# Nicholaswogan/clima

Measured on AMD Instinct MI355X. Metric: radiate() calls/sec, higher is better.
Workload: dtype f64; 1 GPU; ModernEarth column, one Radtran%radiate call: nz=200, nw=1000 (600 IR + 600 solar bins), 8 g-points, 8 zenith angles, nk=5; config 2 of BASELINE.json; parallelism=1 GPU

## Files before the change

### clima_amd/csrc/kernels.hip

```cpp
#include "radtran_dev.h"
#include <algorithm>
#include <cstring>
#include <mutex>
#include <set>
#include <utility>

namespace clima {

static bool ensure_max_lds(const void *fn, int bytes = 160 * 1024) {
  static std::mutex mu;
  static std::set<std::pair<int, const void *>> done;
  int dev = 0;
  if (hipGetDevice(&dev) != hipSuccess) return false;
  std::lock_guard<std::mutex> lk(mu);
  if (done.count({dev, fn})) return true;
  if (hipFuncSetAttribute(fn, hipFuncAttributeMaxDynamicSharedMemorySize, bytes) != hipSuccess) return false;
  done.insert({dev, fn});
  return true;
}
static int device_cus() {
  static std::mutex mu;
  static int cus[64] = {0};
  int dev = 0;
  if (hipGetDevice(&dev) != hipSuccess || dev < 0 || dev >= 64) return 256;
// ... 108 lines not shown
  double p = fma3(K.c[0], r, K.c[1]);
#pragma unroll
  for (int i = 2; i < 11; i++) p = fma3(p, r, K.c[i]);
  p = __builtin_fma(p, r, 0.5);
  p = __builtin_fma(p, r, 1.0);
  p = __builtin_fma(p, r, 1.0);
  return exp_scale(p, k);
}

constexpr int EXP2_N = 256;
__device__ const double EXP2_TAB[EXP2_N] = {
    1.0, 1.0027112750502025, 1.0054299011128027, 1.0081558981184175,
    1.0108892860517005, 1.0136300849514894, 1.016378314910953, 1.019133996077738,
    1.0218971486541166, 1.0246677928971357, 1.0274459491187637, 1.030231637686041,
    1.0330248790212284, 1.0358256936019572, 1.0386341019613787, 1.041450124688316,
    1.0442737824274138, 1.0471050958792898, 1.0499440858006872, 1.0527907730046264,
    1.0556451783605572, 1.0585073227945128, 1.061377227289262, 1.0642549128844645,
    1.0671404006768237, 1.0700337118202419, 1.0729348675259756, 1.075843889062791,
    1.0787607977571199, 1.0816856149932152, 1.0846183622133092, 1.0875590609177697,
    1.0905077326652577, 1.0934643990728858, 1.0964290818163769, 1.099401802630222,
    1.102382583307841, 1.1053714457017412, 1.1083684117236787, 1.1113735033448175,
    1.1143867425958924, 1.1174081515673693, 1.1204377524096067, 1.12347556733302,
    1.1265216186082418, 1.129575928566288, 1.1326385195987192, 1.1357094141578055,
    1.1387886347566916, 1.1418762039695616, 1.1449721444318042, 1.148076478840179,
    1.1511892299529827, 1.154310420590216, 1.1574400736337511, 1.1605782120274988,
    1.1637248587775775, 1.1668800369524817, 1.1700437696832502, 1.1732160801636373,
    1.1763969916502812, 1.1795865274628758, 1.182784710984341, 1.1859915656609938,
    1.189207115002721, 1.1924313825831512, 1.1956643920398273, 1.1989061670743806,
    1.202156731452703, 1.2054161090051239, 1.2086843236265816, 1.2119613992768012,
    1.215247359980469, 1.2185422298274085, 1.2218460329727576, 1.2251587936371455,
    1.22848053610687, 1.2318112847340759, 1.2351510639369334, 1.2384998981998165,
    1.241857812073484, 1.245224830175258, 1.2486009771892048, 1.2519862778663162,
    1.255380757024691, 1.2587844395497165, 1.2621973503942507, 1.2656195145788063,
    1.2690509571917332, 1.2724917033894028, 1.275941778396392, 1.2794012075056693,
    1.2828700160787783, 1.2863482295460256, 1.2898358734066657, 1.2933329732290895,
    1.2968395546510096, 1.3003556433796506, 1.3038812651919358, 1.3074164459346773,
    1.3109612115247644, 1.3145155879493546, 1.318079601266064, 1.3216532776031575,
    1.3252366431597413, 1.3288297242059544, 1.3324325470831615, 1.3360451382041458,
    1.339667524053303, 1.3432997311868353, 1.3469417862329458, 1.3505937158920345,
    1.3542555469368927, 1.3579273062129011, 1.3616090206382248, 1.365300717204012,
    1.3690024229745905, 1.3727141650876684, 1.3764359707545302, 1.380167867260238,
    1.383909881963832, 1.387662042298529, 1.3914243757719262, 1.3951969099662003,
    1.3989796725383112, 1.4027726912202048, 1.4065759938190154, 1.4103896082172707,
    1.4142135623730951, 1.4180478843204152, 1.4218926021691656, 1.4257477441054942,
    1.42961333839197, 1.433489413367789, 1.4373759974489824, 1.4412731191286257,
    1.4451808069770467, 1.449099089642035, 1.4530279958490526, 1.4569675544014438,
    1.460917794180647, 1.4648787441464057, 1.4688504333369818, 1.4728328908693675,
    1.4768261459394993, 1.4808302278224719, 1.4848451658727524, 1.488870989524397,
    1.4929077282912648, 1.4969554117672355, 1.5010140696264256, 1.5050837316234065,
    1.5091644275934228, 1.5132561874526098, 1.5173590411982147, 1.5214730189088146,
    1.5255981507445384, 1.529734466947287, 1.533881997840956, 1.5380407738316568,
    1.5422108254079407, 1.5463921831410214, 1.550584877685, 1.5547889397770887,
    1.559004400237837, 1.5632312899713576, 1.567469639965553, 1.5717194812923414,
    1.5759808451078865, 1.5802537626528246, 1.5845382652524937, 1.588834384317164,
    1.593142151342267, 1.597461597908627, 1.6017927556826934, 1.606135656416771,
    1.6104903319492543, 1.6148568142048607, 1.6192351351948637, 1.6236253270173289,
    1.6280274218573478, 1.632441451987275, 1.6368674497669644, 1.6413054476440063,
    1.645755478153965, 1.6502175739206177, 1.6546917676561943, 1.6591780921616162,
    1.6636765803267364, 1.6681872651305825, 1.6727101796415966, 1.6772453570178785,
    1.681792830507429, 1.6863526334483934, 1.6909247992693053, 1.6955093614893326,
    1.7001063537185235, 1.7047158096580513, 1.709337763100463, 1.713972247929926,
    1.718619298122478, 1.723278947746274, 1.7279512309618377, 1.732636182022311,
    1.7373338352737062, 1.7420442251551564, 1.746767386199169, 1.7515033530318782,
    1.7562521603732995, 1.761013843037584, 1.7657884359332727, 1.7705759740635547,
    1.7753764925265212, 1.7801900265154245, 1.785016611318935, 1.789856282321401,
    1.7947090750031072, 1.7995750249405351, 1.804454167806624, 1.809346539371032,
    1.8142521755003989, 1.8191711121586085, 1.8241033854070534, 1.8290490314048973,
    1.8340080864093424, 1.8389805867758937, 1.843966568958626, 1.8489660695104508,
    1.8539791250833855, 1.8590057724288205, 1.864046048397789, 1.8690999899412386,
    1.8741676341103, 1.8792490180565602, 1.8843441790323345, 1.8894531543909392,
    1.8945759815869656, 1.8997126981765553, 1.9048633418176741, 1.9100279502703899,
    1.9152065613971474, 1.9203992131630474, 1.925605943636125, 1.930826790987627,
    1.9360617934922943, 1.9413109895286405, 1.9465744175792332, 1.9518521162309783,
    1.9571441241754002, 1.9624504802089273, 1.9677712232331759, 1.9731063922552343,
    1.978456026387951, 1.9838201648502194, 1.9891988469672663, 1.9945921121709402};
constexpr double EXP2_PER_E = 369.3299304675746, EXP2_PER_10 = 850.4135922911647;
__device__ __forceinline__ double exp_tab_any(double x, double k, const double *s_tab) {
  double f, nf, r;
  {
#pragma clang fp contract(off)
    f = x * k;
    nf = __builtin_rint(f);
    r = f - nf;
  }
  const int n = (int)nf;
  const double t = s_tab[n & (EXP2_N - 1)];
  double p = 2.239395190875157e-12;
  p = __builtin_fma(p, r, 3.3083026805413713e-09);
  p = __builtin_fma(p, r, 3.6655655969101062e-06);
  p = __builtin_fma(p, r, 0.0027076061740622863);
  p = __builtin_fma(p, r, 1.0);
  return __builtin_ldexp(t * p, n >> 8);
}
__device__ __forceinline__ double exp_tab(double x, const double *s_tab) { return exp_tab_any(x, EXP2_PER_E, s_tab); }
__device__ __forceinline__ double ten2power_tab(double y, const double *s_tab) { return exp_tab_any(y, EXP2_PER_10, s_tab); }
__device__ __forceinline__ double rcp_n1(double x) {
  double r = __builtin_amdgcn_rcp(x);
  const double e = __builtin_fma(-x, r, 1.0);
  return __builtin_fma(r, e, r);
}

__device__ __forceinline__ double ten2power(double y) { return fast_exp(y * LN10); }

__device__ __forceinline__ double planck_fcn(double nu, double T, const ExpK &K) {
  return 1.0e3 * ((2.0 * PLANK * (nu * nu * nu)) / (C_LIGHT * C_LIGHT)) *
         ((1.0) / (fast_exp((PLANK * nu) / (K_BOLTZ_SI * T), K) - 1.0));
}
__device__ __forceinline__ double planck_fcn(double nu, double T) {
  return 1.0e3 * ((2.0 * PLANK * (nu * nu * nu)) / (C_LIGHT * C_LIGHT)) *
         ((1.0) / (fast_exp((PLANK * nu) / (K_BOLTZ_SI * T)) - 1.0));
}

template <int CTRL, int ROW_MASK, int BANK_MASK>
__device__ __forceinline__ double dpp_mov(double old, double src) {
  const long long o = __double_as_longlong(old), v = __double_as_longlong(src);
  const int lo = __builtin_amdgcn_update_dpp((int)o, (int)v, CTRL, ROW_MASK, BANK_MASK, false);
  const int hi = __builtin_amdgcn_update_dpp((int)(o >> 32), (int)(v >> 32), CTRL, ROW_MASK, BANK_MASK, false);
  return __longlong_as_double(((long long)hi << 32) | (unsigned int)lo);
}
constexpr int DPP_ROW_SHL = 0x100, DPP_ROW_SHR = 0x110, DPP_WAVE_SHR1 = 0x138, DPP_ROW_BCAST15 = 0x142, DPP_ROW_BCAST31 = 0x143;
template <int D>
__device__ __forceinline__ double row_shr(double old, double x) { return dpp_mov<DPP_ROW_SHR + D, 0xf, 0xf>(old, x); }
template <int D>
__device__ __forceinline__ double row_shl(double old, double x) { return dpp_mov<DPP_ROW_SHL + D, 0xf, 0xf>(old, x); }

__device__ __forceinline__ bool is_close(double a, double b, double tol) {
  return fabs(a - b) <= fabs(tol * fmax(fabs(a), fabs(b)));
}

__device__ __forceinline__ int bracket(const double *xt, int n, double x) {
  if (x < xt[0]) return 0;
  if (x >= xt[n - 1]) return n - 2;
  int lo = 0, hi = n - 1;
  while (hi - lo > 1) {
    int mid = (lo + hi) >> 1;
    if (x < xt[mid]) hi = mid; else lo = mid;
  }
  return lo;
}

constexpr int PREP_AXIS_MAX = 1024;
constexpr int PREP_ZERO_BLOCKS = 32;

__device__ __forceinline__ ColumnDev column_at(const ColumnDev &c0, const BatchStrides &bs, const int cb) {
  ColumnDev c = c0;
  const size_t oc = (size_t)cb * bs.col, op = (size_t)cb * bs.prep;
  c.T += oc; c.P += oc; c.dz += oc; c.dens += oc; c.pdens += oc; c.radii += oc; c.T_surface += oc;
  c.meta += 2 * oc;
  c.log10P += op; c.cols += op; c.foreign_col += op; c.absw += op; c.q += op;
  c.ix += 2 * op;
  return c;
}

__global__ __launch_bounds__(256) void k_prep(PrepParams p) {
  __shared__ double s_axis[PREP_AXIS_MAX];
  const int nz = p.nz;
  const int cb = blockIdx.y;
  const ColumnDev c = column_at(p.col, p.bs, cb);
  const int *src = c.meta + 1 + nz;
  if (blockIdx.x == 0) {
    for (int j = threadIdx.x; j < nz; j += blockDim.x) {
      const double Pj = c.P[j], dzj = c.dz[j];
      double fc = 0.0;
      for (int i0 = 0; i0 < p.nsp; i0 += 8) {
        double d[8];
#pragma unroll
        for (int k = 0; k < 8; k++) d[k] = c.dens[min(i0 + k, p.nsp - 1) * nz + j];
#pragma unroll
        for (int k = 0; k < 8; k++) {
          const int i = i0 + k;
          if (i < p.nsp) {
            const double col = d[k] * dzj;
            c.cols[i * nz + j] = col;
            if (p.has_cont && i != p.LH2O) fc = fc + col;
          }
        }
      }
      c.log10P[j] = log10(Pj);
      c.foreign_col[j] = fc;
    }
    return;
  }
  if ((int)blockIdx.x > p.nslots + p.nabs) {
    const int zb = (int)blockIdx.x - (p.nslots + p.nabs + 1);
    const int arr = zb / PREP_ZERO_BLOCKS, part = zb - arr * PREP_ZERO_BLOCKS;
    double *dst = p.zero_ptr[arr] + (size_t)cb * p.bs.res;
    const size_t n = p.zero_count[arr];
    for (size_t i = (size_t)part * blockDim.x + threadIdx.x; i < n; i += (size_t)PREP_ZERO_BLOCKS * blockDim.x) dst[i] = 0.0;
    return;
  }
  if ((int)blockIdx.x > p.nslots) {
    const int e = (int)blockIdx.x - p.nslots - 1;
    const int a = p.abs_a[e], b = p.abs_b[e], kind = p.abs_kind[e];
    for (int j = threadIdx.x; j < nz; j += blockDim.x) {
      double w;
      if (kind == ABS_CIA) w = c.dens[a * nz + j] * c.dens[b * nz + j] * c.dz[j];
      else if (kind == ABS_COLUMN) w = c.dens[a * nz + j] * c.dz[j];
      else if (kind == ABS_H2O_SELF) w = c.dens[a * nz + j] * (c.dens[a * nz + j] * c.dz[j]);
      else if (kind == ABS_ZERO) w = 0.0;
      else {
        double fc = 0.0;
        for (int i = 0; i < p.nsp; i++)
          if (i != p.LH2O) fc = fc + c.dens[i * nz + j] * c.dz[j];
        w = c.dens[a * nz + j] * fc;
      }
      c.absw[e * nz + j] = w;
    }
    return;
  }
  const int s = blockIdx.x - 1;
  const SlotDev &sl = p.slots[s];
  const bool in_lds = sl.n <= PREP_AXIS_MAX;
  const double *in = sl.source <= 0 ? c.P : sl.source == 1 ? c.T : c.radii + (size_t)(sl.source - 2) * nz;
  const int j0 = threadIdx.x;
  int js0 = 0;
  double x0 = 0.0;
  if (j0 < nz) { js0 = sl.source < 0 ? j0 : src[j0]; x0 = in[j0]; }
  if (in_lds)
    for (int i = threadIdx.x; i < sl.n; i += blockDim.x) s_axis[i] = sl.axis[i];
  __syncthreads();
  const double *axis = in_lds ? s_axis : sl.axis;
  for (int j = threadIdx.x; j < nz; j += blockDim.x) {
    const int js = j == j0 ? js0 : (sl.source < 0 ? j : src[j]);
    const double xin = (j == j0 && js == j) ? x0 : in[js];
    double x;
    if (sl.source < 0) x = log10(xin * 1.0e6);
    else if (sl.source == 0) x = log10(xin);
    else x = xin;
    if (sl.flag_clamp && (x < sl.lo || x > sl.hi)) atomicMax(c.err_flag, p.call_id);
    x = fmin(fmax(x, sl.lo), sl.hi);
    const int i = bracket(axis, sl.n, x);
    c.ix[s * nz + j] = i;
    c.q[s * nz + j] = (x - axis[i]) / (axis[i + 1] - axis[i]);
  }
}

void launch_prep(const PrepParams &p, hipStream_t s) {
  hipLaunchKernelGGL(k_prep, dim3(1 + p.nslots + p.nabs + p.nzero * PREP_ZERO_BLOCKS, p.ncol > 0 ? p.ncol : 1), dim3(256), 0, s, p);
}


__device__ __forceinline__ double lerp1(const double *f, int i, double q) {
  const double p1 = 1.0 - q;
  return p1 * f[i] + q * f[i + 1];
}

constexpr int OP_THREADS = 256;
constexpr int HWREG_HW_ID_WAVE_ID = (3 << 11) | (0 << 6) | 4;

template <bool COHERENT>
__device__ __forceinline__ void st_opr(double *p, double v) {
  if constexpr (COHERENT) __hip_atomic_store(p, v, __ATOMIC_RELAXED, __HIP_MEMORY_SCOPE_AGENT);
  else *p = v;
}
template <bool COHERENT>
__device__ __forceinline__ double ld_opr(const double *p) {
  if constexpr (COHERENT) return __hip_atomic_load(p, __ATOMIC_RELAXED, __HIP_MEMORY_SCOPE_AGENT);
  else return *p;
}

#ifdef CLIMA_STAMPS
__device__ long long *g_stamp_buf = nullptr;
#endif

template <bool TIGHT>
constexpr int rb_lo(int k) {
  constexpr int wide[8] = {0, 1, 5, 10, 18, 27, 39, 52};
  constexpr int tight[8] = {0, 5, 12, 19, 27, 35, 45, 55};
  return TIGHT ? tight[k] : wide[k];
}
template <bool TIGHT>
constexpr int rb_hi(int k) {
  constexpr int wide[8] = {0, 11, 24, 36, 45, 53, 58, 62};
  constexpr int tight[8] = {0, 8, 18, 28, 36, 44, 51, 58};
  return TIGHT ? tight[k] : wide[k];
}

constexpr unsigned long long KEY_IDX_MASK = 0x1f8ULL;
__device__ __forceinline__ double key_weight(const double key, const double *s_wxy) {
  const unsigned int off = (unsigned int)__double_as_longlong(key) & (unsigned int)KEY_IDX_MASK;
  return *(const double *)((const char *)s_wxy + off);
}

__device__ __forceinline__ void rebin_window(const double (&key)[64], const bool xys, const double *s_wxy,
                                             const double *s_Ew, const double *rW, double (&out)[8]) {
  asm volatile("" ::: "memory");
  double E[8];
#pragma unroll
  for (int k = 1; k < 8; k++) E[k] = s_Ew[k];
  double C = 0.0, IC = 0.0, Ie[9];
#pragma unroll
  for (int k = 1; k < 8; k++) Ie[k] = -1.0e300;
  constexpr int RB = 8;
  double wn[RB];
#pragma unroll
  for (int u = 0; u < RB; u++) wn[u] = key_weight(key[u], s_wxy);
#pragma unroll
  for (int pb = 0; pb < 64; pb += RB) {
    double wv[RB];
#pragma unroll
    for (int u = 0; u < RB; u++) wv[u] = wn[u];
    if (pb + RB < 64) {
#pragma unroll
      for (int u = 0; u < RB; u++)
        wn[u] = key_weight(key[pb + RB + u], s_wxy);
    }
    const double Cb = C, ICb = IC;
#pragma unroll
    for (int u = 0; u < RB; u++) {
      const int j = pb + u;
      const double v = key[j];
#pragma unroll
      for (int k = 1; k < 8; k++) {
        if (j >= rb_lo<true>(k) && j <= rb_hi<true>(k))
          Ie[k] = dmax(Ie[k], __builtin_fma(v, E[k] - C, IC));
      }
      IC = __builtin_fma(v, wv[u], IC);
      C = C + wv[u];
    }
    if (!xys) {
      double c2 = Cb, ic2 = ICb;
#pragma unroll
      for (int u = 0; u < RB; u++) {
        const int j = pb + u;
        const double v = key[j];
#pragma unroll
        for (int k = 1; k < 8; k++) {
          if (j >= rb_lo<false>(k) && j <= rb_hi<false>(k) && !(j >= rb_lo<true>(k) && j <= rb_hi<true>(k)))
            Ie[k] = dmax(Ie[k], __builtin_fma(v, E[k] - c2, ic2));
        }
        ic2 = __builtin_fma(v, wv[u], ic2);
        c2 = c2 + wv[u];
      }
    }
  }
  Ie[8] = IC;
  out[0] = Ie[1] * rW[0];
#pragma unroll
  for (int q = 1; q < 8; q++) out[q] = (Ie[q + 1] - Ie[q]) * rW[q];
}

#include "rorr_xys_asm.inc"
#ifndef CLIMA_RORR_ASM
#define CLIMA_RORR_ASM 1
#endif
constexpr bool RORR_ASM = CLIMA_RORR_ASM != 0;

template <int RM>
__device__ __forceinline__ void rorr_mix8(const double (&x)[8], const double (&y)[8],
                                          double (*sI)[OP_THREADS], const int tid, const int tile,
                                          const double *s_wxy, const double *s_E,
                                          const double *s_Ew, const double *rW,
                                          double (&out)[8], const double *rorr_tab, long long *stamps = nullptr, const int stamp_slot = 0) {
  (void)stamps; (void)stamp_slot;
  double key[64];
  bool ysorted = true, xsorted = true;
#pragma unroll
  for (int j = 0; j < 7; j++) {
    ysorted = ysorted && (y[j] <= y[j + 1]);
    xsorted = xsorted && (x[j] <= x[j + 1]);
  }
  const bool ys = __all(ysorted), xys = ys && __all(xsorted);
  if constexpr (RM == 0 && RORR_ASM) {
    if (__builtin_expect(xys, 1)) {
      double xx[8], yy[8];
#pragma unroll
      for (int g = 0; g < 8; g++) { xx[g] = x[g]; yy[g] = y[g]; }
      typedef __attribute__((address_space(3))) const double lds_cdouble;
      const unsigned wxy_addr = (unsigned)(unsigned long)(lds_cdouble *)s_wxy;
      asm volatile(RORR_XYS_ASM_TEXT
                   : "+v"(xx[0]), "+v"(xx[1]), "+v"(xx[2]), "+v"(xx[3]), "+v"(xx[4]), "+v"(xx[5]), "+v"(xx[6]), "+v"(xx[7]),
                     "+v"(yy[0]), "+v"(yy[1]), "+v"(yy[2]), "+v"(yy[3]), "+v"(yy[4]), "+v"(yy[5]), "+v"(yy[6]), "+v"(yy[7])
                   : "v"(wxy_addr), "s"(rorr_tab)
                   : RORR_XYS_ASM_CLOBBERS);
#pragma unroll
      for (int g = 0; g < 8; g++) out[g] = yy[g];
      STAMP(stamps, stamp_slot);
      return;
    }
  }
#pragma unroll
  for (int i = 0; i < 8; i++) {
#pragma unroll
    for (int j = 0; j < 8; j++) {
      const double v = x[i] + y[j];
      unsigned long long b = (unsigned long long)__double_as_longlong(v);
      b = (b & ~KEY_IDX_MASK) | (unsigned long long)((i * 8 + j) << 3);
      key[i * 8 + j] = __longlong_as_double((long long)b);
    }
  }
#define CE(a, b)                              \
  {                                           \
    const double lo_ = dmin(key[a], key[b]);  \
    const double hi_ = dmax(key[a], key[b]);  \
    key[a] = lo_;                             \
    key[b] = hi_;                             \
  }
#define CE_X(a, b) \
  if (!xys) CE(a, b)
#define CE_MERGE_BEGIN(P, M)
#define CE_MERGE_END
  if (!ys) {
#define CE_FULL_HEAD
#include "sort_network_64.inc"
#undef CE_FULL_HEAD
  }
  if (!xys) {
#define CE_L8_FIRST
#include "sort_network_64.inc"
#undef CE_L8_FIRST
  }
#define CE_L8_REST
#include "sort_network_64.inc"
#undef CE_L8_REST
  if (!xys) {
#define CE_L16_FIRST
#include "sort_network_64.inc"
#undef CE_L16_FIRST
  }
#define CE_L16_REST
#include "sort_network_64.inc"
#undef CE_L16_REST
  if (!xys) {
#define CE_L32_FIRST
#include "sort_network_64.inc"
#undef CE_L32_FIRST
  }
#define CE_L32_REST
#include "sort_network_64.inc"
#undef CE_L32_REST
#undef CE_MERGE_BEGIN
#undef CE_MERGE_END
#undef CE_X
#undef CE
  STAMP(stamps, stamp_slot);
  if constexpr (RM == 0) {
    rebin_window(key, xys, s_wxy, s_Ew, rW, out);
    return;
  }
  const double *E = s_Ew;
  constexpr bool MULTI = RM == 2;
  double S = 0.0, c0 = 0.0;
  double bk = E[1], bn = E[2];
  const double *en = s_E + 2;
  double *slot = &sI[0][tid];
  double *const slot_end = &sI[0][tid] + 8 * OP_THREADS;
  constexpr int RB = 8;
  double wn[RB];
#pragma unroll
  for (int u = 0; u < RB; u++) wn[u] = key_weight(key[u], s_wxy);
#pragma unroll
  for (int pb = 0; pb < 64; pb += RB) {
    double wv[RB];
#pragma unroll
    for (int u = 0; u < RB; u++) wv[u] = wn[u];
    if (pb + RB < 64) {
#pragma unroll
      for (int u = 0; u < RB; u++)
        wn[u] = key_weight(key[pb + RB + u], s_wxy);
    }
#pragma unroll
    for (int u = 0; u < RB; u++) {
      const double v = key[pb + u];
      const double w = wv[u];
      const double c1 = c0 + w;
      if (c1 > bk) {
        *slot = __builtin_fma(v, bk - c0, S);
        slot += OP_THREADS;
        bk = bn;
        en++;
        if constexpr (MULTI) {
          while (c1 > bk) {
            *slot = __builtin_fma(v, bk - c0, S);
            slot += OP_THREADS;
            bk = *en;
            en++;
          }
        }
      }
      bn = *en;
      S = __builtin_fma(v, w, S);
      c0 = c1;
    }
  }
  for (; slot < slot_end; slot += OP_THREADS) *slot = S;
  double Ik[8];
#pragma unroll
  for (int q = 0; q < 8; q++) Ik[q] = sI[q][tid];
  out[0] = Ik[0] * rW[0];
#pragma unroll
  for (int q = 1; q < 8; q++) out[q] = (Ik[q] - Ik[q - 1]) * rW[q];
}

struct LayerTerms {
  double tausg, taua, tauc, tausc, taup, tausp, gt;
};

template <int RM, bool CUSTOM, bool COHERENT>
__device__ __forceinline__ void opacity8_body(const OpacityParams &p, const int tile, const size_t oc,
                                              const size_t opf, const size_t oo) {
  const ColumnDev &c = p.col;
  constexpr int NG = 8;
  __shared__ double sI[RM == 0 ? 1 : NG][OP_THREADS];
  __shared__ __align__(512) double s_wxy[NG * NG];
  __shared__ double s_E[NG + 4];
  const int tid = threadIdx.x;
  __shared__ double s_Ew[2 * NG + 1];
  __shared__ double s_e2[EXP2_N];
  __shared__ double rW[NG];
  {
    static_assert(EXP2_N == OP_THREADS, "one table entry per thread");
    const double v_wxy = p.wxy[tid & (NG * NG - 1)];
    const double v_Ep = p.wbin_e_pad[min(tid, NG + 3)];
    const double v_e2 = EXP2_TAB[tid];
    const double v_e = p.wbin_e[min(tid, NG)], v_e1 = p.wbin_e[min(tid + 1, NG)];
    const double v_w = p.wbin[min(max(tid - (NG + 1), 0), NG - 1)];
    if (tid < NG * NG) s_wxy[tid] = v_wxy;
    if (tid < NG + 4) s_E[tid] = v_Ep;
    s_e2[tid] = v_e2;
    if (tid < 2 * NG + 1) s_Ew[tid] = tid < NG + 1 ? v_e : v_w;
    if (tid < NG) rW[tid] = 1.0 / (v_e1 - v_e);
  }
  __syncthreads();

#ifdef CLIMA_STAMPS
  const long long wt0 = __builtin_amdgcn_s_memrealtime();
#endif
  const int nz = p.nz;
  const int nsrc = c.meta[2 * oc + 0];
  const long total = (long)p.nbins * nsrc;
  long t = (long)tile * OP_THREADS + tid;
  const bool valid = t < total;
  if (!valid) t = total - 1;
  const int l = p.bin_lo + (int)(t / nsrc);
  const int ent = c.meta[2 * oc + 1 + (int)(t % nsrc)];
  const int j = ent & SRC_LAYER;
  const bool pair = (ent & SRC_PAIR) != 0, exact = (ent & SRC_EXACT) != 0;
  const int n = nz - 1 - j;

  STAMP(p.stamps, 0);
  auto layer_terms = [&](const int jl, LayerTerms &o) {
#ifdef CLIMA_EXP_NOTERMS
    o.tausg = 1e-3; o.taua = 1e-3; o.tauc = TINY; o.tausc = TINY * TINY; o.taup = 0.0; o.tausp = 0.0; o.gt = 0.0;
    if (jl >= 0) return;
#endif
    const double dzj = c.dz[oc + jl];
    double tausg = 0.0;
  #pragma unroll 4
    for (int i = 0; i < p.nray; i++) tausg = tausg + p.ray[i].data[l] * c.cols[opf + p.ray[i].sp1 * nz + jl];
    double taua = 0.0;
    constexpr int AB = ABS_BATCH;
    for (int e0 = 0; e0 < p.nabs; e0 += AB) {
      int ixx[AB];
      double qq[AB], ww[AB];
  #pragma unroll
      for (int u = 0; u < AB; u++) {
        const AbsEntry &x = p.abs[e0 + u];
        ixx[u] = c.ix[2 * opf + x.slot * nz + jl];
        qq[u] = c.q[opf + x.slot * nz + jl];
        ww[u] = c.absw[opf + (e0 + u) * nz + jl];
      }
      double v0[AB], v1[AB];
  #pragma unroll
      for (int u = 0; u < AB; u++) {
        const AbsEntry &x = p.abs[e0 + u];
#ifdef CLIMA_EXP_NODEP
        const double *base = x.data + (x.nT ? (size_t)l * x.nT : (size_t)l);
#else
        const double *base = x.data + (x.nT ? (size_t)l * x.nT + ixx[u] : (size_t)l);
#endif
        v0[u] = base[0];
        v1[u] = base[x.nT ? 1 : 0];
      }
  #pragma unroll
      for (int u = 0; u < AB; u++) {
        const AbsEntry &x = p.abs[e0 + u];
        double sgm = v0[u];
        if (x.nT) sgm = ten2power_tab((1.0 - qq[u]) * v0[u] + qq[u] * v1[u], s_e2);
        taua = taua + sgm * ww[u];
      }
    }
    double tauc = TINY, tausc = TINY * TINY;
    double g0c = TINY;
    if constexpr (CUSTOM) {
      const int ix = c.ix[2 * opf + p.cust.slot * nz + jl];
      const double q = c.q[opf + p.cust.slot * nz + jl];
      const size_t o = (size_t)l * p.cust.nP;
      tauc = lerp1(p.cust.dtau + o, ix, q) * dzj;
      const double w0c = lerp1(p.cust.w0 + o, ix, q);
      g0c = lerp1(p.cust.g0 + o, ix, q);
      tausc = w0c * tauc;
    }
    double tausp = 0.0, taup = 0.0;
    double tausp_1[MAX_PART], gtp[MAX_PART];
    for (int i = 0; i < p.npart; i++) {
      const PartDev &pt = p.part[i];
      const int ix = c.ix[2 * opf + pt.slot * nz + jl];
      const double q = c.q[opf + pt.slot * nz + jl];
      const double w0p = lerp1(pt.w0 + (size_t)l * pt.nrad, ix, q);
      const double qext = lerp1(pt.qext + (size_t)l * pt.nrad, ix, q);
      gtp[i] = lerp1(pt.gt + (size_t)l * pt.nrad, ix, q);
      const double rr = c.radii[oc + pt.p_ind * nz + jl];
      const double taup_1 = qext * PI * (rr * rr) * c.pdens[oc + pt.p_ind * nz + jl] * dzj;
      taup = taup + taup_1;
      tausp_1[i] = w0p * taup_1;
      tausp = tausp + tausp_1[i];
    }
    double gt = 0.0;
    for (int i = 0; i < p.npart; i++) gt = gt + gtp[i] * tausp_1[i] / fmax(TAU_MIN, (tausp + tausg + tausc));
    gt = gt + g0c * tausc / fmax(TAU_MIN, (tausp + tausg + tausc));
    gt = fmin(gt, MAX_GT);
    o.tausg = tausg; o.taua = taua; o.tauc = tauc; o.tausc = tausc; o.taup = taup; o.tausp = tausp; o.gt = gt;
  };
  LayerTerms lt;
  const bool terms_first = (__builtin_amdgcn_s_getreg(HWREG_HW_ID_WAVE_ID) & 1) == 0;
  __shared__ double s_lt[7][OP_THREADS];
  if (terms_first) {
    layer_terms(j, lt);
    if constexpr (RM == 0 && RORR_ASM) {
      s_lt[0][tid] = lt.tausg; s_lt[1][tid] = lt.taua; s_lt[2][tid] = lt.tauc; s_lt[3][tid] = lt.tausc;
      s_lt[4][tid] = lt.taup; s_lt[5][tid] = lt.tausp; s_lt[6][tid] = lt.gt;
    }
  }

  STAMP(p.stamps, 1);
  auto k_times_col = [&](const int s, const int jl, const int iP, const int iT, const double q1, const double q2,
                         double (&kc)[NG]) {
    const KDev &kd = p.k[s];
    const double p1 = 1.0 - q1, p2 = 1.0 - q2;
    const double *slab = kd.log10k + (size_t)l * kd.nT * kd.nP * NG;
    const double *f11 = slab + ((size_t)iT * kd.nP + iP) * NG;
    const double *f21 = f11 + NG;
    const double *f12 = f11 + (size_t)kd.nP * NG;
    const double *f22 = f12 + NG;
    const double col = c.cols[opf + kd.sp * nz + jl];
#pragma unroll
    for (int g = 0; g < NG; g++) {
      const double fx1 = p1 * f11[g] + q1 * f21[g];
      const double fx2 = p1 * f12[g] + q1 * f22[g];
      kc[g] = ten2power_tab(p2 * fx1 + q2 * fx2, s_e2) * col;
    }
  };
  double tk[NG];
#pragma unroll
  for (int g = 0; g < NG; g++) tk[g] = 0.0;
  int iP_n = c.ix[2 * opf + p.k[0].slotP * nz + j], iT_n = c.ix[2 * opf + p.k[0].slotT * nz + j];
  double q1_n = c.q[opf + p.k[0].slotP * nz + j], q2_n = c.q[opf + p.k[0].slotT * nz + j];
  for (int s = 0; s < p.nk; s++) {
    const int iP = iP_n, iT = iT_n;
    const double q1 = q1_n, q2 = q2_n;
    int jv = j;
    if constexpr (RM == 0 && RORR_ASM) asm volatile("" : "+v"(jv));
    if (s + 1 < p.nk) {
      const KDev &kn = p.k[s + 1];
      iP_n = c.ix[2 * opf + kn.slotP * nz + jv]; iT_n = c.ix[2 * opf + kn.slotT * nz + jv];
      q1_n = c.q[opf + kn.slotP * nz + jv]; q2_n = c.q[opf + kn.slotT * nz + jv];
    }
    double kc[NG];
    k_times_col(s, jv, iP, iT, q1, q2, kc);
    STAMP(p.stamps, 2 + 3 * s);
    if (s == 0) {
#pragma unroll
      for (int g = 0; g < NG; g++) tk[g] = kc[g];
    } else {
#ifdef CLIMA_STAMPS
      if (tile == 100 && threadIdx.x == 0) g_stamp_buf = p.stamps;
#endif
      double out[NG];
      rorr_mix8<RM>(tk, kc, sI, tid, tile, s_wxy, s_E, s_Ew, rW, out, p.rorr_tab, p.stamps, 21 + s);
#pragma unroll
      for (int g = 0; g < NG; g++) tk[g] = out[g];
      STAMP(p.stamps, 4 + 3 * s);
    }
  }
  if (!terms_first) {
    layer_terms(j, lt);
  } else if constexpr (RM == 0 && RORR_ASM) {
    lt.tausg = s_lt[0][tid]; lt.taua = s_lt[1][tid]; lt.tauc = s_lt[2][tid]; lt.tausc = s_lt[3][tid];
    lt.taup = s_lt[4][tid]; lt.tausp = s_lt[5][tid]; lt.gt = s_lt[6][tid];
  }
  STAMP(p.stamps, 20);
#ifdef CLIMA_STAMPS
  if (p.stamps && (tid & 63) == 0) {
    const long w = (long)tile * (OP_THREADS / 64) + (tid >> 6);
    p.stamps[64 + 2 * w] = wt0;
    p.stamps[64 + 2 * w + 1] = __builtin_amdgcn_s_memrealtime();
  }
#endif

  auto store_layer = [&](const int nn, const LayerTerms &T, const double (&tkv)[NG]) {
    asm volatile("" ::: "memory");
    const double *wbin = s_Ew + NG + 1;
    double tb = 0.0;
    const size_t base = ((size_t)l * NG) * nz + nn;
    const double scat = T.tausg + T.tausp + T.tausc;
    if (p.write_w0) {
#pragma unroll
      for (int g = 0; g < NG; g++) {
        const double tau = T.tausg + T.taua + T.taup + tkv[g] + T.tauc;
        double w0;
        if (tau <= TAU_MIN) w0 = 0.0;
        else w0 = fmin(MAX_W0, scat / tau);
        st_opr<COHERENT>(&p.w0[oo + base + (size_t)g * nz], w0);
      }
    }
#pragma unroll
    for (int g = 0; g < NG; g++) {
      const double tau = T.tausg + T.taua + T.taup + tkv[g] + T.tauc;
      st_opr<COHERENT>(&p.tau[oo + base + (size_t)g * nz], tau);
      tb = tb + tau * wbin[g];
    }
    st_opr<COHERENT>(&p.scat[oo + (size_t)l * nz + nn], scat);
    st_opr<COHERENT>(&p.tau_band[oo + (size_t)l * nz + nn], tb);
    st_opr<COHERENT>(&p.g[oo + (size_t)l * nz + nn], T.gt);
  };
  if (valid) {
    store_layer(n, lt, tk);
    if (pair) {
      if (exact) {
        store_layer(n - 1, lt, tk);
      } else {
        LayerTerms lt2;
        layer_terms(j + 1, lt2);
        if (p.nk == 1) {
          double tk2[NG];
          k_times_col(0, j + 1, c.ix[2 * opf + p.k[0].slotP * nz + j], c.ix[2 * opf + p.k[0].slotT * nz + j], c.q[opf + p.k[0].slotP * nz + j],
                      c.q[opf + p.k[0].slotT * nz + j], tk2);
          store_layer(n - 1, lt2, tk2);
        } else {
          store_layer(n - 1, lt2, tk);
        }
      }
    }
  }
}

template <int RM, bool CUSTOM>
__global__ __launch_bounds__(OP_THREADS, 2) void k_opacity8(OpacityParams p) {
  opacity8_body<RM, CUSTOM, false>(p, (int)blockIdx.x, 0, 0, 0);
}

constexpr int OPG_MAX_NG = 32;

__global__ __launch_bounds__(64) void k_opacity_generic(OpacityParams p, int N2) {
  extern __shared__ __align__(16) double sm[];
  const int ng = p.ng, n2 = ng * ng, nz = p.nz;
  double *s_key = sm;
  double *s_cum = s_key + N2;
  double *s_tk = s_cum + (n2 + 1);
  double *s_kc = s_tk + ng;
  double *s_out = s_kc + ng;
  double *s_wxy = s_out + ng;
  int *s_idx = (int *)(s_wxy + n2);
  const int lane = threadIdx.x;
  for (int m = lane; m < n2; m += 64) s_wxy[m] = p.wxy[m];
  const ColumnDev &c = p.col;
  const long t = blockIdx.x;
  const int l = p.bin_lo + (int)(t / nz);
  const int j = (int)(t % nz);
  const int n = nz - 1 - j;
  const double dzj = c.dz[j];
  const int jk = (p.nk >= 2) ? c.meta[1 + nz + j] : j;

  double tausg = 0.0;
  for (int i = 0; i < p.nray; i++) tausg = tausg + p.ray[i].data[l] * c.cols[p.ray[i].sp1 * nz + j];
  double taua = 0.0;
  for (int e = 0; e < p.nabs; e++) {
    const AbsEntry &x = p.abs[e];
    double sgm;
    if (x.nT) {
      const int ix = c.ix[x.slot * nz + j];
      const double q = c.q[x.slot * nz + j];
      const double *base = x.data + (size_t)l * x.nT + ix;
      sgm = ten2power((1.0 - q) * base[0] + q * base[1]);
    } else {
      sgm = x.data[l];
    }
    taua = taua + sgm * c.absw[e * nz + j];
  }
  double tauc = TINY, tausc = TINY * TINY, g0c = TINY;
  if (p.cust.on) {
    const int ix = c.ix[p.cust.slot * nz + j];
    const double q = c.q[p.cust.slot * nz + j];
    const size_t o = (size_t)l * p.cust.nP;
    tauc = lerp1(p.cust.dtau + o, ix, q) * dzj;
    const double w0c = lerp1(p.cust.w0 + o, ix, q);
    g0c = lerp1(p.cust.g0 + o, ix, q);
    tausc = w0c * tauc;
  }
  double tausp = 0.0, taup = 0.0;
  double tausp_1[MAX_PART], gtp[MAX_PART];
  for (int i = 0; i < p.npart; i++) {
    const PartDev &pt = p.part[i];
    const int ix = c.ix[pt.slot * nz + j];
    const double q = c.q[pt.slot * nz + j];
    const double w0p = lerp1(pt.w0 + (size_t)l * pt.nrad, ix, q);
    const double qext = lerp1(pt.qext + (size_t)l * pt.nrad, ix, q);
    gtp[i] = lerp1(pt.gt + (size_t)l * pt.nrad, ix, q);
    const double rr = c.radii[pt.p_ind * nz + j];
    const double taup_1 = qext * PI * (rr * rr) * c.pdens[pt.p_ind * nz + j] * dzj;
    taup = taup + taup_1;
    tausp_1[i] = w0p * taup_1;
    tausp = tausp + tausp_1[i];
  }
  double gt = 0.0;
  for (int i = 0; i < p.npart; i++) gt = gt + gtp[i] * tausp_1[i] / fmax(TAU_MIN, (tausp + tausg + tausc));
  gt = gt + g0c * tausc / fmax(TAU_MIN, (tausp + tausg + tausc));
  gt = fmin(gt, MAX_GT);

  for (int s = 0; s < p.nk; s++) {
    const KDev &kd = p.k[s];
    if (lane < ng) {
      const int iP = c.ix[kd.slotP * nz + jk], iT = c.ix[kd.slotT * nz + jk];
      const double q1 = c.q[kd.slotP * nz + jk], q2 = c.q[kd.slotT * nz + jk];
      const double p1 = 1.0 - q1, p2 = 1.0 - q2;
      const double *f11 = kd.log10k + (size_t)l * kd.nT * kd.nP * ng + ((size_t)iT * kd.nP + iP) * ng;
      const double *f21 = f11 + ng, *f12 = f11 + (size_t)kd.nP * ng, *f22 = f12 + ng;
      const double fx1 = p1 * f11[lane] + q1 * f21[lane];
      const double fx2 = p1 * f12[lane] + q1 * f22[lane];
      const double v = ten2power(p2 * fx1 + q2 * fx2) * c.cols[kd.sp * nz + jk];
      if (s == 0) s_tk[lane] = v;
      else s_kc[lane] = v;
    }
    __syncthreads();
    if (s == 0) continue;
    for (int m = lane; m < N2; m += 64) {
      double v = __longlong_as_double(0x7ff0000000000000LL);
      if (m < n2) v = s_tk[m / ng] + s_kc[m % ng];
      s_key[m] = v;
      s_idx[m] = m;
    }
    __syncthreads();
    for (int k = 2; k <= N2; k <<= 1) {
      for (int d = k >> 1; d > 0; d >>= 1) {
        for (int u = lane; u < (N2 >> 1); u += 64) {
          const int i = ((u & ~(d - 1)) << 1) | (u & (d - 1));
          const int x = i + d;
          const bool up = (i & k) == 0;
          const double ka = s_key[i], kb = s_key[x];
          const int ia = s_idx[i], ib = s_idx[x];
          const bool gtr = (ka > kb) || (ka == kb && ia > ib);
          if (gtr == up) { s_key[i] = kb; s_key[x] = ka; s_idx[i] = ib; s_idx[x] = ia; }
        }
        __syncthreads();
      }
    }
    {
      const int seg = (N2 + 63) / 64;
      double tot = 0.0;
      for (int q = 0; q < seg; q++) {
        const int m = lane * seg + q;
        if (m < n2) tot = tot + s_wxy[s_idx[m]];
      }
      double incl = tot;
#pragma unroll
      for (int d = 1; d < 64; d <<= 1) {
        const double nb = __shfl_up(incl, d);
        if (lane >= d) incl = incl + nb;
      }
      double cum = incl - tot;
      if (lane == 0) { cum = 0.0; s_cum[0] = 0.0; }
      for (int q = 0; q < seg; q++) {
        const int m = lane * seg + q;
        if (m < n2) { cum = cum + s_wxy[s_idx[m]]; s_cum[m + 1] = cum; }
      }
    }
    __syncthreads();
    if (lane < ng) {
      const double b0 = p.wbin_e[lane], b1 = p.wbin_e[lane + 1];
      int lo = 0, hi = n2;
      while (lo < hi) { const int mid = (lo + hi) >> 1; if (s_cum[mid + 1] <= b0) lo = mid + 1; else hi = mid; }
      double acc = 0.0;
      for (int m = lo; m < n2; m++) {
        const double e0 = s_cum[m], e1 = s_cum[m + 1];
        if (e0 >= b1) break;
        const double a = e0 > b0 ? e0 : b0, b = e1 < b1 ? e1 : b1;
        if (b > a) acc = acc + (b - a) * s_key[m];
      }
      s_out[lane] = acc / (b1 - b0);
    }
    __syncthreads();
    if (lane < ng) s_tk[lane] = s_out[lane];
    __syncthreads();
  }

  if (lane < ng) {
    const double tau = tausg + taua + taup + s_tk[lane] + tauc;
    double w0;
    if (tau <= TAU_MIN) w0 = 0.0;
    else w0 = fmin(MAX_W0, (tausg + tausp + tausc) / tau);
    const size_t o = ((size_t)l * ng + lane) * nz + n;
    p.tau[o] = tau;
// ... 1456 lines not shown
    if (lane == 63) rho = 0.0;
  }
  const double mm = rcp_nr(1.0 - rho * dU);
  constexpr bool STEP_REGS = NW == 4;
  double *sStep = sF0 + (size_t)4 * NW * (nl + 1) + threadIdx.x;
  double stA[WSCAN_STEPS], stB[WSCAN_STEPS];
  {
    double dummy = 0.0, bq = wave_reverse(uU * mm);
    wscan_build(dummy, bq, stA);
    double sb = dD * (1.0 + dU * mm * rho);
    dummy = 0.0;
    wscan_build(dummy, sb, stB);
    if constexpr (!STEP_REGS) {
#pragma unroll
      for (int k = 0; k < WSCAN_STEPS; k++) {
        sStep[(size_t)k * blockDim.x] = stA[k];
        sStep[(size_t)(WSCAN_STEPS + k) * blockDim.x] = stB[k];
      }
    }
  }
  const double kA = uU * mm * rho;
  const double kS = dU * mm;
  int face[L + 1];
#pragma unroll
  for (int s = 0; s <= L; s++) face[s] = a + max(s - pad, 0);

  for (int c0 = c_begin; c0 < c_end; c0 += IRB_TILE) {
    const int nt = min(IRB_TILE, c_end - c0);
    __syncthreads();
    for (int idx = threadIdx.x; idx < nt * nl; idx += blockDim.x) {
      const int cj = idx / nl, n = idx - cj * nl;
      const double *Tc = p.T + (size_t)(c0 + cj) * p.b_T;
      const double temp = (n == nz) ? p.T_surface[(size_t)(c0 + cj) * p.b_Ts] : Tc[nz - 1 - n];
      sB[(size_t)cj * nl + n] = p.bplanck ? p.bplanck[n] : planck_fcn(avg_freq, temp);
    }
    __syncthreads();
    for (int cj = 0; cj < nt; cj++) {
      const double *Bc = sB + (size_t)cj * nl;
      double Bf[L + 1];
#pragma unroll
      for (int s = 0; s <= L; s++) Bf[s] = Bc[face[s]];
      double dd[2 * L], cpbv[L], cmbv[L];
      double cp0_top, b1n_last = 0.0;
      {
        double dpv = 0.0;
        E4 u = make_e(G[0], X[0]);
#pragma unroll
        for (int t = 0; t < L; t++) {
          const double Bt = Bf[t], Bb = Bf[t + 1];
          const double b1n = (Bb - Bt) * itau[t];
          const double b0n = (itau[t] == 0.0) ? 0.5 * (Bt + Bb) : Bt;
          const double cp0 = PI * (b0n + b1n * rq[t]);
          cpbv[t] = PI * (b0n + b1n * (tauv[t] + rq[t]));
          const double cm0 = PI * (b0n - b1n * rq[t]);
          cmbv[t] = PI * (b0n + b1n * (tauv[t] - rq[t]));
          if (t == 0) {
            cp0_top = cp0;
            dpv = (0.0 - cm0) * rr[0];
            dd[0] = dpv;
          } else {
            const E4 v = make_e(G[t], X[t]);
            const double E1 = v.e2 * (cp0 - cpbv[t - 1]) - v.e4 * (cm0 - cmbv[t - 1]);
            const double dn = E1 * rr[2 * t - 1] - ar[2 * t - 1] * dpv;
            dd[2 * t - 1] = dn;
            const double E2 = u.e3 * (cp0 - cpbv[t - 1]) + u.e1 * (cmbv[t - 1] - cm0);
            dpv = E2 * rr[2 * t] - ar[2 * t] * dn;
            dd[2 * t] = dpv;
            u = v;
          }
          if (t == L - 1) b1n_last = b1n;
        }
        const double Ssfc = hard ? emis * PI * Bf[L] : PI * (Bf[L] + 0.5 * b1n_last);
        const double E = is_sfc ? Ssfc - cpbv[L - 1] + Rsfc * cmbv[L - 1] : 0.0 - cpbv[L - 1];
        dd[2 * L - 1] = E * rr[2 * L - 1] - ar[2 * L - 1] * dpv;
      }
      {
        double al = 0.0;
#pragma unroll
        for (int r = 2 * L - 1; r >= 0; r--) {
          al = dd[r] - cc[r] * al;
          dd[r] = al;
        }
      }
      const double uS = empty ? 0.0 : dd[0] * ea3 - dd[1] * ea4 + cp0_top;
      const double dS = empty ? 0.0 : dd[2 * L - 2] * eb3 + dd[2 * L - 1] * eb4 + cmbv[L - 1];
      const double sgr = wscan_apply(wave_reverse(uS + kA * dS),
                                     [&](int k) { return STEP_REGS ? stA[k] : sStep[(size_t)k * blockDim.x]; });
      const double sig = wave_reverse(wave_shr1(sgr));
      const double sa = wscan_apply(dS + kS * (rho * dS + sig),
                                    [&](int k) { return STEP_REGS ? stB[k] : sStep[(size_t)(WSCAN_STEPS + k) * blockDim.x]; });
      const double Din = wave_shr1(sa);
      const double Uin = mm * (rho * dS + sig + rho * dD * Din);
      const int buf = cj & 1;
      double *sFu = sF0 + (size_t)buf * 2 * NW * (nl + 1) + (size_t)(0 * NW + wave) * (nl + 1);
      double *sFd = sF0 + (size_t)buf * 2 * NW * (nl + 1) + (size_t)(1 * NW + wave) * (nl + 1);
      double top_up = 0.0;
#pragma unroll
      for (int t = 0; t < L; t++) {
        const int i = a + t - pad;
        const E4 e = make_e(G[t], X[t]);
        const double y1 = dd[2 * t] + be[2 * t] * Uin + ga[2 * t] * Din;
        const double y2 = dd[2 * t + 1] + be[2 * t + 1] * Uin + ga[2 * t + 1] * Din;
        const int lv = t >= pad ? i + 1 : nl;
        sFu[lv] = wcol * (y1 * e.e1 + y2 * e.e2 + cpbv[t]);
        sFd[lv] = wcol * (y1 * e.e3 + y2 * e.e4 + cmbv[t]);
        if (t == 0) top_up = (y1 * e.e3 - y2 * e.e4) + cp0_top;
      }
      if (is_toa) {
        sFu[0] = wcol * top_up;
        sFd[0] = 0.0;
      }
      __syncthreads();
      for (int n = threadIdx.x; n < nl; n += blockDim.x) {
        const double *sF = sF0 + (size_t)buf * 2 * NW * (nl + 1);
        const size_t o = (size_t)(c0 + cj) * p.b_out + (size_t)ll * nl + (nz - n);
        double fu = 0.0, fd = 0.0;
        if (g0 > 0) { fu = p.ir_fup_a[o]; fd = p.ir_fdn_a[o]; }
#pragma unroll
        for (int w = 0; w < NW; w++) {
          fu = fu + sF[(size_t)(0 * NW + w) * (nl + 1) + n];
          fd = fd + sF[(size_t)(1 * NW + w) * (nl + 1) + n];
        }
        p.ir_fup_a[o] = fu;
        p.ir_fdn_a[o] = fd;
      }
    }
  }
  __syncthreads();
  }
}

bool launch_twostream_ir_batch(TwoStreamParams &p, int ncol, hipStream_t s, int force_nw) {
  const int lmax = std::max((p.nz + 63) / 64, p.force_slots);
  if (lmax > 8 || p.n_ir <= 0 || ncol <= 0 || p.ng < 1) return false;
  const int nw = (lmax > 4 || p.ng > 8 || force_nw == 4) ? 4 : 8;
  const size_t lds = sizeof(double) * ((size_t)IRB_TILE * ((size_t)p.nz + 1) + (size_t)4 * nw * ((size_t)p.nz + 2) + (nw == 8 ? 2 * WSCAN_STEPS * 64 * nw : 0));
  if (lds > 160 * 1024) return false;
  using Kern = void (*)(TwoStreamParams, int, int);
  static const Kern kern8[4] = {k_twostream_ir_batch<1, 8>, k_twostream_ir_batch<2, 8>, k_twostream_ir_batch<3, 8>, k_twostream_ir_batch<4, 8>};
  static const Kern kern4[8] = {k_twostream_ir_batch<1, 4>, k_twostream_ir_batch<2, 4>, k_twostream_ir_batch<3, 4>, k_twostream_ir_batch<4, 4>,
                                k_twostream_ir_batch<5, 4>, k_twostream_ir_batch<6, 4>, k_twostream_ir_batch<7, 4>, k_twostream_ir_batch<8, 4>};
  const Kern k = nw == 8 ? kern8[lmax - 1] : kern4[lmax - 1];
  if (!ensure_max_lds((const void *)k)) return false;
  int cpb = (ncol + 3) / 4;
  if (cpb < IRB_TILE) cpb = std::min(ncol, IRB_TILE);
  const dim3 grid(p.n_ir, 1, (ncol + cpb - 1) / cpb), blk(64 * nw);
  hipLaunchKernelGGL(k, grid, blk, lds, s, p, ncol, cpb);
  return true;
}

#ifndef FUSED_NZMAX
#define FUSED_NZMAX 8
#endif
template <int RM, bool CUSTOM, int LSEL, bool PAIRED = false, bool HALF = false>
__global__ __launch_bounds__(OP_THREADS, 2) void k_fused(OpacityParams op, TwoStreamParams ts, FusedParams fp) {
  extern __shared__ __align__(16) double lds[];
  const int per_col = fp.n_op + fp.n_ts;
  const int cb = (int)blockIdx.x / per_col, loc = (int)blockIdx.x - cb * per_col;
  if (loc < fp.n_op) {
    __builtin_amdgcn_s_setprio(1);
    const size_t oc = (size_t)cb * fp.bs.col;
    if ((long)loc * OP_THREADS < (long)op.nbins * op.col.meta[2 * oc])
      opacity8_body<RM, CUSTOM, true>(op, loc, oc, (size_t)cb * fp.bs.prep, (size_t)cb * fp.bs.opr);
    __builtin_amdgcn_fence(__ATOMIC_RELEASE, "workgroup");
    asm volatile("s_waitcnt vmcnt(0)" ::: "memory");
    __syncthreads();
    if (threadIdx.x == 0)
      __hip_atomic_store(&fp.done[(size_t)cb * fp.bs.done + loc], fp.call_id, __ATOMIC_RELAXED, __HIP_MEMORY_SCOPE_AGENT);
    return;
  }
  const int b = loc - fp.n_op;
  int gy, bl;
  {
    const int nS = ts.n_sol, nI = ts.n_ir, E = fp.sol_early, Lt = nS - E;
    if constexpr (HALF) {
      gy = 0;
      bl = b < E ? b : b < E + nI ? nS + (b - E) : b - nI;
    } else {
      const int seg[6] = {E, E, nI, nI, Lt, Lt};
      int r = b, k = 0;
      while (k < 5 && r >= seg[k]) { r -= seg[k]; k++; }
      gy = k & 1;
      bl = k < 2 ? r : k < 4 ? nS + r : E + r;
    }
  }
  const bool solar = bl < ts.n_sol;
  const int ll = solar ? ts.sol_lo + bl : ts.ir_lo + (bl - ts.n_sol);
  const int l = (solar ? ts.sol_start : ts.ir_start) + ll;
#ifdef CLIMA_STAMPS
  if (op.stamps && threadIdx.x == 0 && cb == 0) op.stamps[64 + 2 * 3128 + 3 * b] = __builtin_amdgcn_s_memrealtime();
#endif
  __shared__ int s_ok;
  if (threadIdx.x == 0) {
    const int nsrc = op.col.meta[2 * (size_t)cb * fp.bs.col];
    const long t0 = (long)(l - op.bin_lo) * nsrc;
    const int d0 = max((int)(t0 / OP_THREADS), 0), d1 = min((int)((t0 + nsrc - 1) / OP_THREADS), fp.n_op - 1);
    const int *done = fp.done + (size_t)cb * fp.bs.done;
    int ok = 1;
    for (int d = d0; d <= d1 && ok; d++) {
      int spins = 0;
      while (__hip_atomic_load(&done[d], __ATOMIC_RELAXED, __HIP_MEMORY_SCOPE_AGENT) != fp.call_id) {
        __builtin_amdgcn_s_sleep(16);
        if (++spins > fp.max_spins) { ok = 0; break; }
      }
    }
    if (!ok) atomicMax(fp.timeout_flag, fp.call_id);
    s_ok = ok;
  }
  __syncthreads();
  if (!s_ok) return;
#ifdef CLIMA_STAMPS
  if (op.stamps && threadIdx.x == 0 && cb == 0) op.stamps[64 + 2 * 3128 + 3 * b + 1] = __builtin_amdgcn_s_memrealtime();
  const int tslot = HALF ? (b == fp.sol_early / 2 ? 32 : (b == fp.sol_early + ts.n_ir / 2 ? 48 : -1))
                         : (b == 1500) ? 32 : (b == 2200 ? 48 : -1);
#else
  const int tslot = -1;
#endif
  const TsOfs co{(size_t)cb * fp.bs.opr, (size_t)cb * fp.bs.col, (size_t)cb * fp.bs.res};
  if constexpr (HALF) {
    if (solar) twostream_p_body<LSEL, true, FUSED_NZMAX, true, false, false, true>(ts, bl, lds, gy, 0, tslot, co);
    else twostream_p_body<LSEL, false, 0, true, false, false, true>(ts, bl - ts.n_sol, lds, gy, 0, tslot, co);
  } else if constexpr (LSEL == 0 && PAIRED) {
    if (fp.slots == 2) {
      if (solar) twostream_p_body<2, true, FUSED_NZMAX, true, true, true>(ts, bl, lds, gy, 0, tslot, co);
      else twostream_p_body<2, false, 0, true, true, true>(ts, bl - ts.n_sol, lds, gy, 0, tslot, co);
    } else {
      if (solar) twostream_p_body<4, true, FUSED_NZMAX, true, true, true>(ts, bl, lds, gy, 0, tslot, co);
      else twostream_p_body<4, false, 0, true, true, true>(ts, bl - ts.n_sol, lds, gy, 0, tslot, co);
    }
  } else if constexpr (LSEL == 0) {
    if (fp.slots == 2) {
      if (solar) twostream_p_body<2, true, FUSED_NZMAX, true, true>(ts, bl, lds, gy, 0, tslot, co);
      else twostream_p_body<2, false, 0, true, true>(ts, bl - ts.n_sol, lds, gy, 0, tslot, co);
    } else if (fp.slots == 3) {
      if (solar) twostream_p_body<3, true, FUSED_NZMAX, true, true>(ts, bl, lds, gy, 0, tslot, co);
      else twostream_p_body<3, false, 0, true, true>(ts, bl - ts.n_sol, lds, gy, 0, tslot, co);
    } else {
      if (solar) twostream_p_body<4, true, FUSED_NZMAX, true, true>(ts, bl, lds, gy, 0, tslot, co);
      else twostream_p_body<4, false, 0, true, true>(ts, bl - ts.n_sol, lds, gy, 0, tslot, co);
    }
  } else {
    if (solar) twostream_p_body<LSEL, true, FUSED_NZMAX, true, false, PAIRED>(ts, bl, lds, gy, 0, tslot, co);
    else twostream_p_body<LSEL, false, 0, true, false, PAIRED>(ts, bl - ts.n_sol, lds, gy, 0, tslot, co);
  }
#ifdef CLIMA_STAMPS
  __syncthreads();
  if (op.stamps && threadIdx.x == 0 && cb == 0) op.stamps[64 + 2 * 3128 + 3 * b + 2] = __builtin_amdgcn_s_memrealtime();
#endif
}

int fused_tiles(const OpacityParams &op) {
  return (int)(((long)op.nbins * op.nsrc + OP_THREADS - 1) / OP_THREADS);
}

static size_t wave_lds(int nz, int cols) { return sizeof(double) * (3 * cols + 1) * ((size_t)nz + 1); }
static int wave_groups(int ng) { return (ng + TSW_COLS - 1) / TSW_COLS; }

LaunchPlan plan_radiate(const PlanIn &in) {
  LaunchPlan pl{};
  const int slots = (in.nz + 63) / 64, nb = in.n_sol + in.n_ir;
  const bool plain = in.rebin_mode == 0 && !in.cust_on;
  const bool coop8 = !in.batch && in.ng == 8 && (long)in.op_n * in.nsrc <= in.coop_items;
  if (in.compute_opacity) {
    if (in.ng < 1 || in.ng > OPG_MAX_NG) pl.opacity = OP_UNSUPPORTED;
    else if (in.ng == 8) pl.opacity = coop8 ? OP_COOP : OP_TILE;
    else pl.opacity = in.generic_opacity ? OP_GENERIC : OP_COOP;
    pl.coop_ng = in.ng <= 8 ? 8 : in.ng <= 16 ? 16 : 32;
  }

  const bool want_fused = in.compute_opacity && in.fused && in.allow_fused && !coop8 && !in.ts_block_mode;
  const bool covered = in.ng == 8 && slots >= 2 && slots <= 8 && in.nzen <= MAX_ZEN && (slots <= 4 || plain) &&
                       (long)in.op_n * in.nz > 0 && nb > 0;
  if (want_fused && covered) {
    const int hs = (in.nz + 31) / 32, ps = 2 * ((in.nz / 2 + 63) / 64);
    TsPlan &f = pl.fused;
    if (!in.no_half && plain && hs >= 3 && hs <= 7) { f.form = TS_HALF; f.slots = hs; }
    else if (in.ncol <= 1 && in.allow_paired && in.all_pairs && !(in.nz & 1) && plain && ps <= 8) { f.form = TS_PAIRED; f.slots = ps; }
    else { f.form = TS_WAVE; f.slots = slots; }
    f.cols = f.form == TS_HALF ? 2 * TSW_COLS : TSW_COLS;
    f.groups = f.per_launch = in.ng / f.cols;
    f.lds = wave_lds(in.nz, f.cols);
    pl.write_w0 = !in.w0_from_scat;
  } else {
    pl.write_w0 = true;
  }

  const int lmax = std::max(slots, in.force_slots);
  if ((in.ir_batch || (!in.ts_block_mode && in.nzen <= MAX_ZEN)) && lmax <= 8 && wave_lds(in.nz, TSW_COLS) <= 64 * 1024) {
    const int hs = (in.nz + 31) / 32;
    TsPlan &t = pl.ts;
    if (!in.no_half && in.ng % 8 == 0 && hs >= 3 && hs <= 7 && in.force_slots == 0 && in.nzen <= MAX_ZEN &&
        !(in.ng == 8 && in.n_sol > 0 && nb < 512)) { t.form = TS_HALF; t.slots = hs; t.cols = 2 * TSW_COLS; }
    else { t.form = TS_WAVE; t.slots = lmax; t.cols = TSW_COLS; }
    t.groups = (in.ng + t.cols - 1) / t.cols;
    t.per_launch = t.groups <= 2 ? t.groups : 1;
    t.lds = wave_lds(in.nz, t.cols);
  }
  if (!in.ir_batch) pl.block = plan_block(in.nz, in.ng, in.ts_ncols_env);

  const bool headed_fused = in.fused && in.allow_fused && !coop8;
  const bool whole_stores = headed_fused ? pl.fused.form == TS_HALF : (pl.ts.form == TS_HALF && pl.ts.groups == 1);
  pl.prep_clears = in.compute_opacity && !in.ts_block_mode && slots <= 8 && wave_groups(in.ng) >= 2 && !whole_stores;
  pl.caller_clears = in.ir_batch && wave_groups(in.ng) > 1;
  pl.ts.zero_launch = pl.ts.groups > 1 && !pl.prep_clears && !pl.caller_clears;
  return pl;
}

using FusedKern = void (*)(OpacityParams, TwoStreamParams, FusedParams);
static FusedKern fused_kernel(const TsPlan &f, int rebin_mode, bool cust_on) {
  static const FusedKern kp[3] = {k_fused<0, false, 0, true>, k_fused<0, false, 6, true>, k_fused<0, false, 8, true>};
  static const FusedKern kh[5] = {k_fused<0, false, 3, false, true>, k_fused<0, false, 4, false, true>, k_fused<0, false, 5, false, true>,
                                  k_fused<0, false, 6, false, true>, k_fused<0, false, 7, false, true>};
  static const FusedKern k04[2][3] = {{k_fused<0, false, 0>, k_fused<1, false, 0>, k_fused<2, false, 0>},
                                      {k_fused<0, true, 0>, k_fused<1, true, 0>, k_fused<2, true, 0>}};
  static const FusedKern k58[4] = {k_fused<0, false, 5>, k_fused<0, false, 6>, k_fused<0, false, 7>, k_fused<0, false, 8>};
  if (f.form == TS_HALF) return kh[f.slots - 3];
  if (f.form == TS_PAIRED) return kp[f.slots <= 4 ? 0 : f.slots == 6 ? 1 : 2];
  return f.slots <= 4 ? k04[cust_on ? 1 : 0][rebin_mode] : k58[f.slots - 5];
}

bool launch_fused(const OpacityParams &op, TwoStreamParams ts, FusedParams fp, const TsPlan &f, hipStream_t s) {
  if (f.form == TS_NONE) return false;
  fp.n_op = fused_tiles(op);
  fp.n_ts = (ts.n_sol + ts.n_ir) * f.groups;
  fp.slots = f.slots;
  if (fp.ncol < 1) fp.ncol = 1;
  {
    const long first_round_bins = ((long)2 * device_cus() * OP_THREADS) / std::max(op.nsrc, 1);
    fp.sol_early = (int)std::min<long>(ts.n_sol, std::max<long>(0, first_round_bins - (long)(ts.sol_start + ts.sol_lo - op.bin_lo)));
  }
  ts.col_base = 0; ts.accumulate = f.groups > 1 ? 1 : 0;
  ts.scat = op.scat; ts.w0_from_scat = op.write_w0 ? 0 : 1;
  const long items = (long)fp.ncol * (fp.n_op + fp.n_ts);
  const FusedKern k = fused_kernel(f, op.rebin_mode, op.cust.on != 0);
  if (f.lds > 48 * 1024 && !ensure_max_lds((const void *)k, 64 * 1024)) return false;
  hipLaunchKernelGGL(k, dim3((unsigned)items), dim3(OP_THREADS), f.lds, s, op, ts, fp);
  return true;
}

bool launch_fused_twostream_only(TwoStreamParams &ts, int slots, const int *meta_nsrc, hipStream_t s, bool half, bool paired) {
  if (ts.ng != 8 || slots < 2 || slots > 8 || (ts.nz + 63) / 64 > slots || ts.nzen > MAX_ZEN) return false;
  if (half && (paired || slots < 3 || slots > 7 || (ts.nz + 31) / 32 > slots)) return false;
  if (paired && ((ts.nz & 1) || (slots & 1) || 2 * ((ts.nz / 2 + 63) / 64) > slots)) return false;
  TsPlan f{};
  f.form = half ? TS_HALF : paired ? TS_PAIRED : TS_WAVE;
  f.slots = slots;
  f.cols = half ? 2 * TSW_COLS : TSW_COLS;
  f.groups = ts.ng / f.cols;
  f.lds = wave_lds(ts.nz, f.cols);
  OpacityParams op;
  memset(&op, 0, sizeof(op));
  op.nz = ts.nz;
  op.col.meta = meta_nsrc;
  FusedParams fp;
  memset(&fp, 0, sizeof(fp));
  fp.ncol = 1;
  fp.n_op = 0;
  fp.n_ts = (ts.n_sol + ts.n_ir) * f.groups;
  fp.slots = slots;
  fp.sol_early = ts.n_sol;
  ts.col_base = 0; ts.accumulate = half ? 0 : 1;
  const FusedKern k = fused_kernel(f, 0, false);
  if (f.lds > 48 * 1024 && !ensure_max_lds((const void *)k, 64 * 1024)) return false;
  hipLaunchKernelGGL(k, dim3(fp.n_ts), dim3(OP_THREADS), f.lds, s, op, ts, fp);
  return true;
}

#ifndef CLIMA_INT_CHUNK
#define CLIMA_INT_CHUNK 32
#endif
constexpr int INT_CHUNK = CLIMA_INT_CHUNK;

__global__ __launch_bounds__(256) void k_integrate_partial(IntegrateParams p) {
  const int nl = p.nz + 1;
  const int a = blockIdx.y;
  const bool sol = a >= 2;
  if (sol && !p.do_solar) return;
  const double *src = a == 0 ? p.ir_fup_a : a == 1 ? p.ir_fdn_a : a == 2 ? p.sol_fup_a : p.sol_fdn_a;
  const double *freq = sol ? p.sol_freq : p.ir_freq;
  const int lo = sol ? p.sol_lo : p.ir_lo, cnt = sol ? p.sol_n : p.ir_n;
  const int l0 = lo + blockIdx.x * INT_CHUNK;
  const int l1 = min(lo + cnt, l0 + INT_CHUNK);
  for (int i = threadIdx.x; i < nl; i += blockDim.x) {
    double acc = 0.0;
    if (l0 < l1) {
      double v[INT_CHUNK];
#pragma unroll
      for (int k = 0; k < INT_CHUNK; k++) v[k] = (l0 + k < l1) ? src[(size_t)(l0 + k) * nl + i] : 0.0;
#pragma unroll
      for (int k = 0; k < INT_CHUNK; k++)
        if (l0 + k < l1) acc = __builtin_fma(v[k], freq[l0 + k] - freq[l0 + k + 1], acc);
    }
    p.partial[((size_t)a * p.nchunk + blockIdx.x) * nl + i] = acc;
  }
}

__global__ __launch_bounds__(1024) void k_integrate_final(IntegrateParams p) {
  const int nl = p.nz + 1;
  if (p.timeout_out && threadIdx.x == 0) {
    const int t = *p.timeout_flag;
    *p.timeout_out = (t == p.id_opr ? 1.0 : 0.0) + (t == p.id_sol ? 1024.0 : 0.0);
  }
  for (int t = threadIdx.x; t < 4 * nl; t += blockDim.x) {
    const int a = t / nl, i = t - a * nl;
    if (a >= 2 && !p.do_solar) {
      if (p.flux_part) p.flux_n[a * nl + i] = p.flux_part[a * nl + i];
      continue;
    }
    double acc = 0.0;
#pragma unroll 8
    for (int k = 0; k < p.nchunk; k++) acc = acc + p.partial[((size_t)a * p.nchunk + k) * nl + i];
    p.flux_n[a * nl + i] = acc;
    if (p.flux_part) p.flux_part[a * nl + i] = acc;
  }
  __syncthreads();
  if (p.f_total)
    for (int i = threadIdx.x; i < nl; i += blockDim.x)
      p.f_total[i] = (p.flux_n[3 * nl + i] - p.flux_n[2 * nl + i]) + (p.flux_n[1 * nl + i] - p.flux_n[0 * nl + i]);
}

__global__ __launch_bounds__(256) void k_integrate_partial_b(BatchIntegrateParams p) {
  const int nl = p.nz + 1;
  const int a = blockIdx.y, col = blockIdx.z;
  const double *src = (a == 0 ? p.fup_a : p.fdn_a) + (size_t)col * p.spec_stride;
  const int l0 = p.ir_lo + blockIdx.x * INT_CHUNK;
  const int l1 = min(p.ir_lo + p.ir_n, l0 + INT_CHUNK);
  if (l1 <= l0) {
    for (int i = threadIdx.x; i < nl; i += blockDim.x) p.partial[(((size_t)col * 2 + a) * p.nchunk + blockIdx.x) * nl + i] = 0.0;
    return;
  }
  for (int i = threadIdx.x; i < nl; i += blockDim.x) {
    double v[INT_CHUNK], df[INT_CHUNK];
#pragma unroll
    for (int k = 0; k < INT_CHUNK; k++) {
      const int l = min(l0 + k, l1 - 1);
      v[k] = src[(size_t)l * nl + i];
      df[k] = p.freq[l] - p.freq[l + 1];
    }
    double acc = 0.0;
#pragma unroll
    for (int k = 0; k < INT_CHUNK; k++)
      if (l0 + k < l1) acc = __builtin_fma(v[k], df[k], acc);
    p.partial[(((size_t)col * 2 + a) * p.nchunk + blockIdx.x) * nl + i] = acc;
  }
}

__global__ __launch_bounds__(256) void k_integrate_final_b(BatchIntegrateParams p) {
  const int nl = p.nz + 1;
  const int col = blockIdx.x;
  for (int i = threadIdx.x; i < nl; i += blockDim.x) {
    double up = 0.0, dn = 0.0;
    for (int k0 = 0; k0 < p.nchunk; k0 += 8) {
      double u[8], d[8];
#pragma unroll
      for (int k = 0; k < 8; k++) {
        const int kk = min(k0 + k, p.nchunk - 1);
        u[k] = p.partial[(((size_t)col * 2 + 0) * p.nchunk + kk) * nl + i];
        d[k] = p.partial[(((size_t)col * 2 + 1) * p.nchunk + kk) * nl + i];
      }
#pragma unroll
      for (int k = 0; k < 8; k++)
        if (k0 + k < p.nchunk) { up = up + u[k]; dn = dn + d[k]; }
    }
    double *o = p.out + (size_t)(p.col0 + col) * nl;
    o[i] = up;
    o[p.out_arr + i] = dn;
    o[2 * p.out_arr + i] = (p.flux_n[3 * nl + i] - p.flux_n[2 * nl + i]) + (dn - up);
  }
}

void launch_integrate_batch(const BatchIntegrateParams &p, int ncol, hipStream_t s) {
  hipLaunchKernelGGL(k_integrate_partial_b, dim3(p.nchunk, 2, ncol), dim3(256), 0, s, p);
  hipLaunchKernelGGL(k_integrate_final_b, dim3(ncol), dim3(256), 0, s, p);
}

int integrate_chunks(int nbins) { return nbins <= 0 ? 1 : (nbins + INT_CHUNK - 1) / INT_CHUNK; }

#ifndef CLIMA_INT_LV
#define CLIMA_INT_LV 16
#endif
#ifndef CLIMA_INT_CG
#define CLIMA_INT_CG 32
#endif
constexpr int INT_LV = CLIMA_INT_LV;
constexpr int INT_CG = CLIMA_INT_CG;

__global__ __launch_bounds__(INT_LV * INT_CG) void k_integrate_one(IntegrateParams p) {
// ... 262 lines not shown
```

### clima_amd/csrc/radtran_api.hip

```cpp
#include "../../include/clima_radtran_hip.h"
#include "radtran_dev.h"

#include <rccl/rccl.h>
#include <sys/stat.h>
#include <unistd.h>
#include <ctime>

#include <algorithm>
#include <cmath>
#include <cstdio>
#include <cstdlib>
#include <chrono>
#include <cstring>
#include <functional>
#include <set>
#include <string>
#include <utility>
#include <limits>
#include <vector>

using namespace clima;

namespace {

// ... 51 lines not shown
    n = 0;
    owned = true;
  }
  ~DevBuf() { release(); }
};

struct KTabHost {
  int sp, ng, nP, nT;
  std::vector<double> weights, log10P, temp, log10k;
  DevBuf<double> d_log10k, d_log10P, d_temp;
};
struct XsHost {
  int type, dim, sp1, sp2, nT;
  std::vector<double> temp, data;
  DevBuf<double> d_data, d_temp;
};
struct PartHost {
  int p_ind, nrad;
  std::vector<double> radii, w0, qext, gt;
  DevBuf<double> d_radii, d_w0, d_qext, d_gt;
};

struct Radtran;
struct ChannelObj {
  Radtran *parent = nullptr;
  int which = 0;
  int ind_start = 0, ind_end = -1, nw = 0;
  std::vector<double> wavl, freq;
  DevBuf<double> d_freq;
};
struct WrkObj {
  Radtran *parent = nullptr;
  int which = 0;
  DevBuf<double> fup_a, fdn_a, amean, tau_band;
};

struct BatchRun {
  int n = 0, first_call = 0, CH = 0;
  bool one_launch = false, pending = false;
  double *ISR = nullptr, *OLR = nullptr, *fluxes = nullptr;
  double *rows = nullptr;
};

struct Radtran {
  unsigned magic = MAGIC;
  int state = 0;
  int nz = 0, nsp = 0, np = 0, nw = 0, ng = 0;
  std::vector<double> wavl, freq;
  std::vector<KTabHost *> k;
  std::vector<XsHost *> cia, ray, pxs;
  std::vector<PartHost *> part;
  std::vector<int> part_slot;
  bool has_cont = false;
  int LH2O = -1, cont_nT = 0;
  std::vector<double> cont_temp, cont_H2O, cont_foreign;
  DevBuf<double> d_cont_temp, d_cont_H2O, d_cont_foreign;
  std::vector<double> wbin, wbin_e, wxy;
  DevBuf<double> d_wbin, d_wbin_e, d_wbin_e_pad, d_wxy, d_freq, d_rorr_tab;
  ChannelObj ir, sol;
  WrkObj wrk_ir, wrk_sol;
  double diurnal_fac = 0.5;
  std::vector<double> zenith_u, zenith_w, surface_albedo, surface_emissivity, photons_sol;
  bool has_hard_surface = true;
  double ir_tau_min = 1.0e-6;
  double photon_scale_factor = 1.0;
  bool fields_dirty = true;
  DevBuf<double> d_zen_u, d_zen_w, d_zen_iu, d_partial, d_albedo, d_emis, d_photons, d_am_f1, d_am_f2, d_am_dw;
  int nslots = 0;
  std::vector<std::string> species_names, particle_names, particle_data;
  std::string k_method_name = "RandomOverlapResortRebin", continuum_model = "MT_CKD";
  std::vector<SlotDev> slots;
  bool cust_on = false;
  int cust_nP = 0;
  std::vector<double> cust_axis;
  DevBuf<double> d_cust_axis, d_cust_dtau, d_cust_w0, d_cust_g0;
  DevBuf<double> d_bT, d_bTs, d_bup, d_bdn, d_bpartial, d_bout;
  DevBuf<double> d_green, d_green_acc, d_green_in, d_gen_out;
  int green_last_n = -1;
  double *h_bout = nullptr;
  size_t h_bout_n = 0;
  char *h_green = nullptr;
  size_t h_green_n = 0;
  DevBuf<int> d_green_idx;
  int ir_green_mode = 1;
  long ir_green_batches = 0;
  DevBuf<double> d_col;
  size_t meta_ofs = 0;
  int nsrc = 0;
  bool all_pairs_exact = false;
  DevBuf<double> d_prep;
  size_t prep_count = 0;
  std::vector<AbsEntry> abs_entries;
  DevBuf<double> d_zero_xs;
  DevBuf<int> d_err;
#ifdef CLIMA_STAMPS
  DevBuf<long long> d_stamps;
#endif
  double *h_col = nullptr;
  double *h_col_dev = nullptr;
  size_t col_count = 0;
  bool column_has_particles = false;
  bool column_loaded = false;
  hipEvent_t ev_upload = nullptr;
  bool upload_pending = false;
  int call_id = 0, checked_id = 0;
  long upload_id = 0, opr_upload_id = 0;
  std::string deferred_err;
  int fused_max_spins = 400000, checked_timeout = 0, solar_id = 0, fused_fallbacks = 0;
  bool last_cs = true;
  std::vector<double> last_T, last_P, last_radii;
  DevBuf<double> d_opr;
  size_t opr_count = 0;
  DevBuf<double> d_tau, d_w0, d_g, d_tau_band, d_scat;
  bool opr_valid = false;
  DevBuf<double> d_small;
  DevBuf<double> d_flux_n, d_f_total;
  std::vector<std::pair<void *, size_t>> host_registered;
  double *batch_out[3] = {nullptr, nullptr, nullptr};
  size_t batch_out_n = 0;
  int batch_shared_min = 2;
  bool batch_pin_results = false;
  hipEvent_t bout_ev[6] = {nullptr, nullptr, nullptr, nullptr, nullptr, nullptr};
  hipStream_t copy_streams[3] = {nullptr, nullptr, nullptr};
  double *h_small = nullptr;
  double *h_small_dev = nullptr;
  bool small_in_host = false;
  int *h_errflag = nullptr;
  std::vector<double> f_total;
  bool small_valid = false;
  bool w0_valid = true;
  DevBuf<double> d_flux_part;
  int shard_rank = 0, shard_world = 1;
  ncclComm_t comm = nullptr;
  int comm_n = 1, comm_rank = 0, device = 0;
  long comm_reduces = 0;
  double comm_status = 0.0;
  int op_lo = 0, op_n = 0, ir_lo = 0, ir_n = 0, sol_lo = 0, sol_n = 0;
  hipStream_t stream = nullptr;
  DevBuf<double> d_cols_arena, d_flux_arena;
  DevBuf<double> d_prep_arena, d_opr_arena, d_res_arena;
  int batch_cols_in_flight = 64;
  BatchRun dev_batch;
  DevBuf<int> d_batch_nsrc;
  std::vector<int> batch_nsrc;
  hipEvent_t ev_producer = nullptr;
  bool batch_shared = true;
  int rebin_mode = 1;
  long coop_items = 34816;
  bool fused = true;
  bool generic_opacity = false;
  bool ts_block_mode = false;
  int ts_ncols_env = 0;
  DevBuf<int> d_done;
  int profile = 0;
  long timer_calls = 0;
  int profile_stride = 1;
  struct Ev { hipEvent_t a, b; int id; };
  std::vector<Ev> pending;
  std::vector<hipEvent_t> pool;
  double k_ms[4] = {0, 0, 0, 0};
  int k_n[4] = {0, 0, 0, 0};

  ~Radtran() {
    for (auto *x : k) delete x;
    for (auto *x : cia) delete x;
    for (auto *x : ray) delete x;
    for (auto *x : pxs) delete x;
    for (auto *x : part) delete x;
    for (auto &e : pending) { (void)hipEventDestroy(e.a); (void)hipEventDestroy(e.b); }
    for (auto &e : pool) (void)hipEventDestroy(e);
    if (h_col) (void)hipHostFree(h_col);
    for (auto &e : host_registered) (void)hipHostUnregister(e.first);
    for (auto &cs : copy_streams) if (cs) (void)hipStreamDestroy(cs);
    for (auto &e : bout_ev) if (e) (void)hipEventDestroy(e);
    if (h_small) (void)hipHostFree(h_small);
    if (h_bout) (void)hipHostFree(h_bout);
    if (h_green) (void)hipHostFree(h_green);
    if (ev_upload) (void)hipEventDestroy(ev_upload);
    if (ev_producer) (void)hipEventDestroy(ev_producer);
    if (comm) (void)ncclCommDestroy(comm);
    if (stream) (void)hipStreamDestroy(stream);
    magic = 0;
  }
};

Radtran *as_rad(void *ptr) {
  Radtran *r = reinterpret_cast<Radtran *>(ptr);
  if (!r || r->magic != MAGIC) return nullptr;
  return r;
}

bool is_close(double a, double b, double tol) { return std::fabs(a - b) <= std::fabs(tol * std::max(std::fabs(a), std::fabs(b))); }

void gauss_legendre(int n, std::vector<double> &x, std::vector<double> &w) {
  x.assign(n, 0.0);
  w.assign(n, 0.0);
  for (int i = 0; i < n; i++) {
    double z = std::cos(PI * (i + 0.75) / (n + 0.5)), pp = 0.0;
    for (int it = 0; it < 100; it++) {
      double p1 = 1.0, p2 = 0.0;
      for (int j = 0; j < n; j++) {
        double p3 = p2;
        p2 = p1;
        p1 = ((2.0 * j + 1.0) * z * p2 - j * p3) / (j + 1.0);
      }
      pp = n * (z * p1 - p2) / (z * z - 1.0);
      double z1 = z;
      z = z1 - p1 / pp;
      if (std::fabs(z - z1) < 1e-16) break;
    }
    x[n - 1 - i] = z;
    w[n - 1 - i] = 2.0 / ((1.0 - z * z) * pp * pp);
  }
}

int host_bracket(const std::vector<double> &xt, double x) {
  int n = (int)xt.size();
  if (x < xt[0]) return 0;
  if (x >= xt[n - 1]) return n - 2;
  int lo = 0, hi = n - 1;
  while (hi - lo > 1) {
    int mid = (lo + hi) / 2;
    if (x < xt[mid]) hi = mid; else lo = mid;
  }
  return lo;
}

bool make_channel(Radtran *r, ChannelObj &c, int which, int n, const double *wavl, char *err) {
  int ind1 = 0, ind2 = 0;
  double best1 = INFINITY, best2 = INFINITY;
  for (int i = 0; i < r->nw + 1; i++) {
    double d1 = std::fabs(wavl[0] - r->wavl[i]), d2 = std::fabs(wavl[n - 1] - r->wavl[i]);
    if (d1 < best1) { best1 = d1; ind1 = i; }
    if (d2 < best2) { best2 = d2; ind2 = i; }
  }
  const char *msg = "The wavelength bins are not compatible with the k-distribution wavelength bins.";
  if (n != ind2 - ind1 + 1) { set_err(err, msg); return false; }
  for (int i = 0; i < n; i++)
    if (!is_close(wavl[i], r->wavl[ind1 + i], 1.0e-7)) { set_err(err, msg); return false; }
  c.parent = r;
  c.which = which;
  c.nw = n - 1;
  c.wavl.assign(wavl, wavl + n);
  c.freq.resize(n);
  for (int i = 0; i < n; i++) c.freq[i] = C_LIGHT / (wavl[i] * 1.0e-9);
  c.ind_start = ind1;
  c.ind_end = ind2 - 1;
  return true;
}

void upload_fields(Radtran *r) {
  if (!r->fields_dirty) return;
  if (r->stream) HIPCHK(hipStreamSynchronize(r->stream));
  r->d_zen_u.upload(r->zenith_u);
  r->d_zen_w.upload(r->zenith_w);
  {
    std::vector<double> iu(r->zenith_u.size());
    for (size_t i = 0; i < iu.size(); i++) iu[i] = 1.0 / r->zenith_u[i];
    r->d_zen_iu.upload(iu);
  }
  r->d_albedo.upload(r->surface_albedo);
  r->d_emis.upload(r->surface_emissivity);
  r->d_photons.upload(r->photons_sol);
  r->fields_dirty = false;
}

int rebin_mode_for(const std::vector<double> &wbin, const std::vector<double> &wbin_e, const std::vector<double> &wxy) {
  const int multi = (*std::max_element(wxy.begin(), wxy.end()) > *std::min_element(wbin.begin(), wbin.end())) ? 2 : 1;
  if (wbin.size() != 8) return multi;
  if (const char *e = getenv("CLIMA_HIP_REBIN")) { if (std::strcmp(e, "stream") == 0) return multi; }
  std::vector<double> s(wxy);
  std::sort(s.begin(), s.end());
  if (s[0] <= 0.0) return multi;
  double lo[64], hi[64], a = 0.0, b = 0.0;
  for (int j = 0; j < 64; j++) { a += s[j]; b += s[63 - j]; lo[j] = a; hi[j] = b; }
  for (int k = 1; k < 8; k++) {
    const double E = wbin_e[k];
    int jlo = 0, jhi = 0;
    while (jlo < 63 && hi[jlo] < E * (1.0 - 1e-9)) jlo++;
    while (jhi < 63 && lo[jhi] < E * (1.0 + 1e-9)) jhi++;
    if (jlo < RB_WIN_LO[k] || jhi > RB_WIN_HI[k]) return multi;
  }
  double dlo[65], dhi[65];
  for (int n = 0; n <= 64; n++) { dlo[n] = 1e300; dhi[n] = -1.0; }
  double rowcum[8][9];
  for (int i = 0; i < 8; i++) { rowcum[i][0] = 0.0; for (int j = 0; j < 8; j++) rowcum[i][j + 1] = rowcum[i][j] + wbin[i] * wbin[j]; }
  int len[8];
  std::function<void(int, int, int, double)> rec = [&](int i, int maxlen, int size, double wt) {
    if (i == 8) { dlo[size] = std::min(dlo[size], wt); dhi[size] = std::max(dhi[size], wt); return; }
    for (int rl = 0; rl <= maxlen; rl++) { len[i] = rl; rec(i + 1, rl, size + rl, wt + rowcum[i][rl]); }
  };
  rec(0, 8, 0, 0.0);
  for (int k = 1; k < 8; k++) {
    const double E = wbin_e[k];
    int jlo = 0, jhi = 0;
    while (jlo < 63 && dhi[jlo + 1] < E * (1.0 - 1e-9)) jlo++;
    while (jhi < 63 && dlo[jhi + 1] < E * (1.0 + 1e-9)) jhi++;
    if (jlo < RB_TIGHT_LO[k] || jhi > RB_TIGHT_HI[k]) return multi;
  }
  return 0;
}

constexpr double SHARD_W_OP = 3.0, SHARD_W_IR = 1.0, SHARD_W_SOL0 = 0.6, SHARD_W_SOLZ = 0.24;

void compute_shard(Radtran *r) {
  const int nw = r->nw, W = r->shard_world, R = r->shard_rank;
// ... 110 lines not shown
  CallKind kind;
  double *col, *prep;
  int nsrc;
  bool all_pairs_exact;
  OprViews opr;
  SpectraViews spec;
  double *flux_n, *f_total;
  int *done;
  int ncol;
  BatchStrides bs;
  bool host_out;
};

CallBufs resident_bufs(Radtran *r, bool host_out = false) {
  CallBufs b{};
  b.kind = CALL_RESIDENT; b.ncol = 1; b.host_out = host_out;
  b.col = r->d_col.p; b.prep = r->d_prep.p;
  b.nsrc = r->nsrc; b.all_pairs_exact = r->all_pairs_exact;
  b.opr = OprViews{r->d_tau.p, r->d_w0.p, r->d_g.p, r->d_tau_band.p, r->d_scat.p, r->opr_count};
  b.spec = SpectraViews{r->wrk_ir.fup_a.p, r->wrk_ir.fdn_a.p, r->wrk_ir.tau_band.p, r->wrk_sol.fup_a.p,
                        r->wrk_sol.fdn_a.p, r->wrk_sol.amean.p, r->wrk_sol.tau_band.p, 0};
  b.flux_n = r->d_flux_n.p; b.f_total = r->d_f_total.p; b.done = r->d_done.p;
  return b;
}
CallBufs arena_column_bufs(Radtran *r, int c, int nsrc) {
  CallBufs b = resident_bufs(r);
  b.kind = CALL_ARENA_COLUMN; b.nsrc = nsrc; b.all_pairs_exact = false;
  b.col = r->d_cols_arena.p + (size_t)c * r->col_count;
  b.flux_n = r->d_flux_arena.p + (size_t)c * 5 * (r->nz + 1); b.f_total = b.flux_n + 4 * (r->nz + 1);
  return b;
}
CallBufs arena_chunk_bufs(Radtran *r, int c0, int ncol) {
  CallBufs b = resident_bufs(r);
  b.kind = CALL_ARENA_CHUNK; b.ncol = ncol; b.nsrc = r->nz; b.all_pairs_exact = false;
  b.col = r->d_cols_arena.p + (size_t)c0 * r->col_count; b.prep = r->d_prep_arena.p;
  b.opr = opr_views(r, r->d_opr_arena.p); b.spec = spectra_views(r, r->d_res_arena.p);
  b.flux_n = r->d_flux_arena.p + (size_t)c0 * 5 * (r->nz + 1);
  b.bs = BatchStrides{r->col_count, r->prep_count, b.opr.count, b.spec.count, (size_t)5 * (r->nz + 1),
                      (int)(((size_t)r->op_n * r->nz + 255) / 256)};
  return b;
}

ColumnDev column_dev(Radtran *r, const CallBufs &b) {
  ColumnDev c;
  const int nz = r->nz;
  c.T_surface = b.col;
  c.T = b.col + 1;
  c.P = c.T + nz;
  c.dz = c.P + nz;
  c.dens = c.dz + nz;
  c.pdens = c.dens + (size_t)r->nsp * nz;
  c.radii = c.pdens + (size_t)r->np * nz;
  c.meta = reinterpret_cast<const int *>(b.col + r->meta_ofs);
  prep_views(r, b.prep, c);
  c.err_flag = r->d_err.p;
  return c;
}

int build_meta(Radtran *r, const double *T, const double *P, const double *dz, const double *dens,
               const double *pdens, const double *radii, bool has_particles, int *meta) {
#pragma clang fp contract(off)
  const int nz = r->nz, nsp = r->nsp, np = r->np;
  const double tol = 1.0e-12;
  const bool use_radii = has_particles && radii && !r->part.empty();
  int nsrc = 0;
  int *srcl = meta + 1, *src = meta + 1 + nz;
  for (int j = 0; j < nz; j++) {
    bool reuse = false, exact = false;
    if ((nz & 1) == 0 && (j & 1) == 1) {
      reuse = is_close(P[j], P[j - 1], tol) && is_close(T[j], T[j - 1], tol);
      exact = P[j] == P[j - 1] && T[j] == T[j - 1] && dz[j] == dz[j - 1];
      for (int i = 0; i < nsp && reuse; i++) {
        const volatile double ca = dens[(size_t)i * nz + j] * dz[j], cb = dens[(size_t)i * nz + j - 1] * dz[j - 1];
        reuse = is_close(ca, cb, tol);
        exact = exact && dens[(size_t)i * nz + j] == dens[(size_t)i * nz + j - 1];
      }
      if (use_radii)
        for (int i = 0; i < np && reuse; i++) reuse = is_close(radii[(size_t)i * nz + j], radii[(size_t)i * nz + j - 1], tol);
      if (reuse && np > 0 && has_particles && pdens && radii)
        for (int i = 0; i < np; i++)
          exact = exact && pdens[(size_t)i * nz + j] == pdens[(size_t)i * nz + j - 1] &&
                  radii[(size_t)i * nz + j] == radii[(size_t)i * nz + j - 1];
      exact = exact && reuse;
    }
    if (reuse) {
      srcl[nsrc - 1] |= SRC_PAIR | (exact ? SRC_EXACT : 0);
      src[j] = j - 1;
    } else {
      srcl[nsrc++] = j;
      src[j] = j;
    }
  }
  for (int m = nsrc; m < nz; m++) srcl[m] = nz - 1;
  meta[0] = nsrc;
  return nsrc;
}

int pack_column(Radtran *r, double *h, double T_surface, const double *T, const double *P, const double *dz,
                const double *dens, const double *pdens, const double *radii) {
  const size_t nz = r->nz;
  h[0] = T_surface;
  std::memcpy(h + 1, T, sizeof(double) * nz);
  std::memcpy(h + 1 + nz, P, sizeof(double) * nz);
  std::memcpy(h + 1 + 2 * nz, dz, sizeof(double) * nz);
  std::memcpy(h + 1 + 3 * nz, dens, sizeof(double) * nz * r->nsp);
  double *hp = h + 1 + 3 * nz + nz * r->nsp;
  if (r->np > 0 && pdens && radii) {
    std::memcpy(hp, pdens, sizeof(double) * nz * r->np);
    std::memcpy(hp + nz * r->np, radii, sizeof(double) * nz * r->np);
  }
  return build_meta(r, T, P, dz, dens, pdens, radii, pdens && radii, reinterpret_cast<int *>(h + r->meta_ofs));
}

void f_total_row(double *h, int nl) {
  for (int i = 0; i < nl; i++) h[4 * nl + i] = (h[3 * nl + i] - h[2 * nl + i]) + (h[1 * nl + i] - h[0 * nl + i]);
}
void toa_fluxes(const double *h, int nz, double *ISR, double *OLR) {
  const int nl = nz + 1;
  *ISR = (h[3 * nl + nz] - h[2 * nl + nz]);
  *OLR = -(h[1 * nl + nz] - h[0 * nl + nz]);
}

void invalidate_small(Radtran *r) { r->small_valid = false; r->small_in_host = false; }

TwoStreamParams make_twostream_params(Radtran *r, const CallBufs &b, const ColumnDev &col, bool compute_solar) {
  TwoStreamParams ts;
  const int nz = r->nz;
  std::memset(&ts, 0, sizeof(ts));
  ts.nz = nz; ts.ng = r->ng;
  ts.n_sol = compute_solar ? r->sol_n : 0; ts.sol_lo = r->sol_lo;
  ts.n_ir = r->ir_n; ts.ir_lo = r->ir_lo;
  ts.sol_start = r->sol.ind_start; ts.ir_start = r->ir.ind_start;
  ts.tau = b.opr.tau; ts.w0 = b.opr.w0; ts.g = b.opr.g; ts.tau_band = b.opr.tau_band; ts.scat = b.opr.scat;
  ts.wbin = r->d_wbin.p; ts.freq = r->d_freq.p;
  ts.T = col.T; ts.T_surface = col.T_surface;
  ts.emissivity = r->d_emis.p; ts.has_hard_surface = r->has_hard_surface ? 1 : 0; ts.ir_tau_min = r->ir_tau_min;
  ts.nzen = (int)r->zenith_u.size(); ts.zen_u = r->d_zen_u.p; ts.zen_w = r->d_zen_w.p; ts.zen_iu = r->d_zen_iu.p;
  for (int z = 0; z < ts.nzen && z < MAX_ZEN; z++) {
    ts.zen_u_v[z] = r->zenith_u[z]; ts.zen_w_v[z] = r->zenith_w[z]; ts.zen_iu_v[z] = 1.0 / r->zenith_u[z];
  }
  ts.albedo = r->d_albedo.p; ts.photons_sol = r->d_photons.p;
  ts.photon_scale_factor = r->photon_scale_factor; ts.diurnal_fac = r->diurnal_fac;
  ts.am_f1 = r->d_am_f1.p; ts.am_f2 = r->d_am_f2.p; ts.am_dw = r->d_am_dw.p;
  ts.ir_fup_a = b.spec.ir_fup_a; ts.ir_fdn_a = b.spec.ir_fdn_a; ts.ir_tau_band = b.spec.ir_tau_band;
  ts.sol_fup_a = b.spec.sol_fup_a; ts.sol_fdn_a = b.spec.sol_fdn_a; ts.sol_amean = b.spec.sol_amean;
  ts.sol_tau_band = b.spec.sol_tau_band;
  return ts;
}

PrepParams make_prep_params(Radtran *r, const CallBufs &b, const ColumnDev &col, int call_id, const TwoStreamParams *clears) {
  PrepParams pp;
  std::memset(&pp, 0, sizeof(pp));
  pp.ncol = b.ncol; pp.bs = b.bs;
  pp.nz = r->nz; pp.nsp = r->nsp; pp.np = r->np; pp.nslots = r->nslots;
  pp.has_cont = r->has_cont; pp.LH2O = r->LH2O;
  for (int s = 0; s < r->nslots; s++) pp.slots[s] = r->slots[s];
  if (r->cust_on) {
    SlotDev cs;
    cs.axis = r->d_cust_axis.p; cs.n = r->cust_nP; cs.source = -1;
    cs.lo = -std::numeric_limits<double>::infinity(); cs.hi = std::numeric_limits<double>::infinity();
    cs.flag_clamp = 0;
    pp.slots[pp.nslots++] = cs;
  }
  pp.nabs = (int)r->abs_entries.size();
  for (int e = 0; e < pp.nabs; e++) { pp.abs_kind[e] = r->abs_entries[e].kind; pp.abs_a[e] = r->abs_entries[e].a; pp.abs_b[e] = r->abs_entries[e].b; }
  pp.col = col;
  pp.call_id = call_id;
  if (clears) pp.nzero = ts_clear_ranges(*clears, pp.zero_ptr, pp.zero_count);
  return pp;
}

OpacityParams make_opacity_params(Radtran *r, const CallBufs &b, const ColumnDev &col, bool write_w0) {
  OpacityParams op;
  std::memset(&op, 0, sizeof(op));
  op.nz = r->nz; op.nw = r->nw; op.ng = r->ng; op.nsp = r->nsp; op.np = r->np;
  op.bin_lo = r->op_lo; op.nbins = r->op_n; op.nsrc = b.nsrc;
  op.nk = (int)r->k.size(); op.nray = (int)r->ray.size(); op.npart = (int)r->part.size();
  for (size_t i = 0; i < r->k.size(); i++)
    op.k[i] = KDev{r->k[i]->d_log10k.p, r->k[i]->sp, r->k[i]->nP, r->k[i]->nT, (int)(2 * i), (int)(2 * i + 1)};
  for (size_t i = 0; i < r->ray.size(); i++) op.ray[i] = XsDev{r->ray[i]->d_data.p, 0, r->ray[i]->sp1, -1, 0, -1};
  op.nabs = (int)r->abs_entries.size();
  for (int e = 0; e < op.nabs; e++) op.abs[e] = r->abs_entries[e];
  for (size_t i = 0; i < r->part.size(); i++)
    op.part[i] = PartDev{r->part[i]->d_w0.p, r->part[i]->d_qext.p, r->part[i]->d_gt.p, r->part[i]->p_ind, r->part[i]->nrad, r->part_slot[i]};
  op.wbin = r->d_wbin.p; op.wbin_e = r->d_wbin_e.p; op.wxy = r->d_wxy.p; op.wbin_e_pad = r->d_wbin_e_pad.p; op.rorr_tab = r->d_rorr_tab.p;
  op.col = col;
  op.cust = CustomDev{r->d_cust_dtau.p, r->d_cust_w0.p, r->d_cust_g0.p, r->cust_nP, r->nslots, r->cust_on ? 1 : 0};
  op.rebin_mode = r->rebin_mode;
#ifdef CLIMA_STAMPS
  op.stamps = r->d_stamps.p;
#endif
  op.tau = b.opr.tau; op.w0 = b.opr.w0; op.g = b.opr.g; op.tau_band = b.opr.tau_band; op.scat = b.opr.scat;
  op.write_w0 = write_w0 ? 1 : 0;
  return op;
}

IntegrateParams make_integrate_params(Radtran *r, const CallBufs &b, bool compute_solar, bool reduce) {
  IntegrateParams ip;
  std::memset(&ip, 0, sizeof(ip));
  ip.ncol = b.ncol; ip.bs = b.bs;
  ip.nz = r->nz; ip.nw_ir = r->ir.nw; ip.nw_sol = r->sol.nw;
  ip.ir_lo = r->ir_lo; ip.ir_n = r->ir_n; ip.sol_lo = r->sol_lo; ip.sol_n = r->sol_n;
  ip.do_solar = compute_solar ? 1 : 0;
  ip.ir_fup_a = b.spec.ir_fup_a; ip.ir_fdn_a = b.spec.ir_fdn_a;
  ip.sol_fup_a = b.spec.sol_fup_a; ip.sol_fdn_a = b.spec.sol_fdn_a;
  ip.ir_freq = r->ir.d_freq.p; ip.sol_freq = r->sol.d_freq.p;
  ip.flux_n = b.flux_n;
  ip.flux_part = r->shard_world > 1 ? r->d_flux_part.p : nullptr;
  ip.f_total = r->shard_world == 1 ? b.f_total : nullptr;
  ip.nchunk = integrate_chunks(std::max(r->ir_n, r->sol_n));
  ip.partial = r->d_partial.p;
  if (b.host_out && r->h_small_dev && b.kind == CALL_RESIDENT && !reduce && r->shard_world == 1 && integrate_one_launch(ip)) {
    ip.host_out = r->h_small_dev;
    ip.err_words = r->d_err.p;
  }
  if (reduce) {
    ip.f_total = nullptr;
    ip.timeout_out = r->d_small.p + 4 * ((size_t)r->nz + 1); ip.timeout_flag = r->d_err.p + 1;
    ip.id_opr = r->call_id; ip.id_sol = r->solar_id;
  }
  return ip;
}

bool sw_no_half() { static const bool v = [] { const char *e = getenv("CLIMA_HIP_NO_HALF"); return e && e[0] == '1'; }(); return v; }
bool sw_paired() { static const bool v = [] { const char *e = getenv("CLIMA_HIP_PAIRED"); return !(e && e[0] == '0'); }(); return v; }
bool sw_w0_scat() { static const bool v = [] { const char *e = getenv("CLIMA_HIP_W0_SCAT"); return !(e && e[0] == '0'); }(); return v; }

PlanIn plan_input(const Radtran *r, const CallBufs &b, bool compute_solar, bool compute_opacity, bool allow_fused) {
  PlanIn in{};
  in.nz = r->nz; in.ng = r->ng; in.nzen = (int)r->zenith_u.size();
  in.n_ir = r->ir_n; in.n_sol = compute_solar ? r->sol_n : 0; in.op_n = r->op_n;
  in.batch = b.kind == CALL_ARENA_CHUNK; in.ncol = b.ncol;
  in.nsrc = b.nsrc;
  in.rebin_mode = r->rebin_mode; in.cust_on = r->cust_on; in.compute_opacity = compute_opacity;
  in.all_pairs = compute_opacity && b.all_pairs_exact;
  in.fused = r->fused; in.allow_fused = allow_fused; in.generic_opacity = r->generic_opacity;
  in.ts_block_mode = r->ts_block_mode; in.ts_ncols_env = r->ts_ncols_env; in.coop_items = r->coop_items;
  in.no_half = sw_no_half(); in.allow_paired = sw_paired(); in.w0_from_scat = sw_w0_scat();
  return in;
}

void ensure_w0(Radtran *r) {
  if (r->w0_valid) return;
  launch_w0_from_scat(r->d_tau.p, r->d_scat.p, r->d_w0.p, r->nw, r->ng, r->nz, r->stream);
  HIPCHK(hipGetLastError());
  r->w0_valid = true;
}

void enqueue_radiate(Radtran *r, const CallBufs &b, bool compute_solar, bool compute_opacity, bool allow_fused = true) {
  r->timer_calls++;
  upload_fields(r);
  const bool resident = b.kind == CALL_RESIDENT, chunk = b.kind == CALL_ARENA_CHUNK;
  const ColumnDev col = column_dev(r, b);
  TwoStreamParams ts = make_twostream_params(r, b, col, compute_solar);
  const LaunchPlan plan = plan_radiate(plan_input(r, b, compute_solar, compute_opacity, allow_fused));
  bool fused_done = false;
  if (compute_opacity) {
    const int call_id = ++r->call_id;
    const PrepParams pp = make_prep_params(r, b, col, call_id, plan.prep_clears ? &ts : nullptr);
    { KernelTimer t(r, 0); launch_prep(pp, r->stream); HIPCHK(hipGetLastError()); t.stop(); }

    OpacityParams op = make_opacity_params(r, b, col, plan.write_w0);
    if (plan.fused.form != TS_NONE) {
      FusedParams fp;
      std::memset(&fp, 0, sizeof(fp));
      fp.ncol = b.ncol; fp.bs = b.bs;
      fp.call_id = call_id; fp.max_spins = r->fused_max_spins;
      fp.done = b.done; fp.timeout_flag = r->d_err.p + 1;
      KernelTimer t(r, 1);
      fused_done = launch_fused(op, ts, fp, plan.fused, r->stream);
      HIPCHK(hipGetLastError());
      t.stop();
      if (!fused_done) op = make_opacity_params(r, b, col, true);
    }
    if (chunk && !fused_done) throw HipFail{"internal: a one-launch batch needs the fused grid"};
    if (!fused_done) {
      KernelTimer t(r, 1);
      const bool ok = launch_opacity(op, plan, r->stream);
      HIPCHK(hipGetLastError());
      if (!ok)
        throw HipFail{"k-distributions with " + std::to_string(r->ng) + " g-points are not supported (1..32)"};
      t.stop();
    }
    r->opr_valid = true;
    if (!chunk) r->w0_valid = op.write_w0 != 0;
    if (resident) r->opr_upload_id = r->upload_id;
  } else if (!chunk) {
    ensure_w0(r);
  }
  r->last_cs = compute_solar;
  if (compute_solar) r->solar_id = r->call_id;

  if (!fused_done) {
    KernelTimer t(r, 2);
    bool ok = launch_twostream_w(ts, plan.ts, r->stream);
    if (!ok) { HIPCHK(hipGetLastError()); ok = launch_twostream(ts, plan.block, r->stream); }
    HIPCHK(hipGetLastError());
    if (!ok)
      throw HipFail{"nz*ngauss = " + std::to_string(r->nz * r->ng) + " exceeds what the two-stream kernels can stage"};
    t.stop();
  }

  const bool reduce = r->comm && resident;
  const IntegrateParams ip = make_integrate_params(r, b, compute_solar, reduce);
  r->small_in_host = ip.host_out != nullptr;
  { KernelTimer t(r, 3); launch_integrate(ip, r->stream); HIPCHK(hipGetLastError()); t.stop(); }
  if (reduce) {
    NCCLCHK(ncclAllReduce(r->d_small.p, r->d_small.p, 4 * ((size_t)r->nz + 1) + 1, ncclDouble, ncclSum, r->comm, r->stream));
    r->comm_reduces++;
  }
  r->small_valid = false;
}

bool recover_fused_timeout(Radtran *r);
void settle_device_batch(Radtran *r);

void fetch_small(Radtran *r) {
  settle_device_batch(r);
  if (r->small_valid) return;
  const int nl = r->nz + 1;
  for (int pass = 0; pass < 2; pass++) {
    if (!r->small_in_host)
      HIPCHK(hipMemcpyAsync(r->h_small, r->d_small.p, sizeof(double) * (5 * nl + 1), hipMemcpyDeviceToHost, r->stream));
    HIPCHK(hipStreamSynchronize(r->stream));
    resolve_events(r);
    if (r->comm) r->comm_status = r->h_small[4 * nl];
    if (!r->column_loaded || !recover_fused_timeout(r)) break;
  }
  f_total_row(r->h_small, nl);
  r->small_valid = true;
}

bool check_dims(Radtran *r, int dim_T, int dim_P, int d1, int d2, int dim_dz, int has_p, int p1, int p2,
                int r1, int r2, const double *pdens, const double *radii, char *err) {
  if (has_p && ((pdens && !radii) || (radii && !pdens))) { set_err(err, "Both pdensities and radii must be arguments."); return false; }
  if (r->np > 0 && (!has_p || !radii)) { set_err(err, "The model contains particles but \"pdensities\" and \"radii\" are not arguments."); return false; }
  if (dim_T != r->nz) { set_err(err, "\"T\" has the wrong input dimension."); return false; }
  if (dim_P != r->nz) { set_err(err, "\"P\" has the wrong input dimension."); return false; }
  if (d1 != r->nz || d2 != r->nsp) { set_err(err, "\"densities\" has the wrong input dimension."); return false; }
  if (dim_dz != r->nz) { set_err(err, "\"dz\" has the wrong input dimension."); return false; }
  if (has_p && radii) {
    if (p1 != r->nz || p2 != r->np) { set_err(err, "\"pdensities\" has the wrong input dimension."); return false; }
    if (r1 != r->nz || r2 != r->np) { set_err(err, "\"radii\" has the wrong input dimension."); return false; }
  }
  return true;
}

void do_upload(Radtran *r, double T_surface, const double *T, const double *P, const double *dens,
               const double *dz, const double *pdens, const double *radii) {
  const int nz = r->nz;
  double *h = r->h_col;
  settle_device_batch(r);
  if (r->upload_pending) { HIPCHK(hipEventSynchronize(r->ev_upload)); r->upload_pending = false; }
  r->nsrc = pack_column(r, h, T_surface, T, P, dz, dens, pdens, radii);
  r->column_has_particles = (pdens && radii);
  r->upload_id++;
  const int *meta = reinterpret_cast<const int *>(h + r->meta_ofs);
  bool all = (nz % 2 == 0) && r->nsrc * 2 == nz;
  for (int m = 0; m < r->nsrc && all; m++) all = (meta[1 + m] & SRC_EXACT) != 0;
  r->all_pairs_exact = all;
  {
    static const bool kcopy = [] { const char *e = getenv("CLIMA_HIP_COPY_KERNEL"); return !(e && e[0] == '0'); }();
    if (kcopy && r->h_col_dev) launch_copy(r->d_col.p, r->h_col_dev, r->col_count, r->stream);
    else HIPCHK(hipMemcpyAsync(r->d_col.p, h, sizeof(double) * r->col_count, hipMemcpyHostToDevice, r->stream));
  }
  HIPCHK(hipEventRecord(r->ev_upload, r->stream));
  r->upload_pending = true;
  r->last_T.assign(T, T + nz);
  r->last_P.assign(P, P + nz);
  if (r->np > 0 && radii) r->last_radii.assign(radii, radii + (size_t)nz * r->np); else r->last_radii.clear();
  r->column_loaded = true;
}

const char *const REPLACED_MSG = "The fused opacity/two-stream hand-off of an earlier opacity pass timed out and the column has "
                                 "been replaced since: repeat the steps from that opacity pass on.";
bool recover_fused_timeout(Radtran *r) {
  if (r->comm) {
    const double st = r->comm_status;
    if (!(st > 0.0)) return false;
    r->comm_status = 0.0;
    r->checked_timeout = r->call_id;
    if (std::fmod(st, 1024.0) > 0.0 && r->upload_id != r->opr_upload_id) throw HipFail{REPLACED_MSG};
    r->fused_fallbacks++;
    enqueue_radiate(r, resident_bufs(r), st >= 1024.0 || r->last_cs, true, false);
    return true;
  }
  const int t = r->h_errflag[1];
  if (t <= r->checked_timeout) return false;
  r->checked_timeout = r->call_id;
  const bool stale_opr = t == r->call_id, stale_sol = t == r->solar_id;
  if (!stale_opr && !stale_sol) return false;
  if (r->shard_world > 1)
    throw HipFail{"The fused opacity/two-stream hand-off timed out on a bin-sharded handle whose all-reduce is the caller's; "
                  "repeat the step (radtran_fused_set(0) selects the separate launches; with radtran_comm_init_rank the "
                  "library repeats it itself)."};
  if (stale_opr && r->upload_id != r->opr_upload_id) throw HipFail{REPLACED_MSG};
  r->fused_fallbacks++;
  enqueue_radiate(r, resident_bufs(r), stale_sol || r->last_cs, true, false);
  return true;
}

constexpr const char *OPACITY_FAILED_MSG = "Opacity computation failed in one or more wavelength bins.";
bool surface_device_error(Radtran *r, char *err) {
  const bool failed = *r->h_errflag > r->checked_id;
  r->checked_id = r->call_id;
  if (failed) set_err(err, OPACITY_FAILED_MSG);
  return failed;
}

void wait_error_words(Radtran *r) {
  HIPCHK(hipMemcpyAsync(r->h_errflag, r->d_err.p, 2 * sizeof(int), hipMemcpyDeviceToHost, r->stream));
  HIPCHK(hipStreamSynchronize(r->stream));
  resolve_events(r);
}

void settle(Radtran *r) {
  settle_device_batch(r);
  for (int pass = 0; pass < 2; pass++) {
    if (r->comm && !r->small_valid)
      HIPCHK(hipMemcpyAsync(&r->comm_status, r->d_small.p + 4 * (r->nz + 1), sizeof(double), hipMemcpyDeviceToHost, r->stream));
    wait_error_words(r);
    if (!r->column_loaded || !recover_fused_timeout(r)) break;
  }
}

void defer_err(Radtran *r, const std::string &msg) {
  if (r && r->deferred_err.empty()) r->deferred_err = msg;
// ... 237 lines not shown
      while (hi - lo > 1) { const int mid = (lo + hi) / 2; if (xv < x[mid]) hi = mid; else lo = mid; }
      const double slope = (y[lo + 1] - y[lo]) / (x[lo + 1] - x[lo]);
      yg[i] = y[lo] + slope * (xv - x[lo]);
    }
  }
  return 0;
}

void radtran_set_custom_optical_properties(void *ptr, const int *dim_wv, const double *wv, const int *dim_P,
                                           const double *P, const int *dim1_dtau_dz, const int *dim2_dtau_dz,
                                           const double *dtau_dz, const int *dim1_w0, const int *dim2_w0,
                                           const double *w0, const int *dim1_g0, const int *dim2_g0,
                                           const double *g0, char *err) {
  clear_err(err);
  GUARD(r, ptr, err);
  if (r->state != 2) { set_err(err, "Radtran is not constructed"); return; }
  const int nwv = *dim_wv, nP = *dim_P;
  for (int i = 0; i < nwv; i++) if (wv[i] <= 0.0) { set_err(err, "All elements of `wv` must be larger than zero"); return; }
  for (int i = 0; i < nP; i++) if (P[i] <= 0.0) { set_err(err, "All elements of `P` must be larger than zero"); return; }
  if (nP != *dim1_dtau_dz) { set_err(err, "`P` and `dtau_dz` have incompatible shapes"); return; }
  if (nwv != *dim2_dtau_dz) { set_err(err, "`wv` and `dtau_dz` have incompatible shapes"); return; }
  if (nP != *dim1_w0) { set_err(err, "`P` and `w0` have incompatible shapes"); return; }
  if (nwv != *dim2_w0) { set_err(err, "`wv` and `w0` have incompatible shapes"); return; }
  if (nP != *dim1_g0) { set_err(err, "`P` and `g0` have incompatible shapes"); return; }
  if (nwv != *dim2_g0) { set_err(err, "`wv` and `g0` have incompatible shapes"); return; }
  TRY
  const int nw = r->nw;
  std::vector<double> wv1(nw), row(nwv), tmp(nw);
  for (int i = 0; i < nw; i++) wv1[i] = 0.5 * (r->wavl[i + 1] + r->wavl[i]);
  std::vector<double> tab[3];
  const double *src[3] = {dtau_dz, w0, g0};
  for (auto &t : tab) t.assign((size_t)nw * nP, 0.0);
  for (int i = 0; i < nP; i++) {
    const int j = nP - 1 - i;
    for (int a = 0; a < 3; a++) {
      for (int k = 0; k < nwv; k++) row[k] = src[a][i + (size_t)k * nP];
      if (futils_interp(wv1, nwv, wv, row.data(), tmp.data()) != 0) {
        set_err(err, "Interpolation error in `set_custom_optical_properties`");
        return;
      }
      for (int l = 0; l < nw; l++) tab[a][(size_t)l * nP + j] = tmp[l];
    }
  }
  std::vector<double> lp(nP);
  for (int i = 0; i < nP; i++) lp[nP - 1 - i] = std::log10(P[i]);
  bool ok = nP >= 2;
  for (int i = 1; i < nP && ok; i++) ok = lp[i] > lp[i - 1];
  if (!ok) { set_err(err, "Interpolation initialization error in `set_custom_optical_properties`"); return; }
  HIPCHK(hipStreamSynchronize(r->stream));
  r->cust_axis = lp; r->cust_nP = nP;
  r->d_cust_axis.upload(lp); r->d_cust_dtau.upload(tab[0]); r->d_cust_w0.upload(tab[1]); r->d_cust_g0.upload(tab[2]);
  r->cust_on = true;
  CATCH(err)
}

static std::vector<std::string> split_lines(const char *s) {
  std::vector<std::string> out;
  if (!s) return out;
  std::string cur;
  for (const char *c = s; *c; c++) {
    if (*c == '\n') { out.push_back(cur); cur.clear(); } else cur.push_back(*c);
  }
  if (!cur.empty()) out.push_back(cur);
  return out;
}

void radtran_set_names(void *ptr, const char *species_names, const char *particle_names, char *err) {
  clear_err(err);
  GUARD(r, ptr, err);
  auto sp = split_lines(species_names), pa = split_lines(particle_names);
  if (r->state >= 1 && ((int)sp.size() != r->nsp || (int)pa.size() != r->np)) {
    set_err(err, "radtran_set_names: the number of names does not match the number of species / particles");
    return;
  }
  r->species_names = sp; r->particle_names = pa;
}

void radtran_set_opacity_labels(void *ptr, const char *k_method, const char *water_continuum_model,
                                const char *particle_data, char *err) {
  clear_err(err);
  GUARD(r, ptr, err);
  if (k_method && k_method[0]) r->k_method_name = k_method;
  if (water_continuum_model && water_continuum_model[0]) r->continuum_model = water_continuum_model;
  r->particle_data = split_lines(particle_data);
}

static std::string opacities2yaml(Radtran *r) {
  auto sp = [&](int i) { return (i >= 0 && i < (int)r->species_names.size()) ? r->species_names[i] : ("species" + std::to_string(i + 1)); };
  auto join = [](const std::vector<std::string> &v) {
    std::string o;
    for (size_t i = 0; i < v.size(); i++) { o += v[i]; if (i + 1 != v.size()) o += ", "; }
    return o;
  };
  std::string out = "  k-method: " + r->k_method_name;
  out += "\n  opacities:";
  if (!r->k.empty()) {
    std::vector<std::string> v;
    for (auto *k : r->k) v.push_back(sp(k->sp));
    out += "\n    k-distributions: [" + join(v) + "]";
  }
  if (!r->cia.empty()) {
    std::vector<std::string> v;
    for (auto *x : r->cia) v.push_back(sp(x->sp1) + "-" + sp(x->sp2));
    out += "\n    CIA: [" + join(v) + "]";
  }
  if (!r->ray.empty()) {
    std::vector<std::string> v;
    for (auto *x : r->ray) v.push_back(sp(x->sp1));
    out += "\n    rayleigh: [" + join(v) + "]";
  }
  if (!r->pxs.empty()) {
    std::vector<std::string> v;
    for (auto *x : r->pxs) v.push_back(sp(x->sp1));
    out += "\n    photolysis-xs: [" + join(v) + "]";
  }
  if (r->has_cont) out += "\n    water-continuum: " + r->continuum_model;
  if (!r->part.empty()) {
    std::vector<std::string> v;
    for (size_t i = 0; i < r->part.size(); i++) {
      const int pi = r->part[i]->p_ind;
      const std::string name = (pi >= 0 && pi < (int)r->particle_names.size()) ? r->particle_names[pi] : ("particle" + std::to_string(pi + 1));
      const std::string dat = i < r->particle_data.size() ? r->particle_data[i] : std::string("unknown");
      v.push_back("{name: " + name + ", data: " + dat + "}");
    }
    out += "\n    particle-xs: [" + join(v) + "]";
  }
  return out;
}

void radtran_opacities2yaml_wrapper_1(void *ptr, int *out_len, void **out_cp) {
  Radtran *r = as_rad(ptr);
  const std::string s = r ? opacities2yaml(r) : std::string();
  char *buf = (char *)std::malloc(s.size() + 1);
  std::memcpy(buf, s.c_str(), s.size() + 1);
  *out_len = (int)s.size();
  *out_cp = buf;
}
void radtran_opacities2yaml_wrapper_2(void *ptr, void **out_cp, const int *out_len, char *out_c) {
  (void)ptr;
  if (!out_cp || !*out_cp) return;
  std::memcpy(out_c, *out_cp, (size_t)*out_len + 1);
  std::free(*out_cp);
  *out_cp = nullptr;
}

void radtran_fused_set(void *ptr, const int *enable) {
  Radtran *r = as_rad(ptr);
  if (r) r->fused = (*enable != 0);
}
void radtran_fused_get(void *ptr, int *enabled) {
  Radtran *r = as_rad(ptr);
  *enabled = (r && r->fused) ? 1 : 0;
}
void radtran_coop_items_set(void *ptr, const int *items) {
  Radtran *r = as_rad(ptr);
  if (r) r->coop_items = *items;
}
void radtran_coop_items_get(void *ptr, int *items) {
  Radtran *r = as_rad(ptr);
  *items = r ? (int)std::min<long>(r->coop_items, 2147483647L) : 0;
}
void radtran_fused_spins_set(void *ptr, const int *spins) {
  Radtran *r = as_rad(ptr);
  if (r) r->fused_max_spins = std::max(0, *spins);
}
void radtran_fused_spins_get(void *ptr, int *spins) {
  Radtran *r = as_rad(ptr);
  *spins = r ? r->fused_max_spins : 0;
}
void radtran_ir_green_set(void *ptr, const int *mode) {
  Radtran *r = as_rad(ptr);
  if (r) r->ir_green_mode = std::max(0, std::min(2, *mode));
}
void radtran_ir_green_get(void *ptr, int *mode, int *batches) {
  Radtran *r = as_rad(ptr);
  *mode = r ? r->ir_green_mode : 0;
  *batches = r ? (int)std::min<long>(r->ir_green_batches, 2147483647L) : 0;
}
void radtran_fused_fallbacks_get(void *ptr, int *count) {
  Radtran *r = as_rad(ptr);
  *count = r ? r->fused_fallbacks : 0;
}

void radtran_unset_custom_optical_properties(void *ptr) {
  Radtran *r = as_rad(ptr);
  if (r) r->cust_on = false;
}

void radtran_create_end(void *ptr, const int *num_zenith_angles, const double *surface_albedo, char *err) {
  clear_err(err);
  GUARD(r, ptr, err);
  if (r->state != 1) { set_err(err, "radtran_create_end: create_begin has not been called"); return; }
  if (r->k.empty()) { set_err(err, "There are no k-distributions, yet there must be some to compute total opacity."); return; }
  if (r->ir.nw == 0 || r->sol.nw == 0) { set_err(err, "wavelength channels are not set"); return; }
  if (*num_zenith_angles < 1) { set_err(err, "number of zenith angles must be >= 1"); return; }
  TRY
  const int nz = r->nz, nw = r->nw;
  std::vector<double> x, w;
  gauss_legendre(*num_zenith_angles, x, w);
  r->zenith_u.resize(*num_zenith_angles);
  r->zenith_w.resize(*num_zenith_angles);
  for (int i = 0; i < *num_zenith_angles; i++) {
    double mu = x[i] / 2.0 + 1.0 / 2.0;
    double ang = std::acos(mu) * 180.0 / PI;
    r->zenith_w[i] = w[i] / 2.0;
    r->zenith_u[i] = std::cos(ang * PI / 180.0);
  }
  r->surface_albedo.assign(r->sol.nw, *surface_albedo);
  r->surface_emissivity.assign(r->ir.nw, 1.0);
  if (r->photons_sol.empty()) r->photons_sol.assign(r->sol.nw, 0.0);

  int dev_count = 0;
  HIPCHK(hipGetDeviceCount(&dev_count));
  if (dev_count < 1) throw HipFail{"no HIP device available: the Radtran hot path has no CPU fallback"};
  HIPCHK(hipGetDevice(&r->device));
  HIPCHK(hipStreamCreateWithFlags(&r->stream, hipStreamNonBlocking));
  HIPCHK(hipEventCreateWithFlags(&r->ev_upload, hipEventDisableTiming));
  if (const char *f = getenv("CLIMA_HIP_FUSED")) r->fused = atoi(f) != 0;
  if (const char *f = getenv("CLIMA_HIP_GENERIC")) r->generic_opacity = atoi(f) != 0;
  if (const char *f = getenv("CLIMA_HIP_TS_MODE")) r->ts_block_mode = std::strcmp(f, "block") == 0;
  if (const char *f = getenv("CLIMA_HIP_TS_NCOLS")) r->ts_ncols_env = atoi(f);
  if (const char *f = getenv("CLIMA_HIP_BATCH_SHARED")) r->batch_shared = atoi(f) != 0;
  if (const char *f = getenv("CLIMA_HIP_IR_GREEN")) r->ir_green_mode = std::max(0, std::min(2, atoi(f)));
  if (const char *f = getenv("CLIMA_HIP_BATCH_SHARED_MIN")) r->batch_shared_min = std::max(0, atoi(f));
  if (const char *f = getenv("CLIMA_HIP_FUSED_SPINS")) r->fused_max_spins = std::max(0, atoi(f));

  r->slots.clear();
  auto add_slot = [&](const double *axis_dev, const std::vector<double> &axis, int source, bool flag) {
    SlotDev s;
    s.axis = axis_dev; s.n = (int)axis.size(); s.source = source;
    s.lo = *std::min_element(axis.begin(), axis.end());
    s.hi = *std::max_element(axis.begin(), axis.end());
    s.flag_clamp = flag ? 1 : 0;
    r->slots.push_back(s);
  };
  for (auto *k : r->k) {
    k->d_log10k.upload(k->log10k); k->d_log10P.upload(k->log10P); k->d_temp.upload(k->temp);
    add_slot(k->d_log10P.p, k->log10P, 0, false);
    add_slot(k->d_temp.p, k->temp, 1, false);
  }
  r->abs_entries.clear();
  for (auto *v : {&r->cia, &r->pxs})
    for (auto *xs : *v) {
      xs->d_data.upload(xs->data);
      AbsEntry e;
      e.data = xs->d_data.p; e.nT = xs->dim ? xs->nT : 0; e.slot = 0;
      e.kind = (v == &r->cia) ? ABS_CIA : ABS_COLUMN; e.a = xs->sp1; e.b = xs->sp2 < 0 ? 0 : xs->sp2;
      if (xs->dim) { xs->d_temp.upload(xs->temp); e.slot = (int)r->slots.size(); add_slot(xs->d_temp.p, xs->temp, 1, false); }
      r->abs_entries.push_back(e);
    }
  for (auto *xs : r->ray) xs->d_data.upload(xs->data);
  if (r->has_cont) {
    r->d_cont_temp.upload(r->cont_temp); r->d_cont_H2O.upload(r->cont_H2O); r->d_cont_foreign.upload(r->cont_foreign);
    const int slot = (int)r->slots.size();
    add_slot(r->d_cont_temp.p, r->cont_temp, 1, false);
    r->abs_entries.push_back(AbsEntry{r->d_cont_H2O.p, r->cont_nT, slot, ABS_H2O_SELF, r->LH2O, 0});
    r->abs_entries.push_back(AbsEntry{r->d_cont_foreign.p, r->cont_nT, slot, ABS_H2O_FOREIGN, r->LH2O, 0});
  }
  if ((int)r->abs_entries.size() > MAX_ABS - (ABS_BATCH - 2)) throw HipFail{"too many continuum terms for this build"};
  if (r->abs_entries.size() % ABS_BATCH) {
    r->d_zero_xs.upload(std::vector<double>((size_t)r->nw + 1, 0.0));
    while (r->abs_entries.size() % ABS_BATCH) r->abs_entries.push_back(AbsEntry{r->d_zero_xs.p, 0, 0, ABS_ZERO, 0, 0});
  }
  r->part_slot.clear();
  for (auto *p : r->part) {
    p->d_radii.upload(p->radii); p->d_w0.upload(p->w0); p->d_qext.upload(p->qext); p->d_gt.upload(p->gt);
    r->part_slot.push_back((int)r->slots.size());
    add_slot(p->d_radii.p, p->radii, 2 + p->p_ind, true);
  }
  r->nslots = (int)r->slots.size();
  if (r->nslots + 1 > MAX_SLOTS) throw HipFail{"too many interpolated tables for this build"};
  r->d_wbin.upload(r->wbin); r->d_wbin_e.upload(r->wbin_e); r->d_wxy.upload(r->wxy);
  {
    std::vector<double> pad = r->wbin_e;
    for (int i = 0; i < 4; i++) pad.push_back(INFINITY);
    r->d_wbin_e_pad.upload(pad);
    std::vector<double> tab(24, 0.0);
    if (r->ng == 8)
      for (int k = 0; k < 8; k++) {
        tab[k] = r->wbin_e[k + 1];
        tab[8 + k] = r->wbin[k];
        tab[16 + k] = 1.0 / (r->wbin_e[k + 1] - r->wbin_e[k]);
      }
    r->d_rorr_tab.upload(tab);
  }
  r->d_freq.upload(r->freq);
  r->ir.d_freq.upload(r->ir.freq); r->sol.d_freq.upload(r->sol.freq);
  std::vector<double> f1(r->sol.nw), f2(r->sol.nw), dw(r->sol.nw);
  for (int l = 0; l < r->sol.nw; l++) {
    double avg_freq = 0.5 * (r->sol.freq[l] + r->sol.freq[l + 1]);
    double avg_wavl = 1.0e9 * C_LIGHT / avg_freq;
    f1[l] = (avg_freq / avg_wavl);
    f2[l] = (avg_wavl / (PLANK * C_LIGHT * 1.0e16));
    dw[l] = (r->sol.wavl[l + 1] - r->sol.wavl[l]);
  }
  r->d_am_f1.upload(f1); r->d_am_f2.upload(f2); r->d_am_dw.upload(dw);

  r->meta_ofs = 1 + (size_t)3 * nz + (size_t)nz * r->nsp + (size_t)2 * nz * r->np;
  r->col_count = r->meta_ofs + (size_t)nz + 1;
  r->d_col.alloc(r->col_count);
  r->d_col.zero();
  HIPCHK(hipHostMalloc((void **)&r->h_col, sizeof(double) * r->col_count, hipHostMallocMapped));
  std::memset(r->h_col, 0, sizeof(double) * r->col_count);
  if (hipHostGetDevicePointer((void **)&r->h_col_dev, r->h_col, 0) != hipSuccess) { r->h_col_dev = nullptr; (void)hipGetLastError(); }
  r->prep_count = prep_block_count(r);
  r->d_prep.alloc(r->prep_count); r->d_prep.zero();
  r->d_done.alloc(((size_t)nw * nz + 255) / 256 + 1); r->d_done.zero();
  if (const char *f = getenv("CLIMA_HIP_BATCH_COLS")) r->batch_cols_in_flight = std::max(1, atoi(f));
  if (const char *f = getenv("CLIMA_HIP_COOP_ITEMS")) r->coop_items = atol(f);
#ifdef CLIMA_STAMPS
  r->d_stamps.alloc(64 + 2 * 8192); r->d_stamps.zero();
#endif
  r->opr_count = opr_views(r, nullptr).count;
  r->d_opr.alloc(r->opr_count); r->d_opr.zero();
  const OprViews o = opr_views(r, r->d_opr.p);
  r->d_tau.view(o.tau, o.w0 - o.tau); r->d_w0.view(o.w0, o.g - o.w0); r->d_g.view(o.g, o.tau_band - o.g);
  r->d_tau_band.view(o.tau_band, o.scat - o.tau_band); r->d_scat.view(o.scat, o.tau + o.count - o.scat);
  auto mk = [&](WrkObj &wk, int which, int nwc) {
    wk.parent = r; wk.which = which;
    wk.fup_a.alloc((size_t)(nz + 1) * nwc); wk.fdn_a.alloc((size_t)(nz + 1) * nwc);
    wk.amean.alloc((size_t)(nz + 1) * nwc); wk.tau_band.alloc((size_t)nz * nwc);
    wk.fup_a.zero(); wk.fdn_a.zero(); wk.amean.zero(); wk.tau_band.zero();
  };
  mk(r->wrk_ir, 0, r->ir.nw);
  mk(r->wrk_sol, 1, r->sol.nw);
  r->d_small.alloc((size_t)5 * (nz + 1) + 1); r->d_small.zero();
  r->d_flux_n.view(r->d_small.p, (size_t)4 * (nz + 1));
  r->d_err.view(reinterpret_cast<int *>(r->d_small.p + (size_t)5 * (nz + 1)), 2);
  r->d_partial.alloc((size_t)4 * integrate_chunks(std::max(r->ir.nw, r->sol.nw)) * (nz + 1)); r->d_partial.zero();
  r->d_f_total.view(r->d_small.p + (size_t)4 * (nz + 1), nz + 1);
  HIPCHK(hipHostMalloc((void **)&r->h_small, sizeof(double) * (5 * (nz + 1) + 1), hipHostMallocMapped));
  std::memset(r->h_small, 0, sizeof(double) * (5 * (nz + 1) + 1));
  {
    static const bool direct = [] { const char *e = getenv("CLIMA_HIP_HOST_OUT"); return !(e && e[0] == '0'); }();
    if (!direct || hipHostGetDevicePointer((void **)&r->h_small_dev, r->h_small, 0) != hipSuccess) { r->h_small_dev = nullptr; (void)hipGetLastError(); }
  }
  r->h_errflag = reinterpret_cast<int *>(r->h_small + 5 * (nz + 1));
  r->f_total.assign(nz + 1, 0.0);
  HIPCHK(hipDeviceSynchronize());
  r->fields_dirty = true;
  compute_shard(r);
  r->small_valid = true;
  r->state = 2;
  CATCH(err)
}

void radtran_upload_column(void *ptr, const double *T_surface, const double *T, const double *P,
                           const double *densities, const double *dz, const double *pdensities,
                           const double *radii, char *err) {
  clear_err(err);
  GUARD(r, ptr, err);
  if (r->state != 2) { set_err(err, "Radtran is not constructed"); return; }
  if (r->np > 0 && (!pdensities || !radii)) { set_err(err, "The model contains particles but \"pdensities\" and \"radii\" are not arguments."); return; }
  TRY
  do_upload(r, *T_surface, T, P, densities, dz, pdensities, radii);
  CATCH(err)
}

void radtran_radiate_resident(void *ptr, const int *compute_solar, const int *compute_opacity, char *err) {
  clear_err(err);
  GUARD(r, ptr, err);
  if (r->state != 2) { set_err(err, "Radtran is not constructed"); return; }
  if (!r->column_loaded) { set_err(err, "no column has been uploaded"); return; }
  TRY
  enqueue_radiate(r, resident_bufs(r), *compute_solar != 0, *compute_opacity != 0);
  CATCH(err)
}

static void ir_batch_general(Radtran *r, const double *d_T, const double *d_Ts, int n, double *d_out, size_t out_arr) {
  const int nz = r->nz, nl = nz + 1, nw_ir = r->ir.nw;
  const int CH = std::min(n, 512);
// ... 1472 lines not shown
```

### clima_amd/csrc/radtran_dev.h

```cpp
#pragma once

#include <hip/hip_runtime.h>

namespace clima {

constexpr int RB_WIN_LO[8] = {0, 1, 5, 10, 18, 27, 39, 52};
constexpr int RB_WIN_HI[8] = {0, 11, 24, 36, 45, 53, 58, 62};
constexpr int RB_TIGHT_LO[8] = {0, 5, 12, 19, 27, 35, 45, 55};
constexpr int RB_TIGHT_HI[8] = {0, 8, 18, 28, 36, 44, 51, 58};

constexpr int MAX_K = 8;
constexpr int MAX_XS = 16;
constexpr int MAX_PART = 4;
constexpr int MAX_ZEN = 16;
constexpr int MAX_SLOTS = 2 * MAX_K + 2 * MAX_XS + 1 + MAX_PART + 1;

constexpr double PLANK = 6.62607004e-34;
constexpr double C_LIGHT = 299792458.0;
constexpr double K_BOLTZ_SI = 1.380649e-23;
constexpr double PI = 3.14159265358979323846e0;
constexpr double SIGMA_SI = 5.670374419e-8;
constexpr double MAX_W0 = 0.99999;
constexpr double MAX_GT = 0.999999;
constexpr double TAU_MIN = 1.0e-20;
constexpr double LN10 = 2.302585092994045684017991454684364207601;
constexpr double TINY = 2.2250738585072014e-308;

struct XsDev {
  const double *data;
  int dim, sp1, sp2, nT, slot;
};

constexpr int ABS_BATCH = 8;
constexpr int MAX_ABS = 2 * 16 + 2 + 6;
enum { ABS_CIA = 0, ABS_COLUMN = 1, ABS_H2O_SELF = 2, ABS_H2O_FOREIGN = 3, ABS_ZERO = 4 };
struct AbsEntry {
  const double *data;
  int nT;
  int slot;
  int kind, a, b;
};

struct KDev {
  const double *log10k;
  int sp, nP, nT, slotP, slotT;
};

struct PartDev {
  const double *w0, *qext, *gt;
  int p_ind, nrad, slot;
};

struct SlotDev {
  const double *axis;
  int n;
  int source;
  double lo, hi;
  int flag_clamp;
};

constexpr int SRC_PAIR = 1 << 30;
constexpr int SRC_EXACT = 1 << 29;
constexpr int SRC_LAYER = 0xffff;

struct BatchStrides {
  size_t col, prep, opr, res, flux;
  int done;
};

struct ColumnDev {
  const double *T, *P, *dz, *dens, *pdens, *radii;
  const int *meta;
  double *log10P, *cols, *foreign_col;
  double *absw;
  int *ix;
  double *q;
  int *err_flag;
  const double *T_surface;
};

struct CustomDev {
  const double *dtau, *w0, *g0;
  int nP, slot, on;
};

struct OpacityParams {
  int nz, nw, ng, nsp, np;
  int bin_lo, nbins;
  int nsrc;
  int coop, generic;
  int nk, nray, npart;
  KDev k[MAX_K];
  XsDev ray[MAX_XS];
  int nabs;
  AbsEntry abs[MAX_ABS];
  PartDev part[MAX_PART];
  const double *wbin, *wbin_e, *wxy;
  const double *wbin_e_pad;
  const double *rorr_tab;
  ColumnDev col;
  double *tau, *w0, *g, *tau_band;
  double *scat;
  int write_w0;
  long long *stamps;
  int rebin_mode;
  CustomDev cust;
};

struct PrepParams {
  int ncol;
  BatchStrides bs;
  int nz, nsp, np, nslots, has_cont, LH2O;
  int call_id;
  SlotDev slots[MAX_SLOTS];
  int nabs;
  int abs_kind[MAX_ABS], abs_a[MAX_ABS], abs_b[MAX_ABS];
  int nzero;
  double *zero_ptr[6];
  size_t zero_count[6];
  ColumnDev col;
};

struct TwoStreamParams {
  int nz, ng;
  int ncols, nchunks, nc_shift;
  int col_base, accumulate;
  int b_ncol, b_T, b_Ts;
  size_t b_out;
  int n_sol, sol_lo, n_ir, ir_lo;
  int sol_start, ir_start;
  const double *tau, *w0, *g, *tau_band;
  const double *scat;
  int w0_from_scat;
  const double *wbin;
  const double *freq;
  const double *bplanck;
  int force_slots;
  int paired;
  const double *T, *T_surface;
  const double *emissivity;
  int has_hard_surface;
  double ir_tau_min;
  int nzen;
  const double *zen_u, *zen_w, *zen_iu;
  double zen_u_v[MAX_ZEN], zen_w_v[MAX_ZEN], zen_iu_v[MAX_ZEN];
  const double *albedo;
  const double *photons_sol;
  double photon_scale_factor, diurnal_fac;
  const double *am_f1, *am_f2, *am_dw;
  double *ir_fup_a, *ir_fdn_a, *ir_tau_band;
  double *sol_fup_a, *sol_fdn_a, *sol_amean, *sol_tau_band;
};

struct FusedParams {
  int ncol;
  int n_op;
  int n_ts;
  int call_id;
  int max_spins;
  int *done;
  int *timeout_flag;
  int slots;
  int sol_early;
  BatchStrides bs;
};

struct IntegrateParams {
  int ncol;
  BatchStrides bs;
  int nz;
  int nw_ir, nw_sol;
  int ir_lo, ir_n, sol_lo, sol_n;
  int do_solar;
  const double *ir_fup_a, *ir_fdn_a, *sol_fup_a, *sol_fdn_a;
  const double *ir_freq, *sol_freq;
  double *flux_n;
  double *flux_part;
  double *f_total;
  double *partial;
  int nchunk;
  double *timeout_out;
  const int *timeout_flag;
  int id_opr, id_sol;
  double *host_out;
  const int *err_words;
};

struct BatchIntegrateParams {
  int nz, ir_lo, ir_n, nchunk, col0;
  const double *fup_a, *fdn_a;
  size_t spec_stride;
  const double *freq;
  double *partial;
  const double *flux_n;
  double *out;
  size_t out_arr;
};

struct PackParams {
  int ncol, nz, nsp, np;
  int has_particles;
  int use_radii;
  size_t col_count, meta_ofs;
  const double *T_surface, *T, *P, *dz, *dens, *pdens, *radii;
  double *blocks;
  int *nsrc;
};
struct BatchFinishParams {
  int ncol, nz;
  double *flux;
  double *ISR, *OLR, *fluxes;
};
void launch_pack_columns(const PackParams &p, hipStream_t s);
void launch_batch_finish(const BatchFinishParams &p, hipStream_t s);

constexpr int GREEN_LB = 16;
__host__ __device__ inline int green_class(int lv, int k, int &slot) {
  slot = 0;
  if (lv >= k + 2) return 1;
  if (lv == 0 && k <= 1) { slot = 2; return 2; }
  if (lv <= k - 1) return 0;
  slot = lv - k;
  return 2;
}
__host__ __device__ inline int green_block_class(int k, int blk, int nz) {
  const int lv0 = blk * GREEN_LB, lv1 = lv0 + GREEN_LB - 1 < nz ? lv0 + GREEN_LB - 1 : nz;
  if (k >= 2 && lv1 <= k - 1) return 0;
  if (lv0 >= k + 2) return 1;
  return 2;
}

struct GreenParams {
  int nz, ng, n_ir, ir_lo, ir_start, NQ;
  const double *tau, *w0, *g, *wbin;
  const double *freq, *ir_freq;
  const double *emissivity;
  int has_hard_surface;
  double ir_tau_min;
  double *RW;
  double *IS;
  double *FS;
  double *DS;
  double *D0;
  int ndev, ndev_pad;
  const int *dev_k;
  const double *dev_T, *base_T;
  double *DB;
  int qsplit;
  int nmix;
  const int *mix_dev, *mix_blk;
  double *partial;
  int msplit;
  double *partial_m;
  const int *col_src, *col_ptr, *col_dev;
  const double *gen_out;
  size_t gen_arr, out_arr;
  const double *flux_n;
  double *out;
};
void launch_green_factor(const GreenParams &p, hipStream_t s);
void launch_green_columns(const GreenParams &p, int ncol, hipStream_t s);
void launch_batch_ftotal(double *out, size_t out_arr, int ncol, int nz, const double *flux_n, hipStream_t s);
void launch_green_accumulate(const GreenParams &p, hipStream_t s);
void launch_green_jacobian(const GreenParams &p, hipStream_t s);
void launch_green_jacobian_reduced(const GreenParams &p, const int *row_lv, int nrow, int ngroup, bool parts, hipStream_t s);
void launch_jacobian_total(double *jac, size_t arr, size_t n, hipStream_t s);
int green_far_resident_waves();
void green_vector_form_set(int vector_form);
int green_far_waves(int ndev, int nl);
int green_far_splits(int n_ir, int waves);

struct PlanIn {
  int nz, ng, nzen;
  int n_ir, n_sol, op_n;
  int nsrc;
  int ncol;
  bool batch;
  bool ir_batch;
  int rebin_mode;
  bool cust_on, compute_opacity;
  bool all_pairs;
  bool fused, allow_fused, generic_opacity, ts_block_mode, no_half, allow_paired, w0_from_scat;
  long coop_items;
  int ts_ncols_env;
  int force_slots;
};
enum { OP_NONE = 0, OP_TILE, OP_COOP, OP_GENERIC, OP_UNSUPPORTED };
enum { TS_NONE = 0, TS_WAVE, TS_HALF, TS_PAIRED, TS_BLOCK };
struct TsPlan {
  int form;
  int slots;
  int cols;
  int groups, per_launch;
  int threads;
  size_t lds;
  bool zero_launch;
};
struct LaunchPlan {
  int opacity, coop_ng;
  TsPlan fused;
  TsPlan ts;
  TsPlan block;
  bool prep_clears;
  bool caller_clears;
  bool write_w0;
};
LaunchPlan plan_radiate(const PlanIn &in);
int ts_clear_ranges(const TwoStreamParams &p, double *ptr[6], size_t count[6]);

void launch_prep(const PrepParams &p, hipStream_t s);
bool launch_opacity(const OpacityParams &p, const LaunchPlan &pl, hipStream_t s);
bool launch_twostream(TwoStreamParams &p, const TsPlan &t, hipStream_t s);
bool launch_twostream_w(TwoStreamParams &p, const TsPlan &t, hipStream_t s);
bool launch_twostream_ir_batch(TwoStreamParams &p, int ncol, hipStream_t s, int force_nw = 0);
int fused_tiles(const OpacityParams &op);
bool launch_fused(const OpacityParams &op, TwoStreamParams ts, FusedParams fp, const TsPlan &f, hipStream_t s);
bool launch_fused_twostream_only(TwoStreamParams &ts, int slots, const int *meta_nsrc, hipStream_t s, bool half = false, bool paired = false);
void launch_integrate(const IntegrateParams &p, hipStream_t s);
bool integrate_one_launch(const IntegrateParams &p);
void launch_integrate_batch(const BatchIntegrateParams &p, int ncol, hipStream_t s);
int integrate_chunks(int nbins);
void launch_f_total(int nz, const double *flux_n, double *f_total, hipStream_t s);
void launch_scale(double *a, size_t n, double f, hipStream_t s);
void launch_copy(double *dst, const double *src, size_t n, hipStream_t s);
void launch_test_rcp(const double *x, double *y, int n, hipStream_t s);
void launch_test_wscan(const double *a, const double *b, double *out, int nwaves, hipStream_t s);
void launch_w0_from_scat(const double *tau, const double *scat, double *w0, int nw, int ng, int nz, hipStream_t s);
void launch_test_exp(const double *x, double *y, int n, hipStream_t s);
void launch_test_exp_tab(const double *x, double *y, int n, int base10, hipStream_t s);

}
```

### clima_amd/lib.py

```python
import ctypes as C
import os

_HERE = os.path.dirname(os.path.abspath(__file__))
LIB_PATH = os.environ.get("CLIMA_HIP_LIB") or os.path.join(_HERE, "csrc", "libclima_radtran_hip.so")
ERR_LEN = 1024

_dp = C.POINTER(C.c_double)
_ip = C.POINTER(C.c_int)
_bp = C.POINTER(C.c_bool)
_vp = C.c_void_p
_vpp = C.POINTER(C.c_void_p)
_err = C.c_char_p

SIGNATURES = {
    "allocate_radtran": [_vpp],
    "deallocate_radtran": [_vp],
    "radtran_create_begin": [_vp, _ip, _ip, _ip, _ip, _dp, _err],
    "radtran_add_ktable": [_vp, _ip, _ip, _dp, _ip, _dp, _ip, _dp, _dp, _err],
    "radtran_add_xsection": [_vp, _ip, _ip, _ip, _ip, _ip, _dp, _dp, _err],
    "radtran_set_water_continuum": [_vp, _ip, _ip, _dp, _dp, _dp, _err],
    "radtran_add_particle": [_vp, _ip, _ip, _dp, _dp, _dp, _dp, _err],
    "radtran_set_channels": [_vp, _ip, _dp, _ip, _dp, _err],
    "radtran_set_photons_sol": [_vp, _ip, _dp, _err],
    "radtran_create_end": [_vp, _ip, _dp, _err],
    "radtran_radiate_wrapper": [_vp, _dp, _ip, _dp, _ip, _dp, _ip, _ip, _dp, _ip, _dp, _ip, _ip, _ip, _dp, _ip, _ip,
                                _dp, _ip, _ip, _err],
    "radtran_toa_fluxes_wrapper": [_vp, _dp, _ip, _dp, _ip, _dp, _ip, _ip, _dp, _ip, _dp, _ip, _ip, _ip, _dp, _ip, _ip,
                                   _dp, _ip, _ip, _dp, _dp, _err],
    "radtran_apply_radiation_enhancement": [_vp, _dp],
    "radtran_set_custom_optical_properties": [_vp, _ip, _dp, _ip, _dp, _ip, _ip, _dp, _ip, _ip, _dp, _ip, _ip, _dp, _err],
    "radtran_unset_custom_optical_properties": [_vp],
    "radtran_opacities2yaml_wrapper_1": [_vp, _ip, _vpp],
    "radtran_opacities2yaml_wrapper_2": [_vp, _vpp, _ip, _err],
    "radtran_set_names": [_vp, _err, _err, _err],
    "radtran_set_opacity_labels": [_vp, _err, _err, _err, _err],
    "radtran_fused_set": [_vp, _ip],
    "radtran_fused_get": [_vp, _ip],
    "radtran_fused_fallbacks_get": [_vp, _ip],
    "radtran_ir_green_set": [_vp, _ip],
    "radtran_ir_green_get": [_vp, _ip, _ip],
    "radtran_coop_items_set": [_vp, _ip],
    "radtran_coop_items_get": [_vp, _ip],
    "radtran_fused_spins_set": [_vp, _ip],
    "radtran_fused_spins_get": [_vp, _ip],
    "radtran_spectra_get_all": [_vp, _bp, _ip, _ip, _ip, _dp, _dp, _dp, _dp, _dp, _dp, _dp, _err],
    "radtran_spectra_release": [_vp],
    "radtran_create_from_files": [_vp, C.c_char_p, C.c_char_p, _ip, _dp, _ip, C.c_char_p, _err],
    "radtran_load_from_files": [_vp, C.c_char_p, C.c_char_p, _ip, C.c_char_p, _err],
    "clima_test_host_tables_digest": [_vp, C.POINTER(C.c_ulonglong)],
    "radtran_dims_get": [_vp, _ip, _ip, _ip, _ip, _ip],
    "radtran_names_get": [_vp, _ip, C.c_char_p, C.c_char_p],
    "radtran_toa_fluxes_batch": [_vp, _ip, _dp, _dp, _dp, _dp, _dp, _ip, _dp, _dp, _dp, _dp, _dp, _err],
    "radtran_toa_fluxes_batch_device": [_vp, _ip, _vp, _vp, _vp, _vp, _vp, _ip, _vp, _vp, _vp, _vp, _vp, _vp, _err],
    "clima_test_pack_columns": [_vp, _ip, _dp, _dp, _dp, _dp, _dp, _ip, _dp, _dp, _dp, _ip, _err],
    "clima_test_pack_columns_host": [_vp, _ip, _dp, _dp, _dp, _dp, _dp, _ip, _dp, _dp, _dp, _ip, _err],
    "radtran_radiate_ir_batch": [_vp, _ip, _dp, _ip, _ip, _dp, _dp, _dp, _dp, _err],
    "radtran_ir_jacobian": [_vp, _dp, _ip, _dp, _ip, _ip, _dp, _dp, _dp, _err],
    "radtran_ir_jacobian_reduced": [_vp, _dp, _ip, _dp, _ip, _ip, _ip, _ip, _ip, _ip, _ip, _dp, _dp, _dp, _err],
    "radtran_upload_column": [_vp, _dp, _dp, _dp, _dp, _dp, _dp, _dp, _err],
    "radtran_radiate_resident": [_vp, _ip, _ip, _err],
    "radtran_synchronize": [_vp, _err],
    "radtran_flux_device_ptr": [_vp, _vpp, _ip],
    "radtran_set_bin_shard": [_vp, _ip, _ip, _err],
    "radtran_bin_shard_get": [_vp, _ip, _ip, _ip, _ip, _ip, _ip],
    "radtran_finish_reduced": [_vp, _err],
    "radtran_set_device": [_ip, _err],
    "radtran_comm_unique_id": [_err, _err],
    "radtran_comm_init_rank": [_vp, _ip, _ip, _err, _err],
    "radtran_comm_init_file": [_vp, _ip, _ip, _err, _err],
    "radtran_comm_get": [_vp, _ip, _ip, _ip],
    "radtran_comm_destroy": [_vp],
    "radtran_stream_get": [_vp, _vpp],
    "radtran_profile_set": [_vp, _ip],
    "radtran_kernel_time_get": [_vp, _ip, _dp, _ip, _err],
    "radtran_profile_reset": [_vp],
    "radtran_profile_stride_set": [_vp, _ip],
    "radtran_algorithmic_bytes": [_vp, _dp, _dp, _dp, _dp, _err],
    "radtran_algorithmic_nodes": [_vp, _dp, _dp, _dp, _dp, _err],
    "radtran_opr_get": [_vp, _dp, _dp, _dp, _dp, _err],
    "clima_bench_toa_fluxes": [_vp, _ip, _dp, _ip, _dp, _ip, _dp, _ip, _ip, _dp, _ip, _dp, _ip, _ip, _ip, _dp, _ip, _ip,
                               _dp, _dp, _dp, _dp, _err],
    "clima_bench_resident_sync": [_vp, _ip, _dp, _err],
    "clima_bench_resident_graph": [_vp, _ip, _ip, _dp, _err],
    "clima_test_device_exp": [_ip, _dp, _dp, _err],
    "clima_test_device_exp_table": [_ip, _ip, _dp, _dp, _err],
    "clima_test_device_rcp": [_ip, _dp, _dp, _err],
    "clima_test_wave_scan": [_ip, _dp, _dp, _dp, _err],
    "clima_test_two_stream": [_ip, _ip, _ip, _ip, _dp, _dp, _dp, _dp, _dp, _dp, _dp, _dp, _dp, _dp, _dp, _dp, _err],
    "clima_test_green_far_form_set": [_ip],
    "radtran_batch_pin_results_set": [_vp, _ip],
    "radtran_batch_pin_results_get": [_vp, _ip],
    "clima_test_ir_response": [_ip, _ip, _dp, _dp, _dp, _dp, _dp, _ip, _ip, _dp, _dp, _dp, _err],
    "radtran_set_bolometric_flux_wrapper": [_vp, _dp],
    "radtran_bolometric_flux_wrapper": [_vp, _dp],
    "radtran_skin_temperature_wrapper": [_vp, _dp, _dp],
    "radtran_equilibrium_temperature_wrapper": [_vp, _dp, _dp],
    "radtran_zenith_u_get_size": [_vp, _ip],
    "radtran_zenith_u_get": [_vp, _ip, _dp],
    "radtran_zenith_u_set": [_vp, _ip, _dp],
    "radtran_zenith_weights_get": [_vp, _ip, _dp],
    "radtran_zenith_weights_set": [_vp, _ip, _dp],
    "radtran_surface_albedo_get_size": [_vp, _ip],
    "radtran_surface_albedo_get": [_vp, _ip, _dp],
    "radtran_surface_albedo_set": [_vp, _ip, _dp],
    "radtran_surface_emissivity_get_size": [_vp, _ip],
    "radtran_surface_emissivity_get": [_vp, _ip, _dp],
    "radtran_surface_emissivity_set": [_vp, _ip, _dp],
    "radtran_has_hard_surface_get": [_vp, _bp],
    "radtran_has_hard_surface_set": [_vp, _bp],
    "radtran_photon_scale_factor_get": [_vp, _dp],
    "radtran_photon_scale_factor_set": [_vp, _dp],
    "radtran_ir_tau_min_get": [_vp, _dp],
    "radtran_ir_tau_min_set": [_vp, _dp],
    "radtran_diurnal_fac_get": [_vp, _dp],
    "radtran_diurnal_fac_set": [_vp, _dp],
    "radtran_ir_get": [_vp, _vpp],
    "radtran_sol_get": [_vp, _vpp],
    "radtran_wrk_ir_get": [_vp, _vpp],
    "radtran_wrk_sol_get": [_vp, _vpp],
    "radtran_f_total_get_size": [_vp, _ip],
    "radtran_f_total_get": [_vp, _ip, _dp],
    "radtran_photons_sol_get_size": [_vp, _ip],
    "radtran_photons_sol_get": [_vp, _ip, _dp],
    "climaradtranwrk_fup_a_get_size": [_vp, _ip, _ip],
    "climaradtranwrk_fup_a_get": [_vp, _ip, _ip, _dp],
    "climaradtranwrk_fdn_a_get_size": [_vp, _ip, _ip],
    "climaradtranwrk_fdn_a_get": [_vp, _ip, _ip, _dp],
    "climaradtranwrk_fup_n_get_size": [_vp, _ip],
    "climaradtranwrk_fup_n_get": [_vp, _ip, _dp],
    "climaradtranwrk_fdn_n_get_size": [_vp, _ip],
    "climaradtranwrk_fdn_n_get": [_vp, _ip, _dp],
    "climaradtranwrk_amean_get_size": [_vp, _ip, _ip],
    "climaradtranwrk_amean_get": [_vp, _ip, _ip, _dp],
    "climaradtranwrk_tau_band_get_size": [_vp, _ip, _ip],
    "climaradtranwrk_tau_band_get": [_vp, _ip, _ip, _dp],
    "rtchannel_wavl_get_size": [_vp, _ip],
    "rtchannel_wavl_get": [_vp, _ip, _dp],
    "rtchannel_freq_get_size": [_vp, _ip],
    "rtchannel_freq_get": [_vp, _ip, _dp],
}

_lib = None


def load():
    global _lib
    if _lib is None:
        if not os.path.exists(LIB_PATH):
            raise ImportError(
                "clima_amd: HIP extension %s is missing. Build it with "
                "`python -m clima_amd.build` (hipcc, gfx950); there is no CPU fallback." % LIB_PATH)
        try:
            import torch
        except ImportError:
            pass
        L = C.CDLL(LIB_PATH)
        for name, argtypes in SIGNATURES.items():
            fn = getattr(L, name)
            fn.argtypes = argtypes
            fn.restype = None
        _lib = L
    return _lib
```

### clima_amd/radtran.py

```python
import ctypes as C
import os

import numpy as np

from . import lib as _lib

_dp = C.POINTER(C.c_double)


class ClimaException(Exception):
    """clima/cython/_clima.pyx: raised with the Fortran `err` text."""


def _d(a):
    return a.ctypes.data_as(_dp)


def _i(v):
    return C.byref(C.c_int(int(v)))


def _f(v):
    return C.byref(C.c_double(float(v)))

# ... 282 lines not shown
            if not t.is_contiguous():
                raise ClimaException('toa_fluxes_batch_device: "%s" is not C-contiguous' % name)
        dev = next((t.device for _, t, _ in want if t.is_cuda), torch.device("cuda", torch.cuda.current_device()))
        isr, olr = torch.empty(n, dtype=torch.float64, device=dev), torch.empty(n, dtype=torch.float64, device=dev)
        fl = torch.empty((n, 5, nz + 1), dtype=torch.float64, device=dev) if return_fluxes else None

        def addr(t):
            return t.data_ptr() if t is not None else None

        cur = torch.cuda.current_stream(dev)
        mine = torch.cuda.ExternalStream(self.stream(), device=dev)
        producer = cur.cuda_stream
        if not producer:
            mine.wait_stream(cur)
        self._L.radtran_toa_fluxes_batch_device(self._ptr, _i(n), addr(T_surface), addr(T), addr(P), addr(densities), addr(dz),
                                                _i(1 if hp else 0), addr(pdensities) if hp else None,
                                                addr(radii) if hp else None, addr(isr), addr(olr), addr(fl), producer or None,
                                                self._err)
        self._check()
        if sync:
            self.synchronize()
        else:
            ev = torch.cuda.Event()
            ev.record(mine)
            cur.wait_event(ev)
        return (isr, olr, fl) if return_fluxes else (isr, olr)

    def radiate_ir_batch(self, T_surface, T, out=None, pin=False):
        T = np.asfortranarray(T, dtype=np.float64)
        Ts = _c(np.atleast_1d(T_surface))
        if T.ndim != 2 or T.shape[0] != self.nz or T.shape[1] != len(Ts):
            raise ClimaException('"T" has the wrong input dimension.')
        n = T.shape[1]
        pin = bool(pin) and out is not None
        if out is None:
            out = [np.empty((self.nz + 1, n), order="F") for _ in range(3)]
        self._L.radtran_batch_pin_results_set(self._ptr, _i(1 if pin else 0))
        self._locked = getattr(self, "_locked", [])
        if pin and not any(out is o for o in self._locked):
            self._locked.append(out)
        self._L.radtran_radiate_ir_batch(self._ptr, _i(n), _d(Ts), _i(T.shape[0]), _i(n), _d(T),
                                         _d(out[0]), _d(out[1]), _d(out[2]), self._err)
        self._check()
        return tuple(out)

    def ir_jacobian(self, T_surface, T):
        T, Ts = _c(np.atleast_1d(T)), _c(np.atleast_1d(T_surface))
        if T.ndim != 1 or Ts.shape != (1,):
            raise ClimaException('"T" has the wrong input dimension.')
        nl = self.nz + 1
        out = [np.empty((nl, nl), order="F") for _ in range(3)]
        self._L.radtran_ir_jacobian(self._ptr, _d(Ts), _i(len(T)), _d(T), _i(nl), _i(nl),
                                    _d(out[0]), _d(out[1]), _d(out[2]), self._err)
        self._check()
        return tuple(out)

    def ir_jacobian_reduced(self, T_surface, T, group_of_x, rows=None, parts=False):
        T, Ts = _c(np.atleast_1d(T)), _c(np.atleast_1d(T_surface))
        if T.ndim != 1 or Ts.shape != (1,):
            raise ClimaException('"T" has the wrong input dimension.')
        grp = np.ascontiguousarray(np.atleast_1d(group_of_x), dtype=np.int32)
        rows = np.arange(1, self.nz + 2) if rows is None else rows
        rows = np.ascontiguousarray(np.atleast_1d(rows), dtype=np.int32)
        if grp.ndim != 1:
            raise ClimaException('ir_jacobian_reduced: "group_of_x" has the wrong dimension (%d axes, one expected)' % grp.ndim)
        if rows.ndim != 1:
            raise ClimaException('ir_jacobian_reduced: "rows" has the wrong dimension (%d axes, one expected)' % rows.ndim)
        ngroup, nrow = int(grp.max()) if grp.size else 0, len(rows)
        out = [np.empty((nrow, max(ngroup, 0)), order="F") if (parts or i == 2) else None for i in range(3)]
        ip = C.POINTER(C.c_int)
        self._L.radtran_ir_jacobian_reduced(self._ptr, _d(Ts), _i(len(T)), _d(T), _i(len(grp)), grp.ctypes.data_as(ip),
                                            _i(ngroup), _i(nrow), rows.ctypes.data_as(ip), _i(nrow), _i(ngroup),
                                            _d(out[0]) if parts else None, _d(out[1]) if parts else None, _d(out[2]),
                                            self._err)
        self._check()
        return tuple(out) if parts else out[2]

    def upload_column(self, T_surface, T, P, densities, dz, pdensities=None, radii=None):
        T, P, dz, densities = _c(T), _c(P), _c(dz), _fo(densities)
        if len(T) != self.nz or len(P) != self.nz or len(dz) != self.nz or densities.shape != (self.nz, self.ng):
            raise ClimaException('"densities" has the wrong input dimension.')
        pd = ra = None
        if pdensities is not None:
            pdensities, radii = _fo(pdensities), _fo(radii)
            pd, ra = _d(pdensities), _d(radii)
        self._L.radtran_upload_column(self._ptr, _f(T_surface), _d(T), _d(P), _d(densities), _d(dz), pd, ra, self._err)
        self._check()

    def radiate_resident(self, compute_solar=True, compute_opacity=True):
        self._L.radtran_radiate_resident(self._ptr, _i(compute_solar), _i(compute_opacity), self._err)
        self._check()

    def synchronize(self):
        self._L.radtran_synchronize(self._ptr, self._err)
        self._check()

    def set_bin_shard(self, rank, world):
        self._L.radtran_set_bin_shard(self._ptr, _i(rank), _i(world), self._err)
        self._check()

    COMM_ID_BYTES = 128

    @staticmethod
    def set_device(device):
        L = _lib.load()
        err = C.create_string_buffer(_lib.ERR_LEN + 1)
        L.radtran_set_device(_i(device), err)
        if err.value:
            raise ClimaException(err.value.decode())

    @staticmethod
    def comm_unique_id():
        L = _lib.load()
        err = C.create_string_buffer(_lib.ERR_LEN + 1)
        buf = C.create_string_buffer(Radtran.COMM_ID_BYTES)
        L.radtran_comm_unique_id(buf, err)
        if err.value:
            raise ClimaException(err.value.decode())
        return buf.raw

    def comm_init_rank(self, nranks, rank, comm_id):
        assert len(comm_id) == self.COMM_ID_BYTES
        self._L.radtran_comm_init_rank(self._ptr, _i(nranks), _i(rank), C.create_string_buffer(bytes(comm_id), self.COMM_ID_BYTES), self._err)
        self._check()

    def comm_init_file(self, nranks, rank, path):
        self._L.radtran_comm_init_file(self._ptr, _i(nranks), _i(rank), os.fsencode(path), self._err)
        self._check()

    def comm(self):
        n, r, k = C.c_int(0), C.c_int(0), C.c_int(0)
        self._L.radtran_comm_get(self._ptr, C.byref(n), C.byref(r), C.byref(k))
        return n.value, r.value, k.value

    def comm_destroy(self):
        self._L.radtran_comm_destroy(self._ptr)

    def bin_shard(self):
        v = [C.c_int() for _ in range(6)]
        self._L.radtran_bin_shard_get(self._ptr, *[C.byref(x) for x in v])
        return tuple(x.value for x in v)

    @property
    def fused(self):
        v = C.c_int()
        self._L.radtran_fused_get(self._ptr, C.byref(v))
        return bool(v.value)

    @fused.setter
    def fused(self, on):
        self._L.radtran_fused_set(self._ptr, _i(1 if on else 0))

    @property
    def coop_items(self):
        v = C.c_int()
        self._L.radtran_coop_items_get(self._ptr, C.byref(v))
        return v.value

    @coop_items.setter
    def coop_items(self, n):
        self._L.radtran_coop_items_set(self._ptr, _i(int(n)))

    def spectra_all(self, do_solar=True, out=None):
        nl, ni, ns = self.nz + 1, len(self.ir.freq) - 1, len(self.sol.freq) - 1
        if out is None:
            out = {"ir_fup_a": np.zeros((nl, ni), order="F"), "ir_fdn_a": np.zeros((nl, ni), order="F"),
                   "ir_tau_band": np.zeros((nl - 1, ni), order="F"), "sol_fup_a": np.zeros((nl, ns), order="F"),
                   "sol_fdn_a": np.zeros((nl, ns), order="F"), "sol_amean": np.zeros((nl, ns), order="F"),
                   "sol_tau_band": np.zeros((nl - 1, ns), order="F")}
        err = C.create_string_buffer(1025)
        names = ("ir_fup_a", "ir_fdn_a", "ir_tau_band", "sol_fup_a", "sol_fdn_a", "sol_amean", "sol_tau_band")
        self._L.radtran_spectra_get_all(self._ptr, C.byref(C.c_bool(bool(do_solar))), _i(nl), _i(ni), _i(ns),
                                        *[out[k].ctypes.data_as(C.POINTER(C.c_double)) for k in names], err)
        if err.value:
            raise ClimaException(err.value.decode())
        self._locked = getattr(self, "_locked", [])
        if not any(o is out for o in self._locked):
            self._locked.append(out)
        return out

    def spectra_release(self):
        self._L.radtran_spectra_release(self._ptr)
        self._locked = []

    @property
    def fused_spins(self):
        v = C.c_int()
        self._L.radtran_fused_spins_get(self._ptr, C.byref(v))
        return v.value

    @fused_spins.setter
    def fused_spins(self, n):
        self._L.radtran_fused_spins_set(self._ptr, _i(int(n)))

    @property
    def ir_green(self):
        m, b = C.c_int(), C.c_int()
        self._L.radtran_ir_green_get(self._ptr, C.byref(m), C.byref(b))
        return m.value

    @ir_green.setter
    def ir_green(self, mode):
        self._L.radtran_ir_green_set(self._ptr, _i(int(mode)))

    @property
    def ir_green_batches(self):
        m, b = C.c_int(), C.c_int()
        self._L.radtran_ir_green_get(self._ptr, C.byref(m), C.byref(b))
        return b.value

    @property
    def fused_fallbacks(self):
        v = C.c_int()
        self._L.radtran_fused_fallbacks_get(self._ptr, C.byref(v))
        return v.value

    def flux_tensor(self):
        import torch
        ptr, n = self.flux_device_ptr()

        class _Alias:
            __cuda_array_interface__ = {"shape": (n,), "typestr": "<f8", "data": (ptr, False), "version": 2}

        return torch.as_tensor(_Alias(), device="cuda")

    def finish_reduced(self):
        self._L.radtran_finish_reduced(self._ptr, self._err)
        self._check()

    def flux_device_ptr(self):
        p, n = C.c_void_p(), C.c_int()
        self._L.radtran_flux_device_ptr(self._ptr, C.byref(p), C.byref(n))
        return p.value, n.value

    def stream(self):
        p = C.c_void_p()
        self._L.radtran_stream_get(self._ptr, C.byref(p))
        return p.value

    def profile(self, enable=True):
        self._L.radtran_profile_set(self._ptr, _i(2 if enable == 2 and enable is not True else (1 if enable else 0)))

    def profile_stride(self, stride):
        self._L.radtran_profile_stride_set(self._ptr, _i(int(stride)))

    def profile_reset(self):
        self._L.radtran_profile_reset(self._ptr)

    def kernel_time(self, kernel_id):
        ms, n = C.c_double(), C.c_int()
        self._L.radtran_kernel_time_get(self._ptr, _i(kernel_id), C.byref(ms), C.byref(n), self._err)
        self._check()
        return ms.value, n.value

    def algorithmic_bytes(self):
        a, b, c, d = C.c_double(), C.c_double(), C.c_double(), C.c_double()
        self._L.radtran_algorithmic_bytes(self._ptr, C.byref(a), C.byref(b), C.byref(c), C.byref(d), self._err)
        self._check()
        return dict(tables_distinct=a.value, input=b.value, output=c.value, tables_full=d.value)

    def algorithmic_nodes(self):
        v = [C.c_double() for _ in range(4)]
        self._L.radtran_algorithmic_nodes(self._ptr, *[C.byref(x) for x in v], self._err)
        self._check()
        return dict(N_PT=v[0].value, N_PT_full=v[1].value, N_T=v[2].value, N_T_full=v[3].value)

    def opr(self):
        nz, ng, nw = self.nz, self.ngauss, self.nw
        tau = np.empty((nz, ng, nw), order="F")
        w0 = np.empty((nz, ng, nw), order="F")
        g = np.empty((nz, nw), order="F")
        tb = np.empty((nz, nw), order="F")
        self._L.radtran_opr_get(self._ptr, _d(tau), _d(w0), _d(g), _d(tb), self._err)
        self._check()
        return tau, w0, g, tb

    def set_bolometric_flux(self, flux):
        self._L.radtran_set_bolometric_flux_wrapper(self._ptr, _f(flux))

    def bolometric_flux(self):
        v = C.c_double()
        self._L.radtran_bolometric_flux_wrapper(self._ptr, C.byref(v))
        return v.value

    def skin_temperature(self, bond_albedo):
        v = C.c_double()
        self._L.radtran_skin_temperature_wrapper(self._ptr, _f(bond_albedo), C.byref(v))
        return v.value

    def equilibrium_temperature(self, bond_albedo):
        v = C.c_double()
        self._L.radtran_equilibrium_temperature_wrapper(self._ptr, _f(bond_albedo), C.byref(v))
        return v.value

    def _vec_get(self, name, size_name=None):
        n = C.c_int()
        getattr(self._L, "radtran_%s_get_size" % (size_name or name))(self._ptr, C.byref(n))
        arr = np.empty(n.value, np.double)
        getattr(self._L, "radtran_%s_get" % name)(self._ptr, C.byref(n), _d(arr))
        return arr

    def _vec_set(self, name, arr, size_name=None):
        arr = _c(arr)
        n = C.c_int()
        getattr(self._L, "radtran_%s_get_size" % (size_name or name))(self._ptr, C.byref(n))
        if arr.ndim != 1 or arr.shape[0] != n.value:
# ... 44 lines not shown
```

### include/clima_radtran_hip.h

```cpp
#ifndef CLIMA_RADTRAN_HIP_H
#define CLIMA_RADTRAN_HIP_H

#ifndef __cplusplus
#include <stdbool.h>
#endif

#ifdef __cplusplus
extern "C" {
#endif

#define CLIMA_ERR_LEN 1024

#define CLIMA_XS_CIA 0
#define CLIMA_XS_RAYLEIGH 1
#define CLIMA_XS_ABSORPTION 2
#define CLIMA_XS_PHOTOLYSIS 3


void allocate_radtran(void **ptr);
void deallocate_radtran(void *ptr);

void radtran_create_begin(void *ptr, const int *nz, const int *nsp, const int *np,
                          const int *nw, const double *wavl, char *err);
void radtran_add_ktable(void *ptr, const int *sp_ind, const int *ngauss,
                        const double *weights, const int *npress, const double *log10P,
                        const int *ntemp, const double *temp, const double *log10k,
                        char *err);
void radtran_add_xsection(void *ptr, const int *xs_type, const int *dim, const int *sp_ind1,
                          const int *sp_ind2, const int *ntemp, const double *temp,
                          const double *data, char *err);
void radtran_set_water_continuum(void *ptr, const int *LH2O, const int *ntemp,
                                 const double *temp, const double *log10_xs_H2O,
                                 const double *log10_xs_foreign, char *err);
void radtran_add_particle(void *ptr, const int *p_ind, const int *nrad, const double *radii,
                          const double *w0, const double *qext, const double *gt, char *err);
void radtran_set_channels(void *ptr, const int *n_ir_edges, const double *ir_wavl,
                          const int *n_sol_edges, const double *sol_wavl, char *err);
void radtran_set_photons_sol(void *ptr, const int *n, const double *photons_sol, char *err);
void radtran_create_end(void *ptr, const int *num_zenith_angles, const double *surface_albedo,
                        char *err);


void radtran_radiate_wrapper(void *ptr, const double *T_surface, const int *dim_T,
                             const double *T, const int *dim_P, const double *P,
                             const int *dim1_d, const int *dim2_d, const double *densities,
                             const int *dim_dz, const double *dz, const int *has_particles,
                             const int *dim1_p, const int *dim2_p, const double *pdensities,
                             const int *dim1_r, const int *dim2_r, const double *radii,
                             const int *compute_solar,
                             const int *compute_opacity, char *err);
void radtran_toa_fluxes_wrapper(void *ptr, const double *T_surface, const int *dim_T,
                                const double *T, const int *dim_P, const double *P,
                                const int *dim1_d, const int *dim2_d, const double *densities,
                                const int *dim_dz, const double *dz, const int *has_particles,
                                const int *dim1_p, const int *dim2_p, const double *pdensities,
                                const int *dim1_r, const int *dim2_r, const double *radii,
                                const int *compute_solar,
                                const int *compute_opacity, double *ISR, double *OLR,
                                char *err);
void radtran_apply_radiation_enhancement(void *ptr, const double *rad_enhancement);
void radtran_set_custom_optical_properties(void *ptr, const int *dim_wv, const double *wv, const int *dim_P,
                                           const double *P, const int *dim1_dtau_dz, const int *dim2_dtau_dz,
                                           const double *dtau_dz, const int *dim1_w0, const int *dim2_w0,
                                           const double *w0, const int *dim1_g0, const int *dim2_g0,
                                           const double *g0, char *err);
void radtran_unset_custom_optical_properties(void *ptr);

void radtran_upload_column(void *ptr, const double *T_surface, const double *T, const double *P,
                           const double *densities, const double *dz, const double *pdensities,
                           const double *radii, char *err);
void radtran_radiate_resident(void *ptr, const int *compute_solar, const int *compute_opacity,
                              char *err);
void radtran_synchronize(void *ptr, char *err);
void radtran_flux_device_ptr(void *ptr, void **dptr, int *count);
void radtran_set_bin_shard(void *ptr, const int *rank, const int *world, char *err);
void radtran_bin_shard_get(void *ptr, int *op_lo, int *op_n, int *ir_lo, int *ir_n, int *sol_lo,
                           int *sol_n);
void radtran_finish_reduced(void *ptr, char *err);

#define CLIMA_COMM_ID_BYTES 128
void radtran_set_device(const int *device, char *err);
void radtran_comm_unique_id(char *id , char *err);
void radtran_comm_init_rank(void *ptr, const int *nranks, const int *rank, const char *id, char *err);
void radtran_comm_init_file(void *ptr, const int *nranks, const int *rank, const char *path, char *err);
void radtran_comm_get(void *ptr, int *nranks, int *rank, int *reduces);
void radtran_comm_destroy(void *ptr);
void radtran_toa_fluxes_batch(void *ptr, const int *ncol, const double *T_surface, const double *T, const double *P,
                              const double *densities, const double *dz, const int *has_particles,
                              const double *pdensities, const double *radii, double *ISR, double *OLR,
                              double *fluxes, char *err);
void radtran_toa_fluxes_batch_device(void *ptr, const int *ncol, const double *d_T_surface, const double *d_T,
                                     const double *d_P, const double *d_densities, const double *d_dz,
                                     const int *has_particles, const double *d_pdensities, const double *d_radii,
                                     double *d_ISR, double *d_OLR, double *d_fluxes, const void *producer_stream,
                                     char *err);
void clima_test_pack_columns(void *ptr, const int *ncol, const double *T_surface, const double *T, const double *P,
                             const double *densities, const double *dz, const int *has_particles, const double *pdensities,
                             const double *radii, double *blocks, int *col_count, char *err);
void clima_test_pack_columns_host(void *ptr, const int *ncol, const double *T_surface, const double *T, const double *P,
                                  const double *densities, const double *dz, const int *has_particles,
                                  const double *pdensities, const double *radii, double *blocks, int *col_count, char *err);
void radtran_radiate_ir_batch(void *ptr, const int *ncol, const double *T_surface, const int *dim1_T,
                              const int *dim2_T, const double *T, double *fup_n, double *fdn_n,
                              double *f_total, char *err);
void radtran_ir_jacobian(void *ptr, const double *T_surface, const int *dim_T, const double *T,
                         const int *dim1, const int *dim2, double *jac_up, double *jac_dn, double *jac_total, char *err);
void radtran_ir_jacobian_reduced(void *ptr, const double *T_surface, const int *dim_T, const double *T,
                                 const int *dim_x, const int *group_of_x, const int *ngroup,
                                 const int *nrow, const int *row_level,
                                 const int *dim1, const int *dim2,
                                 double *jac_up, double *jac_dn, double *jac_total, char *err);
void radtran_opacities2yaml_wrapper_1(void *ptr, int *out_len, void **out_cp);
void radtran_opacities2yaml_wrapper_2(void *ptr, void **out_cp, const int *out_len, char *out_c);
void radtran_set_names(void *ptr, const char *species_names, const char *particle_names, char *err);
void radtran_set_opacity_labels(void *ptr, const char *k_method, const char *water_continuum_model,
                                const char *particle_data, char *err);
void radtran_fused_set(void *ptr, const int *enable);
void radtran_fused_get(void *ptr, int *enabled);
void radtran_create_from_files(void *ptr, const char *settings_file, const char *star_file, const int *num_zenith_angles,
                               const double *surface_albedo, const int *nz, const char *datadir, char *err);
void radtran_load_from_files(void *ptr, const char *settings_file, const char *star_file, const int *nz, const char *datadir, char *err);
void radtran_dims_get(void *ptr, int *nz, int *nsp, int *np, int *nw, int *ngauss);
void radtran_names_get(void *ptr, const int *cap, char *species_names, char *particle_names);
void radtran_spectra_get_all(void *ptr, const bool *do_solar, const int *nlev, const int *nw_ir, const int *nw_sol,
                             double *ir_fup_a, double *ir_fdn_a, double *ir_tau_band,
                             double *sol_fup_a, double *sol_fdn_a, double *sol_amean, double *sol_tau_band, char *err);
void radtran_spectra_release(void *ptr);
void radtran_batch_pin_results_set(void *ptr, const int *flag);
void radtran_batch_pin_results_get(void *ptr, int *flag);
void radtran_coop_items_set(void *ptr, const int *items);
void radtran_coop_items_get(void *ptr, int *items);
void radtran_fused_spins_set(void *ptr, const int *spins);
void radtran_fused_spins_get(void *ptr, int *spins);
void radtran_ir_green_set(void *ptr, const int *mode);
void radtran_ir_green_get(void *ptr, int *mode, int *batches);
void radtran_fused_fallbacks_get(void *ptr, int *count);
void radtran_stream_get(void *ptr, void **stream);
void radtran_profile_set(void *ptr, const int *enable);
void radtran_profile_stride_set(void *ptr, const int *stride);
void radtran_kernel_time_get(void *ptr, const int *kernel_id, double *ms_total, int *launches,
                             char *err);
void radtran_profile_reset(void *ptr);
void radtran_algorithmic_bytes(void *ptr, double *bytes_tables_distinct, double *bytes_in,
                               double *bytes_out, double *bytes_tables_full, char *err);

void radtran_algorithmic_nodes(void *ptr, double *n_pt, double *n_pt_full, double *n_t, double *n_t_full, char *err);

void clima_bench_toa_fluxes(void *ptr, const int *n, const double *T_surface, const int *dim_T, const double *T,
                            const int *dim_P, const double *P, const int *dim1_d, const int *dim2_d,
                            const double *densities, const int *dim_dz, const double *dz, const int *has_particles,
                            const int *dim1_p, const int *dim2_p, const double *pdensities, const int *dim1_r,
                            const int *dim2_r, const double *radii, double *us, double *ISR, double *OLR, char *err);
void clima_bench_resident_sync(void *ptr, const int *n, double *us, char *err);
void clima_bench_resident_graph(void *ptr, const int *n, const int *k, double *us, char *err);

void clima_test_device_exp(const int *n, const double *x, double *y, char *err);
void clima_test_host_tables_digest(void *ptr, unsigned long long *digest);
void clima_test_device_exp_table(const int *n, const int *base10, const double *x, double *y, char *err);
void clima_test_device_rcp(const int *n, const double *x, double *y, char *err);
void clima_test_wave_scan(const int *nwaves, const double *a, const double *b, double *out, char *err);

void clima_test_two_stream(const int *nz, const int *ng, const int *form, const int *slots, const double *tau,
                           const double *w0, const double *g, const double *bplanck, const double *ir_par,
                           const double *sol_par, const double *wbin, double *ir_fup, double *ir_fdn,
                           double *sol_fup, double *sol_fdn, double *sol_amean, char *err);
void clima_test_ir_response(const int *nz, const int *ng, const double *tau, const double *w0, const double *g,
                            const double *ir_par, const double *wbin, const int *ndev, const int *dev_k,
                            const double *dev_db, double *resp_up, double *resp_dn, char *err);

void clima_test_green_far_form_set(const int *vector_form);

void radtran_opr_get(void *ptr, double *tau, double *w0, double *g, double *tau_band, char *err);

void radtran_set_bolometric_flux_wrapper(void *ptr, const double *flux);
void radtran_bolometric_flux_wrapper(void *ptr, double *flux);
void radtran_skin_temperature_wrapper(void *ptr, const double *bond_albedo, double *T_skin);
void radtran_equilibrium_temperature_wrapper(void *ptr, const double *bond_albedo, double *T_eq);
void radtran_zenith_u_get_size(void *ptr, int *dim1);
void radtran_zenith_u_get(void *ptr, const int *dim1, double *arr);
void radtran_zenith_u_set(void *ptr, const int *dim1, const double *arr);
void radtran_zenith_weights_get(void *ptr, const int *dim1, double *arr);
void radtran_zenith_weights_set(void *ptr, const int *dim1, const double *arr);
void radtran_surface_albedo_get_size(void *ptr, int *dim1);
void radtran_surface_albedo_get(void *ptr, const int *dim1, double *arr);
void radtran_surface_albedo_set(void *ptr, const int *dim1, const double *arr);
void radtran_surface_emissivity_get_size(void *ptr, int *dim1);
void radtran_surface_emissivity_get(void *ptr, const int *dim1, double *arr);
void radtran_surface_emissivity_set(void *ptr, const int *dim1, const double *arr);
void radtran_has_hard_surface_get(void *ptr, bool *val);
void radtran_has_hard_surface_set(void *ptr, const bool *val);
void radtran_photon_scale_factor_get(void *ptr, double *val);
void radtran_photon_scale_factor_set(void *ptr, const double *val);
void radtran_ir_tau_min_get(void *ptr, double *val);
void radtran_ir_tau_min_set(void *ptr, const double *val);
void radtran_diurnal_fac_get(void *ptr, double *val);
void radtran_diurnal_fac_set(void *ptr, const double *val);
void radtran_ir_get(void *ptr, void **ptr1);
void radtran_sol_get(void *ptr, void **ptr1);
void radtran_wrk_ir_get(void *ptr, void **ptr1);
void radtran_wrk_sol_get(void *ptr, void **ptr1);
void radtran_f_total_get_size(void *ptr, int *dim1);
void radtran_f_total_get(void *ptr, const int *dim1, double *arr);
void radtran_photons_sol_get_size(void *ptr, int *dim1);
void radtran_photons_sol_get(void *ptr, const int *dim1, double *arr);

void climaradtranwrk_fup_a_get_size(void *ptr, int *dim1, int *dim2);
void climaradtranwrk_fup_a_get(void *ptr, const int *dim1, const int *dim2, double *arr);
void climaradtranwrk_fdn_a_get_size(void *ptr, int *dim1, int *dim2);
void climaradtranwrk_fdn_a_get(void *ptr, const int *dim1, const int *dim2, double *arr);
void climaradtranwrk_fup_n_get_size(void *ptr, int *dim1);
void climaradtranwrk_fup_n_get(void *ptr, const int *dim1, double *arr);
void climaradtranwrk_fdn_n_get_size(void *ptr, int *dim1);
void climaradtranwrk_fdn_n_get(void *ptr, const int *dim1, double *arr);
void climaradtranwrk_amean_get_size(void *ptr, int *dim1, int *dim2);
void climaradtranwrk_amean_get(void *ptr, const int *dim1, const int *dim2, double *arr);
void climaradtranwrk_tau_band_get_size(void *ptr, int *dim1, int *dim2);
void climaradtranwrk_tau_band_get(void *ptr, const int *dim1, const int *dim2, double *arr);

void rtchannel_wavl_get_size(void *ptr, int *dim1);
void rtchannel_wavl_get(void *ptr, const int *dim1, double *arr);
void rtchannel_freq_get_size(void *ptr, int *dim1);
void rtchannel_freq_get(void *ptr, const int *dim1, double *arr);

#ifdef __cplusplus
}
#endif
#endif
```

Baseline: 11280 calls/s.

## Fold prep work into the fused opacity/two-stream grid with spin-wait flags

```diff
diff --git a/clima_amd/csrc/kernels.hip b/clima_amd/csrc/kernels.hip
--- a/clima_amd/csrc/kernels.hip
+++ b/clima_amd/csrc/kernels.hip
@@ -284,13 +284,23 @@
   return c;
 }
 
-__global__ __launch_bounds__(256) void k_prep(PrepParams p) {
-  __shared__ double s_axis[PREP_AXIS_MAX];
+template <bool COHERENT, typename V>
+__device__ __forceinline__ void st_opr(V *p, V v) {
+  if constexpr (COHERENT) __hip_atomic_store(p, v, __ATOMIC_RELAXED, __HIP_MEMORY_SCOPE_AGENT);
+  else *p = v;
+}
+template <bool COHERENT, typename V>
+__device__ __forceinline__ V ld_opr(const V *p) {
+  if constexpr (COHERENT) return __hip_atomic_load(p, __ATOMIC_RELAXED, __HIP_MEMORY_SCOPE_AGENT);
+  else return *p;
+}
+
+template <bool COHERENT>
+__device__ __forceinline__ void prep_body(const PrepHandle &p, const ColumnDev &c, const int call_id, const int item,
+                                          double *s_axis, const int axis_max) {
   const int nz = p.nz;
-  const int cb = blockIdx.y;
-  const ColumnDev c = column_at(p.col, p.bs, cb);
   const int *src = c.meta + 1 + nz;
-  if (blockIdx.x == 0) {
+  if (item == 0) {
     for (int j = threadIdx.x; j < nz; j += blockDim.x) {
       const double Pj = c.P[j], dzj = c.dz[j];
       double fc = 0.0;
@@ -303,26 +313,18 @@
           const int i = i0 + k;
           if (i < p.nsp) {
             const double col = d[k] * dzj;
-            c.cols[i * nz + j] = col;
+            st_opr<COHERENT>(&c.cols[i * nz + j], col);
             if (p.has_cont && i != p.LH2O) fc = fc + col;
           }
         }
       }
-      c.log10P[j] = log10(Pj);
-      c.foreign_col[j] = fc;
+      st_opr<COHERENT>(&c.log10P[j], log10(Pj));
+      st_opr<COHERENT>(&c.foreign_col[j], fc);
     }
     return;
   }
-  if ((int)blockIdx.x > p.nslots + p.nabs) {
-    const int zb = (int)blockIdx.x - (p.nslots + p.nabs + 1);
-    const int arr = zb / PREP_ZERO_BLOCKS, part = zb - arr * PREP_ZERO_BLOCKS;
-    double *dst = p.zero_ptr[arr] + (size_t)cb * p.bs.res;
-    const size_t n = p.zero_count[arr];
-    for (size_t i = (size_t)part * blockDim.x + threadIdx.x; i < n; i += (size_t)PREP_ZERO_BLOCKS * blockDim.x) dst[i] = 0.0;
-    return;
-  }
-  if ((int)blockIdx.x > p.nslots) {
-    const int e = (int)blockIdx.x - p.nslots - 1;
+  if (item > p.nslots) {
+    const int e = item - p.nslots - 1;
     const int a = p.abs_a[e], b = p.abs_b[e], kind = p.abs_kind[e];
     for (int j = threadIdx.x; j < nz; j += blockDim.x) {
       double w;
@@ -336,13 +338,13 @@
           if (i != p.LH2O) fc = fc + c.dens[i * nz + j] * c.dz[j];
         w = c.dens[a * nz + j] * fc;
       }
-      c.absw[e * nz + j] = w;
+      st_opr<COHERENT>(&c.absw[e * nz + j], w);
     }
     return;
   }
-  const int s = blockIdx.x - 1;
+  const int s = item - 1;
   const SlotDev &sl = p.slots[s];
-  const bool in_lds = sl.n <= PREP_AXIS_MAX;
+  const bool in_lds = sl.n <= axis_max;
   const double *in = sl.source <= 0 ? c.P : sl.source == 1 ? c.T : c.radii + (size_t)(sl.source - 2) * nz;
   const int j0 = threadIdx.x;
   int js0 = 0;
@@ -359,16 +361,34 @@
     if (sl.source < 0) x = log10(xin * 1.0e6);
     else if (sl.source == 0) x = log10(xin);
     else x = xin;
-    if (sl.flag_clamp && (x < sl.lo || x > sl.hi)) atomicMax(c.err_flag, p.call_id);
+    if (sl.flag_clamp && (x < sl.lo || x > sl.hi)) atomicMax(c.err_flag, call_id);
     x = fmin(fmax(x, sl.lo), sl.hi);
     const int i = bracket(axis, sl.n, x);
-    c.ix[s * nz + j] = i;
-    c.q[s * nz + j] = (x - axis[i]) / (axis[i + 1] - axis[i]);
-  }
+    st_opr<COHERENT>(&c.ix[s * nz + j], i);
+    st_opr<COHERENT>(&c.q[s * nz + j], (x - axis[i]) / (axis[i + 1] - axis[i]));
+  }
+}
+
+int prep_items(const PrepHandle &h) { return 1 + h.nslots + h.nabs; }
+
+__global__ __launch_bounds__(256) void k_prep(PrepParams p) {
+  __shared__ double s_axis[PREP_AXIS_MAX];
+  const int cb = blockIdx.y;
+  const int items = 1 + p.h.nslots + p.h.nabs;
+  if ((int)blockIdx.x >= items) {
+    const int zb = (int)blockIdx.x - items;
+    const int arr = zb / PREP_ZERO_BLOCKS, part = zb - arr * PREP_ZERO_BLOCKS;
+    double *dst = p.zero_ptr[arr] + (size_t)cb * p.bs.res;
+    const size_t n = p.zero_count[arr];
+    for (size_t i = (size_t)part * blockDim.x + threadIdx.x; i < n; i += (size_t)PREP_ZERO_BLOCKS * blockDim.x) dst[i] = 0.0;
+    return;
+  }
+  const ColumnDev c = column_at(p.col, p.bs, cb);
+  prep_body<false>(p.h, c, p.call_id, (int)blockIdx.x, s_axis, PREP_AXIS_MAX);
 }
 
 void launch_prep(const PrepParams &p, hipStream_t s) {
-  hipLaunchKernelGGL(k_prep, dim3(1 + p.nslots + p.nabs + p.nzero * PREP_ZERO_BLOCKS, p.ncol > 0 ? p.ncol : 1), dim3(256), 0, s, p);
+  hipLaunchKernelGGL(k_prep, dim3(prep_items(p.h) + p.nzero * PREP_ZERO_BLOCKS, p.ncol > 0 ? p.ncol : 1), dim3(256), 0, s, p);
 }
 
 
@@ -379,17 +399,6 @@
 
 constexpr int OP_THREADS = 256;
 constexpr int HWREG_HW_ID_WAVE_ID = (3 << 11) | (0 << 6) | 4;
-
-template <bool COHERENT>
-__device__ __forceinline__ void st_opr(double *p, double v) {
-  if constexpr (COHERENT) __hip_atomic_store(p, v, __ATOMIC_RELAXED, __HIP_MEMORY_SCOPE_AGENT);
-  else *p = v;
-}
-template <bool COHERENT>
-__device__ __forceinline__ double ld_opr(const double *p) {
-  if constexpr (COHERENT) return __hip_atomic_load(p, __ATOMIC_RELAXED, __HIP_MEMORY_SCOPE_AGENT);
-  else return *p;
-}
 
 #ifdef CLIMA_STAMPS
 __device__ long long *g_stamp_buf = nullptr;
@@ -628,9 +637,15 @@
   double tausg, taua, tauc, tausc, taup, tausp, gt;
 };
 
-template <int RM, bool CUSTOM, bool COHERENT>
-__device__ __forceinline__ void opacity8_body(const OpacityParams &p, const int tile, const size_t oc,
-                                              const size_t opf, const size_t oo) {
+struct PrepWait {
+  const int *done;
+  int n, call_id, max_spins;
+  int *timeout_flag;
+};
+
+template <int RM, bool CUSTOM, bool COHERENT, bool PREP = false>
+__device__ __forceinline__ bool opacity8_body(const OpacityParams &p, const int tile, const size_t oc,
+                                              const size_t opf, const size_t oo, const PrepWait &pw) {
   const ColumnDev &c = p.col;
   constexpr int NG = 8;
   __shared__ double sI[RM == 0 ? 1 : NG][OP_THREADS];
@@ -653,7 +668,30 @@
     if (tid < 2 * NG + 1) s_Ew[tid] = tid < NG + 1 ? v_e : v_w;
     if (tid < NG) rW[tid] = 1.0 / (v_e1 - v_e);
   }
-  __syncthreads();
+  if constexpr (PREP) {
+    __shared__ int s_prep_ok[OP_THREADS / 64];
+    int ok = 1;
+    for (int t = tid; t < pw.n; t += OP_THREADS) {
+      int spins = 0;
+      while (__hip_atomic_load(&pw.done[t], __ATOMIC_RELAXED, __HIP_MEMORY_SCOPE_AGENT) != pw.call_id) {
+        __builtin_amdgcn_s_sleep(16);
+        if (++spins > pw.max_spins) { ok = 0; break; }
+      }
+      if (!ok) break;
+    }
+    const int wave_ok = __all(ok);
+    if ((tid & 63) == 0) s_prep_ok[tid >> 6] = wave_ok;
+    __syncthreads();
+    int all_ok = 1;
+#pragma unroll
+    for (int w = 0; w < OP_THREADS / 64; w++) all_ok &= s_prep_ok[w];
+    if (!all_ok) {
+      if (tid == 0) atomicMax(pw.timeout_flag, pw.call_id);
+      return false;
+    }
+  } else {
+    __syncthreads();
+  }
 
 #ifdef CLIMA_STAMPS
   const long long wt0 = __builtin_amdgcn_s_memrealtime();
@@ -679,7 +717,7 @@
     const double dzj = c.dz[oc + jl];
     double tausg = 0.0;
   #pragma unroll 4
-    for (int i = 0; i < p.nray; i++) tausg = tausg + p.ray[i].data[l] * c.cols[opf + p.ray[i].sp1 * nz + jl];
+    for (int i = 0; i < p.nray; i++) tausg = tausg + p.ray[i].data[l] * ld_opr<PREP>(&c.cols[opf + p.ray[i].sp1 * nz + jl]);
     double taua = 0.0;
     constexpr int AB = ABS_BATCH;
     for (int e0 = 0; e0 < p.nabs; e0 += AB) {
@@ -688,9 +726,9 @@
   #pragma unroll
       for (int u = 0; u < AB; u++) {
         const AbsEntry &x = p.abs[e0 + u];
-        ixx[u] = c.ix[2 * opf + x.slot * nz + jl];
-        qq[u] = c.q[opf + x.slot * nz + jl];
-        ww[u] = c.absw[opf + (e0 + u) * nz + jl];
+        ixx[u] = ld_opr<PREP>(&c.ix[2 * opf + x.slot * nz + jl]);
+        qq[u] = ld_opr<PREP>(&c.q[opf + x.slot * nz + jl]);
+        ww[u] = ld_opr<PREP>(&c.absw[opf + (e0 + u) * nz + jl]);
       }
       double v0[AB], v1[AB];
   #pragma unroll
@@ -715,8 +753,8 @@
     double tauc = TINY, tausc = TINY * TINY;
     double g0c = TINY;
     if constexpr (CUSTOM) {
-      const int ix = c.ix[2 * opf + p.cust.slot * nz + jl];
-      const double q = c.q[opf + p.cust.slot * nz + jl];
+      const int ix = ld_opr<PREP>(&c.ix[2 * opf + p.cust.slot * nz + jl]);
+      const double q = ld_opr<PREP>(&c.q[opf + p.cust.slot * nz + jl]);
       const size_t o = (size_t)l * p.cust.nP;
       tauc = lerp1(p.cust.dtau + o, ix, q) * dzj;
       const double w0c = lerp1(p.cust.w0 + o, ix, q);
@@ -727,8 +765,8 @@
     double tausp_1[MAX_PART], gtp[MAX_PART];
     for (int i = 0; i < p.npart; i++) {
       const PartDev &pt = p.part[i];
-      const int ix = c.ix[2 * opf + pt.slot * nz + jl];
-      const double q = c.q[opf + pt.slot * nz + jl];
+      const int ix = ld_opr<PREP>(&c.ix[2 * opf + pt.slot * nz + jl]);
+      const double q = ld_opr<PREP>(&c.q[opf + pt.slot * nz + jl]);
       const double w0p = lerp1(pt.w0 + (size_t)l * pt.nrad, ix, q);
       const double qext = lerp1(pt.qext + (size_t)l * pt.nrad, ix, q);
       gtp[i] = lerp1(pt.gt + (size_t)l * pt.nrad, ix, q);
@@ -765,7 +803,7 @@
     const double *f21 = f11 + NG;
     const double *f12 = f11 + (size_t)kd.nP * NG;
     const double *f22 = f12 + NG;
-    const double col = c.cols[opf + kd.sp * nz + jl];
+    const double col = ld_opr<PREP>(&c.cols[opf + kd.sp * nz + jl]);
 #pragma unroll
     for (int g = 0; g < NG; g++) {
       const double fx1 = p1 * f11[g] + q1 * f21[g];
@@ -776,8 +814,8 @@
   double tk[NG];
 #pragma unroll
   for (int g = 0; g < NG; g++) tk[g] = 0.0;
-  int iP_n = c.ix[2 * opf + p.k[0].slotP * nz + j], iT_n = c.ix[2 * opf + p.k[0].slotT * nz + j];
-  double q1_n = c.q[opf + p.k[0].slotP * nz + j], q2_n = c.q[opf + p.k[0].slotT * nz + j];
+  int iP_n = ld_opr<PREP>(&c.ix[2 * opf + p.k[0].slotP * nz + j]), iT_n = ld_opr<PREP>(&c.ix[2 * opf + p.k[0].slotT * nz + j]);
+  double q1_n = ld_opr<PREP>(&c.q[opf + p.k[0].slotP * nz + j]), q2_n = ld_opr<PREP>(&c.q[opf + p.k[0].slotT * nz + j]);
   for (int s = 0; s < p.nk; s++) {
     const int iP = iP_n, iT = iT_n;
     const double q1 = q1_n, q2 = q2_n;
@@ -785,8 +823,8 @@
     if constexpr (RM == 0 && RORR_ASM) asm volatile("" : "+v"(jv));
     if (s + 1 < p.nk) {
       const KDev &kn = p.k[s + 1];
-      iP_n = c.ix[2 * opf + kn.slotP * nz + jv]; iT_n = c.ix[2 * opf + kn.slotT * nz + jv];
-      q1_n = c.q[opf + kn.slotP * nz + jv]; q2_n = c.q[opf + kn.slotT * nz + jv];
+      iP_n = ld_opr<PREP>(&c.ix[2 * opf + kn.slotP * nz + jv]); iT_n = ld_opr<PREP>(&c.ix[2 * opf + kn.slotT * nz + jv]);
+      q1_n = ld_opr<PREP>(&c.q[opf + kn.slotP * nz + jv]); q2_n = ld_opr<PREP>(&c.q[opf + kn.slotT * nz + jv]);
     }
     double kc[NG];
     k_times_col(s, jv, iP, iT, q1, q2, kc);
@@ -856,8 +894,8 @@
         layer_terms(j + 1, lt2);
         if (p.nk == 1) {
           double tk2[NG];
-          k_times_col(0, j + 1, c.ix[2 * opf + p.k[0].slotP * nz + j], c.ix[2 * opf + p.k[0].slotT * nz + j], c.q[opf + p.k[0].slotP * nz + j],
-                      c.q[opf + p.k[0].slotT * nz + j], tk2);
+          k_times_col(0, j + 1, ld_opr<PREP>(&c.ix[2 * opf + p.k[0].slotP * nz + j]), ld_opr<PREP>(&c.ix[2 * opf + p.k[0].slotT * nz + j]), ld_opr<PREP>(&c.q[opf + p.k[0].slotP * nz + j]),
+                      ld_opr<PREP>(&c.q[opf + p.k[0].slotT * nz + j]), tk2);
           store_layer(n - 1, lt2, tk2);
         } else {
           store_layer(n - 1, lt2, tk);
@@ -865,11 +903,12 @@
       }
     }
   }
+  return true;
 }
 
 template <int RM, bool CUSTOM>
 __global__ __launch_bounds__(OP_THREADS, 2) void k_opacity8(OpacityParams p) {
-  opacity8_body<RM, CUSTOM, false>(p, (int)blockIdx.x, 0, 0, 0);
+  opacity8_body<RM, CUSTOM, false>(p, (int)blockIdx.x, 0, 0, 0, PrepWait{});
 }
 
 constexpr int OPG_MAX_NG = 32;
@@ -2632,16 +2671,32 @@
 #ifndef FUSED_NZMAX
 #define FUSED_NZMAX 8
 #endif
-template <int RM, bool CUSTOM, int LSEL, bool PAIRED = false, bool HALF = false>
+template <int RM, bool CUSTOM, int LSEL, bool PAIRED = false, bool HALF = false, bool PREP = false>
 __global__ __launch_bounds__(OP_THREADS, 2) void k_fused(OpacityParams op, TwoStreamParams ts, FusedParams fp) {
   extern __shared__ __align__(16) double lds[];
-  const int per_col = fp.n_op + fp.n_ts;
-  const int cb = (int)blockIdx.x / per_col, loc = (int)blockIdx.x - cb * per_col;
+  const int n_prep = PREP ? fp.n_prep : 0;
+  const int per_col = n_prep + fp.n_op + fp.n_ts;
+  const int cb = (int)blockIdx.x / per_col, loc = (int)blockIdx.x - cb * per_col - n_prep;
+  if constexpr (PREP) {
+  if (loc < 0) {
+    __builtin_amdgcn_s_setprio(1);
+    const int item = loc + n_prep;
+    prep_body<true>(*fp.prep, op.col, fp.call_id, item, lds, fp.lds_doubles);
+    __builtin_amdgcn_fence(__ATOMIC_RELEASE, "workgroup");
+    asm volatile("s_waitcnt vmcnt(0)" ::: "memory");
+    __syncthreads();
+    if (threadIdx.x == 0) __hip_atomic_store(&fp.prep_done[item], fp.call_id, __ATOMIC_RELAXED, __HIP_MEMORY_SCOPE_AGENT);
+    return;
+  }
+  }
   if (loc < fp.n_op) {
     __builtin_amdgcn_s_setprio(1);
     const size_t oc = (size_t)cb * fp.bs.col;
-    if ((long)loc * OP_THREADS < (long)op.nbins * op.col.meta[2 * oc])
-      opacity8_body<RM, CUSTOM, true>(op, loc, oc, (size_t)cb * fp.bs.prep, (size_t)cb * fp.bs.opr);
+    if ((long)loc * OP_THREADS < (long)op.nbins * op.col.meta[2 * oc]) {
+      if (!opacity8_body<RM, CUSTOM, true, PREP>(op, loc, oc, (size_t)cb * fp.bs.prep, (size_t)cb * fp.bs.opr,
+                                                 PrepWait{fp.prep_done, n_prep, fp.call_id, fp.max_spins, fp.timeout_flag}))
+        return;
+    }
     __builtin_amdgcn_fence(__ATOMIC_RELEASE, "workgroup");
     asm volatile("s_waitcnt vmcnt(0)" ::: "memory");
     __syncthreads();
@@ -2783,11 +2838,15 @@
   pl.prep_clears = in.compute_opacity && !in.ts_block_mode && slots <= 8 && wave_groups(in.ng) >= 2 && !whole_stores;
   pl.caller_clears = in.ir_batch && wave_groups(in.ng) > 1;
   pl.ts.zero_launch = pl.ts.groups > 1 && !pl.prep_clears && !pl.caller_clears;
+  pl.prep_in_grid = in.prep_in_grid && pl.fused.form == TS_HALF && !in.batch && in.ncol <= 1 && !pl.prep_clears;
   return pl;
 }
 
 using FusedKern = void (*)(OpacityParams, TwoStreamParams, FusedParams);
-static FusedKern fused_kernel(const TsPlan &f, int rebin_mode, bool cust_on) {
+static FusedKern fused_kernel(const TsPlan &f, int rebin_mode, bool cust_on, bool prep = false) {
+  static const FusedKern khp[5] = {k_fused<0, false, 3, false, true, true>, k_fused<0, false, 4, false, true, true>, k_fused<0, false, 5, false, true, true>,
+                                   k_fused<0, false, 6, false, true, true>, k_fused<0, false, 7, false, true, true>};
+  if (prep) return f.form == TS_HALF ? khp[f.slots - 3] : nullptr;
   static const FusedKern kp[3] = {k_fused<0, false, 0, true>, k_fused<0, false, 6, true>, k_fused<0, false, 8, true>};
   static const FusedKern kh[5] = {k_fused<0, false, 3, false, true>, k_fused<0, false, 4, false, true>, k_fused<0, false, 5, false, true>,
                                   k_fused<0, false, 6, false, true>, k_fused<0, false, 7, false, true>};
@@ -2811,8 +2870,10 @@
   }
   ts.col_base = 0; ts.accumulate = f.groups > 1 ? 1 : 0;
   ts.scat = op.scat; ts.w0_from_scat = op.write_w0 ? 0 : 1;
-  const long items = (long)fp.ncol * (fp.n_op + fp.n_ts);
-  const FusedKern k = fused_kernel(f, op.rebin_mode, op.cust.on != 0);
+  if (fp.n_prep > 0 && (fp.ncol > 1 || !fp.prep || !fp.prep_done || f.form != TS_HALF)) return false;
+  fp.lds_doubles = (int)(f.lds / sizeof(double));
+  const long items = (long)fp.ncol * (fp.n_prep + fp.n_op + fp.n_ts);
+  const FusedKern k = fused_kernel(f, op.rebin_mode, op.cust.on != 0, fp.n_prep > 0);
   if (f.lds > 48 * 1024 && !ensure_max_lds((const void *)k, 64 * 1024)) return false;
   hipLaunchKernelGGL(k, dim3((unsigned)items), dim3(OP_THREADS), f.lds, s, op, ts, fp);
   return true;
diff --git a/clima_amd/csrc/radtran_api.hip b/clima_amd/csrc/radtran_api.hip
--- a/clima_amd/csrc/radtran_api.hip
+++ b/clima_amd/csrc/radtran_api.hip
@@ -227,6 +227,11 @@
   bool ts_block_mode = false;
   int ts_ncols_env = 0;
   DevBuf<int> d_done;
+  bool prep_in_grid = true;
+  DevBuf<PrepHandle> d_prep_handle;
+  PrepHandle prep_handle_current;
+  bool prep_handle_valid = false;
+  DevBuf<int> d_prep_done;
   int profile = 0;
   long timer_calls = 0;
   int profile_stride = 1;
@@ -643,22 +648,35 @@
   PrepParams pp;
   std::memset(&pp, 0, sizeof(pp));
   pp.ncol = b.ncol; pp.bs = b.bs;
-  pp.nz = r->nz; pp.nsp = r->nsp; pp.np = r->np; pp.nslots = r->nslots;
-  pp.has_cont = r->has_cont; pp.LH2O = r->LH2O;
-  for (int s = 0; s < r->nslots; s++) pp.slots[s] = r->slots[s];
+  PrepHandle &h = pp.h;
+  h.nz = r->nz; h.nsp = r->nsp; h.np = r->np; h.nslots = r->nslots;
+  h.has_cont = r->has_cont; h.LH2O = r->LH2O;
+  for (int s = 0; s < r->nslots; s++) h.slots[s] = r->slots[s];
   if (r->cust_on) {
     SlotDev cs;
+    std::memset(&cs, 0, sizeof(cs));
     cs.axis = r->d_cust_axis.p; cs.n = r->cust_nP; cs.source = -1;
     cs.lo = -std::numeric_limits<double>::infinity(); cs.hi = std::numeric_limits<double>::infinity();
     cs.flag_clamp = 0;
-    pp.slots[pp.nslots++] = cs;
-  }
-  pp.nabs = (int)r->abs_entries.size();
-  for (int e = 0; e < pp.nabs; e++) { pp.abs_kind[e] = r->abs_entries[e].kind; pp.abs_a[e] = r->abs_entries[e].a; pp.abs_b[e] = r->abs_entries[e].b; }
+    h.slots[h.nslots++] = cs;
+  }
+  h.nabs = (int)r->abs_entries.size();
+  for (int e = 0; e < h.nabs; e++) { h.abs_kind[e] = r->abs_entries[e].kind; h.abs_a[e] = r->abs_entries[e].a; h.abs_b[e] = r->abs_entries[e].b; }
   pp.col = col;
   pp.call_id = call_id;
   if (clears) pp.nzero = ts_clear_ranges(*clears, pp.zero_ptr, pp.zero_count);
   return pp;
+}
+
+const PrepHandle *prep_handle_dev(Radtran *r, const PrepHandle &h) {
+  if (r->prep_handle_valid && std::memcmp(&h, &r->prep_handle_current, sizeof(h)) == 0) return r->d_prep_handle.p;
+  if (!r->d_prep_handle.p) r->d_prep_handle.alloc(1);
+  if (!r->d_prep_done.p) { r->d_prep_done.alloc(1 + MAX_SLOTS + MAX_ABS); r->d_prep_done.zero(r->stream); }
+  r->prep_handle_current = h;
+  HIPCHK(hipMemcpyAsync(r->d_prep_handle.p, &r->prep_handle_current, sizeof(h), hipMemcpyHostToDevice, r->stream));
+  HIPCHK(hipStreamSynchronize(r->stream));
+  r->prep_handle_valid = true;
+  return r->d_prep_handle.p;
 }
 
 OpacityParams make_opacity_params(Radtran *r, const CallBufs &b, const ColumnDev &col, bool write_w0) {
@@ -725,6 +743,7 @@
   in.nsrc = b.nsrc;
   in.rebin_mode = r->rebin_mode; in.cust_on = r->cust_on; in.compute_opacity = compute_opacity;
   in.all_pairs = compute_opacity && b.all_pairs_exact;
+  in.prep_in_grid = r->prep_in_grid;
   in.fused = r->fused; in.allow_fused = allow_fused; in.generic_opacity = r->generic_opacity;
   in.ts_block_mode = r->ts_block_mode; in.ts_ncols_env = r->ts_ncols_env; in.coop_items = r->coop_items;
   in.no_half = sw_no_half(); in.allow_paired = sw_paired(); in.w0_from_scat = sw_w0_scat();
@@ -749,7 +768,9 @@
   if (compute_opacity) {
     const int call_id = ++r->call_id;
     const PrepParams pp = make_prep_params(r, b, col, call_id, plan.prep_clears ? &ts : nullptr);
-    { KernelTimer t(r, 0); launch_prep(pp, r->stream); HIPCHK(hipGetLastError()); t.stop(); }
+    bool prep_done = false;
+    auto run_prep = [&] { KernelTimer t(r, 0); launch_prep(pp, r->stream); HIPCHK(hipGetLastError()); t.stop(); prep_done = true; };
+    if (!plan.prep_in_grid) run_prep();
 
     OpacityParams op = make_opacity_params(r, b, col, plan.write_w0);
     if (plan.fused.form != TS_NONE) {
@@ -758,12 +779,16 @@
       fp.ncol = b.ncol; fp.bs = b.bs;
       fp.call_id = call_id; fp.max_spins = r->fused_max_spins;
       fp.done = b.done; fp.timeout_flag = r->d_err.p + 1;
+      if (plan.prep_in_grid) {
+        fp.prep = prep_handle_dev(r, pp.h); fp.prep_done = r->d_prep_done.p; fp.n_prep = prep_items(pp.h);
+      }
       KernelTimer t(r, 1);
       fused_done = launch_fused(op, ts, fp, plan.fused, r->stream);
       HIPCHK(hipGetLastError());
       t.stop();
       if (!fused_done) op = make_opacity_params(r, b, col, true);
     }
+    if (!fused_done && !prep_done) run_prep();
     if (chunk && !fused_done) throw HipFail{"internal: a one-launch batch needs the fused grid"};
     if (!fused_done) {
       KernelTimer t(r, 1);
@@ -1307,6 +1332,14 @@
   Radtran *r = as_rad(ptr);
   *enabled = (r && r->fused) ? 1 : 0;
 }
+void radtran_prep_in_grid_set(void *ptr, const int *enable) {
+  Radtran *r = as_rad(ptr);
+  if (r) r->prep_in_grid = (*enable != 0);
+}
+void radtran_prep_in_grid_get(void *ptr, int *enabled) {
+  Radtran *r = as_rad(ptr);
+  *enabled = (r && r->prep_in_grid) ? 1 : 0;
+}
 void radtran_coop_items_set(void *ptr, const int *items) {
   Radtran *r = as_rad(ptr);
   if (r) r->coop_items = *items;
@@ -1372,6 +1405,7 @@
   HIPCHK(hipStreamCreateWithFlags(&r->stream, hipStreamNonBlocking));
   HIPCHK(hipEventCreateWithFlags(&r->ev_upload, hipEventDisableTiming));
   if (const char *f = getenv("CLIMA_HIP_FUSED")) r->fused = atoi(f) != 0;
+  if (const char *f = getenv("CLIMA_HIP_PREP_IN_GRID")) r->prep_in_grid = atoi(f) != 0;
   if (const char *f = getenv("CLIMA_HIP_GENERIC")) r->generic_opacity = atoi(f) != 0;
   if (const char *f = getenv("CLIMA_HIP_TS_MODE")) r->ts_block_mode = std::strcmp(f, "block") == 0;
   if (const char *f = getenv("CLIMA_HIP_TS_NCOLS")) r->ts_ncols_env = atoi(f);
diff --git a/clima_amd/csrc/radtran_dev.h b/clima_amd/csrc/radtran_dev.h
--- a/clima_amd/csrc/radtran_dev.h
+++ b/clima_amd/csrc/radtran_dev.h
@@ -107,14 +107,18 @@
   CustomDev cust;
 };
 
+struct PrepHandle {
+  int nz, nsp, np, nslots, has_cont, LH2O;
+  SlotDev slots[MAX_SLOTS];
+  int nabs;
+  int abs_kind[MAX_ABS], abs_a[MAX_ABS], abs_b[MAX_ABS];
+};
+
 struct PrepParams {
   int ncol;
   BatchStrides bs;
-  int nz, nsp, np, nslots, has_cont, LH2O;
   int call_id;
-  SlotDev slots[MAX_SLOTS];
-  int nabs;
-  int abs_kind[MAX_ABS], abs_a[MAX_ABS], abs_b[MAX_ABS];
+  PrepHandle h;
   int nzero;
   double *zero_ptr[6];
   size_t zero_count[6];
@@ -163,6 +167,10 @@
   int slots;
   int sol_early;
   BatchStrides bs;
+  int n_prep;
+  int lds_doubles;
+  const PrepHandle *prep;
+  int *prep_done;
 };
 
 struct IntegrateParams {
@@ -280,6 +288,7 @@
   int rebin_mode;
   bool cust_on, compute_opacity;
   bool all_pairs;
+  bool prep_in_grid;
   bool fused, allow_fused, generic_opacity, ts_block_mode, no_half, allow_paired, w0_from_scat;
   long coop_items;
   int ts_ncols_env;
@@ -302,6 +311,7 @@
   TsPlan ts;
   TsPlan block;
   bool prep_clears;
+  bool prep_in_grid;
   bool caller_clears;
   bool write_w0;
 };
@@ -309,6 +319,7 @@
 int ts_clear_ranges(const TwoStreamParams &p, double *ptr[6], size_t count[6]);
 
 void launch_prep(const PrepParams &p, hipStream_t s);
+int prep_items(const PrepHandle &h);
 bool launch_opacity(const OpacityParams &p, const LaunchPlan &pl, hipStream_t s);
 bool launch_twostream(TwoStreamParams &p, const TsPlan &t, hipStream_t s);
 bool launch_twostream_w(TwoStreamParams &p, const TsPlan &t, hipStream_t s);
diff --git a/clima_amd/lib.py b/clima_amd/lib.py
--- a/clima_amd/lib.py
+++ b/clima_amd/lib.py
@@ -36,6 +36,8 @@
     "radtran_set_opacity_labels": [_vp, _err, _err, _err, _err],
     "radtran_fused_set": [_vp, _ip],
     "radtran_fused_get": [_vp, _ip],
+    "radtran_prep_in_grid_set": [_vp, _ip],
+    "radtran_prep_in_grid_get": [_vp, _ip],
     "radtran_fused_fallbacks_get": [_vp, _ip],
     "radtran_ir_green_set": [_vp, _ip],
     "radtran_ir_green_get": [_vp, _ip, _ip],
diff --git a/clima_amd/radtran.py b/clima_amd/radtran.py
--- a/clima_amd/radtran.py
+++ b/clima_amd/radtran.py
@@ -458,6 +458,16 @@
         self._L.radtran_fused_set(self._ptr, _i(1 if on else 0))
 
     @property
+    def prep_in_grid(self):
+        v = C.c_int()
+        self._L.radtran_prep_in_grid_get(self._ptr, C.byref(v))
+        return bool(v.value)
+
+    @prep_in_grid.setter
+    def prep_in_grid(self, on):
+        self._L.radtran_prep_in_grid_set(self._ptr, _i(1 if on else 0))
+
+    @property
     def coop_items(self):
         v = C.c_int()
         self._L.radtran_coop_items_get(self._ptr, C.byref(v))
diff --git a/include/clima_radtran_hip.h b/include/clima_radtran_hip.h
--- a/include/clima_radtran_hip.h
+++ b/include/clima_radtran_hip.h
@@ -117,6 +117,8 @@
                                 const char *particle_data, char *err);
 void radtran_fused_set(void *ptr, const int *enable);
 void radtran_fused_get(void *ptr, int *enabled);
+void radtran_prep_in_grid_set(void *ptr, const int *enable);
+void radtran_prep_in_grid_get(void *ptr, int *enabled);
 void radtran_create_from_files(void *ptr, const char *settings_file, const char *star_file, const int *num_zenith_angles,
                                const double *surface_albedo, const int *nz, const char *datadir, char *err);
 void radtran_load_from_files(void *ptr, const char *settings_file, const char *star_file, const int *nz, const char *datadir, char *err);
```

Measured after the change: 10930 calls/s. -3.1%, worse.
